# NVlabs/intrinsic3d

Measured on AMD Instinct MI355X. Metric: Gauss-Newton iterations/s at the finest SDF level, higher is better.
Workload: dtype f32

## Files before the change

### include/intrinsic3d_hip.h

```cpp
#ifndef INTRINSIC3D_HIP_H
#define INTRINSIC3D_HIP_H
#include <stdint.h>
#ifdef __cplusplus
extern "C" {
#endif

typedef struct i3d_context i3d_context;

typedef enum {
    I3D_OK = 0,
    I3D_ERR_INVALID_ARGUMENT = 1,
    I3D_ERR_NO_DEVICE = 2,
    I3D_ERR_HIP = 3,
    I3D_ERR_STATE = 4,
    I3D_ERR_CAPACITY = 5,
    I3D_ERR_COMM = 6,
    I3D_ERR_IO = 7
} i3d_status;

int  i3d_create(int32_t device_ordinal, i3d_context** out);
void i3d_destroy(i3d_context* ctx);
const char* i3d_last_error(const i3d_context* ctx);
const char* i3d_version(void);

// ... 173 lines not shown
    i3d_track_stats base;
    int64_t photo_samples;
    double  photo_rms_initial, photo_rms_final;
} i3d_track_rgbd_stats;

void i3d_track_rgbd_desc_default(i3d_track_rgbd_desc* d);
int  i3d_track_frame_rgbd(i3d_context* ctx, const i3d_track_rgbd_desc* desc, int32_t width, int32_t height, const float* depth, const float* luminance,
                          double* pose6_io, i3d_track_rgbd_stats* stats);
int  i3d_debug_track_rgbd_sums(i3d_context* ctx, const i3d_track_rgbd_desc* desc, int32_t width, int32_t height, const float* depth, const float* luminance,
                               int32_t level, const double* pose_ref6, const double* pose_cur6, double* sums31, int64_t* inliers, int64_t* photo_samples);

int i3d_png_info(const uint8_t* data, uint64_t size, int32_t* width, int32_t* height, int32_t* channels, int32_t* bit_depth);
int i3d_png_decode(const uint8_t* data, uint64_t size, void* pixels, uint64_t capacity_bytes);
int i3d_pose_mat_to_vec6(const float* cam_to_world16, double* pose6);
typedef struct i3d_sensor i3d_sensor;
int  i3d_sensor_open(const char* folder, int32_t max_frames, float min_depth, float max_depth, i3d_sensor** out);
int  i3d_sensor_open_yaml(const char* sensor_yml, i3d_sensor** out, float* min_depth , float* max_depth );
void i3d_sensor_close(i3d_sensor* s);
int  i3d_sensor_info(const i3d_sensor* s, int32_t* num_frames, int32_t* num_loaded, int32_t* color_wh , int32_t* depth_wh ,
                     float* color_intr4 , float* depth_intr4);
int  i3d_sensor_color(const i3d_sensor* s, int32_t id, uint8_t* bgr );
int  i3d_sensor_depth(const i3d_sensor* s, int32_t id, float* depth );
int  i3d_sensor_pose(const i3d_sensor* s, int32_t id, float* cam_to_world16);
int  i3d_sensor_set_pose(i3d_sensor* s, int32_t id, const float* cam_to_world16);
int  i3d_sensor_set_pose_vec6(i3d_sensor* s, int32_t id, const double* pose_world_to_cam6);
int  i3d_sensor_save_poses(const i3d_sensor* s, const char* path);
int i3d_keyframes_load(const char* path, int32_t* window_size, uint64_t capacity, double* scores, uint8_t* is_keyframe, uint64_t* count);
int i3d_keyframes_save(const char* path, int32_t window_size, uint64_t count, const double* scores, const uint8_t* is_keyframe);
int i3d_keyframes_select(int32_t window_size, uint64_t count, const double* scores, uint8_t* is_keyframe);
int i3d_blur_score(const uint8_t* image, int32_t width, int32_t height, int32_t channels, double* score);
int i3d_init_frames_from_sensor(i3d_context* ctx, int32_t device_ordinal, const i3d_sensor* s, uint64_t num_flags, const uint8_t* is_keyframe,
                                int32_t num_rgbd_levels, int32_t frame_capacity, int32_t* frame_ids, int32_t* num_keyframes);

typedef struct i3d_fusion i3d_fusion;
int  i3d_fusion_create(int32_t device_ordinal, float voxel_size, float depth_min, float depth_max, const float* clip6, uint64_t initial_capacity, i3d_fusion** out);
void i3d_fusion_destroy(i3d_fusion* f);
const char* i3d_fusion_last_error(const i3d_fusion* f);
int  i3d_fusion_integrate(i3d_fusion* f, int32_t depth_w, int32_t depth_h, const float* depth_intr4, int32_t color_w, int32_t color_h, const float* color_intr4,
                          const float* depth, const uint8_t* bgr, const float* pose_cam_to_world16, int32_t erode_window);
int  i3d_fusion_finish(i3d_fusion* f, int32_t correct_iterations, uint64_t* count);
int  i3d_fusion_info(const i3d_fusion* f, uint64_t* frames, uint64_t* allocated, uint64_t* capacity, int32_t* correct_launches);
int  i3d_fusion_get(const i3d_fusion* f, int32_t* keys, float* sdf, float* weight, uint8_t* color);
int  i3d_fusion_save(const i3d_fusion* f, const char* path);

int i3d_fusion_render(i3d_fusion* f, const i3d_render_desc* desc, float* depth, float* normal, i3d_render_stats* stats);
int i3d_fusion_track(i3d_fusion* f, const i3d_track_desc* desc, int32_t width, int32_t height, const float* depth, double* pose6_io, i3d_track_stats* stats);

typedef struct {
    int32_t use_refined_sdf;
    int32_t project;
    int32_t max_steps;
    double  tolerance_voxels;
} i3d_query_desc;

typedef struct {
    int64_t valid, projected;
    double  sum_abs_sdf, sum_sq_sdf, max_abs_sdf;
    double  sum_abs_distance, sum_sq_distance, max_abs_distance;
    int64_t steps;
} i3d_query_stats;

void i3d_query_desc_default(i3d_query_desc* d);
int  i3d_query_points(i3d_context* ctx, const i3d_query_desc* desc, int64_t n, const double* points,
                      double* sdf, float* normal , float* albedo, double* foot , double* distance, uint8_t* status, i3d_query_stats* stats);
int  i3d_fusion_query_points(i3d_fusion* f, const i3d_query_desc* desc, int64_t n, const double* points,
                             double* sdf, float* normal , double* foot , double* distance, uint8_t* status, i3d_query_stats* stats);

typedef struct {
    int32_t use_refined_sdf;
    int32_t iterations;
    double  max_distance;
    double  stop_rotation, stop_translation;
} i3d_register_desc;

typedef struct {
    int32_t iterations;
    int32_t status;
    int64_t valid, inliers;
    double  rms_initial, rms_final;
    double  min_pivot_ratio;
} i3d_register_stats;

void i3d_register_desc_default(i3d_register_desc* d);
int  i3d_register_points(i3d_context* ctx, const i3d_register_desc* desc, int64_t n, const double* points , double* pose6_io, i3d_register_stats* stats);
int  i3d_fusion_register_points(i3d_fusion* f, const i3d_register_desc* desc, int64_t n, const double* points, double* pose6_io, i3d_register_stats* stats);

typedef struct {
    int32_t use_refined_sdf;
    int32_t use_context_camera;
    double  intrinsics4[4], distortion5[5];
    int32_t iterations;
    int32_t stride;
    double  max_distance;
    double  huber_delta;
    float   min_depth, max_depth;
    double  stop_rotation, stop_translation;
} i3d_track_sdf_desc;

typedef struct {
    int32_t iterations, status;
    int64_t valid_pixels, valid, inliers;
    double  rms_initial, rms_final;
    double  min_pivot_ratio;
} i3d_track_sdf_stats;

void i3d_track_sdf_desc_default(i3d_track_sdf_desc* d);
int  i3d_track_frame_sdf(i3d_context* ctx, const i3d_track_sdf_desc* desc, int32_t width, int32_t height, const float* depth, double* pose6_io,
                         i3d_track_sdf_stats* stats);
int  i3d_fusion_track_sdf(i3d_fusion* f, const i3d_track_sdf_desc* desc, int32_t width, int32_t height, const float* depth, double* pose6_io,
                          i3d_track_sdf_stats* stats);

int  i3d_track_frames_sdf(i3d_context* ctx, const i3d_track_sdf_desc* desc, int32_t num_frames, int32_t width, int32_t height,
                          const float* depth, double* poses6_io, i3d_track_sdf_stats* stats);
int  i3d_track_keyframes_sdf(i3d_context* ctx, const i3d_track_sdf_desc* desc, int32_t level, int32_t num, const int32_t* frames,
                             double* poses6_io, i3d_track_sdf_stats* stats);

int i3d_comm_unique_id(void* out128, int32_t* bytes);
int i3d_comm_init(i3d_context* ctx, int32_t rank, int32_t world, const void* unique_id, int32_t id_bytes);
void* i3d_comm_sim_create(int32_t world);
void  i3d_comm_sim_destroy(void* shared);
int   i3d_comm_init_sim(i3d_context* ctx, void* shared, int32_t rank);
int   i3d_shard_plan(int32_t A, int32_t world, int32_t rank, const int32_t* anbr, const uint8_t* active,
                     int32_t* chunk, int32_t* own0, int32_t* own1, uint8_t* in_compute_list );
int32_t i3d_shard_vec_index(int32_t a, int32_t chunk, int32_t albedo);
int   i3d_shard_need(int32_t A, int32_t world, const int32_t* anbr , const uint8_t* active , uint64_t* need );
int   i3d_comm_stats(i3d_context* ctx, int64_t* halo_calls, int64_t* halo_bytes_sent, int64_t* reduce_calls, int64_t* reduce_bytes,
                     int32_t* halo_entries_send, int32_t* halo_entries_recv, int32_t* ghost_tiles, int32_t* compute_list);
const char* i3d_comm_transport(i3d_context* ctx);

enum { I3D_K_CLASSIFY = 0, I3D_K_OBSERVE, I3D_K_BUILD, I3D_K_EG_PASS , I3D_K_GATHER, I3D_K_COST, I3D_K_VECTOR, I3D_K_SH,
       I3D_K_EG_AUX ,
       I3D_K_COMM ,
       I3D_K_EG_MR2, I3D_K_EG_MR3 , I3D_K_COUNT };
int i3d_timing_enable(i3d_context* ctx, int32_t on);
int i3d_timing_select(i3d_context* ctx, uint32_t category_mask);
int i3d_timing_get(i3d_context* ctx, double* ms , int64_t* launches , int32_t reset);
int i3d_timing_get_work(i3d_context* ctx, double* ms , int64_t* launches );
int i3d_timing_get_work_ex(i3d_context* ctx, double* ms, int64_t* launches, double* slow_ms , int64_t* slow_launches );
const char* i3d_kernel_name(int32_t k);
int i3d_problem_sizes(i3d_context* ctx, int64_t out[6]);

int i3d_debug_assemble(i3d_context* ctx, const i3d_optimizer_config* cfg, int32_t iteration, int32_t* slots_out);
int64_t i3d_debug_map_order(const int32_t* keys, int64_t n, int32_t mode, int32_t* order);
int i3d_debug_flags(i3d_context* ctx, uint8_t* flags );
int i3d_debug_eg_rows(i3d_context* ctx, int32_t* frame , float* weight ,
                      float* residual , float* jac );
int i3d_debug_reg_rows(i3d_context* ctx, uint8_t* has_er , uint8_t* has_es , float* ea_weight );
int i3d_debug_neighbors(i3d_context* ctx, int32_t* nbr );
int i3d_debug_normal_eq(i3d_context* ctx, double* gradient, double* jtj_diag, double* cost);
int i3d_debug_jtj_apply(i3d_context* ctx, const double* x, double* y);
int i3d_debug_counters(i3d_context* ctx, int64_t* stream_syncs);
int i3d_debug_ladder_stats(i3d_context* ctx, int64_t* out6);
int i3d_debug_ladder_passes(i3d_context* ctx, int64_t* out8);
int i3d_debug_cull_stats(i3d_context* ctx, int64_t* pairs, int64_t* culled);

int i3d_debug_register_sums(i3d_context* ctx, const i3d_register_desc* desc, int64_t n, const double* points, const double* pose6, const double* pivot3,
                            double* sums29, int64_t* valid);
int i3d_debug_register_row_cap(i3d_context* ctx, int32_t rows);
int i3d_debug_track_sdf_sums(i3d_context* ctx, const i3d_track_sdf_desc* desc, int32_t width, int32_t height, const float* depth,
                             const double* pose6 , const double* pivot3, double* sums29, int64_t* valid, int64_t* valid_pixels);
int i3d_debug_track_batch_frames(i3d_context* ctx, int32_t frames_per_chunk);

#ifdef __cplusplus
}
#endif
#endif
```

### intrinsic3d_amd/binding.py

```python
from __future__ import annotations

import ctypes as C
import os

import numpy as np

_HERE = os.path.dirname(os.path.abspath(__file__))
LIB_PATH = os.environ.get("I3D_LIB") or os.path.join(_HERE, "libintrinsic3d_hip.so")

K_NAMES = ["classify", "observe", "build", "eg_pass", "gather", "cost", "vector", "sh", "eg_aux", "comm", "eg_mr2", "eg_mr3"]


class OptimizerConfig(C.Structure):
    _fields_ = [("iterations", C.c_int32), ("lm_steps", C.c_int32),
                ("lambda_g", C.c_double), ("lambda_r0", C.c_double), ("lambda_r1", C.c_double),
                ("lambda_s0", C.c_double), ("lambda_s1", C.c_double), ("lambda_a", C.c_double),
                ("fix_poses", C.c_int32), ("fix_intrinsics", C.c_int32), ("fix_distortion", C.c_int32),
                ("occlusion_distance", C.c_float), ("num_observations", C.c_int32),
                ("thres_shell", C.c_double), ("grid_level", C.c_int32), ("rgbd_level", C.c_int32),
                ("pcg_fixed_iterations", C.c_int32), ("verbose", C.c_int32), ("carry_trust_radius", C.c_int32), ("fix_sdf", C.c_int32)]


class IterationStats(C.Structure):
    _fields_ = [("rows", C.c_int64 * 4), ("weight_sum", C.c_double * 4), ("type_weight", C.c_double * 4),
# ... 93 lines not shown
    names = tuple(k for k in QUERY_OUTPUTS if has_albedo or k != "albedo")
    if outputs is None:
        outputs = tuple(k for k in names if d.project or k not in ("foot", "distance"))
    unknown = set(outputs) - set(names)
    if unknown:
        raise ValueError(f"{what}: unknown outputs {sorted(unknown)}")
    shape = {"sdf": ((n,), np.float64), "normal": ((n, 3), np.float32), "albedo": ((n,), np.float32), "foot": ((n, 3), np.float64),
             "distance": ((n,), np.float64), "status": ((n,), np.uint8)}
    out = {k: np.zeros(*shape[k]) for k in outputs}
    st = QueryStats()
    check(call(C.byref(d), n, _p(pts), *[_p(out.get(k)) for k in names], C.byref(st)), what)
    out["stats"] = st.as_dict()
    return out


class RegisterDesc(C.Structure):
    _fields_ = [("use_refined_sdf", C.c_int32), ("iterations", C.c_int32), ("max_distance", C.c_double), ("stop_rotation", C.c_double),
                ("stop_translation", C.c_double)]


class RegisterStats(C.Structure):
    _fields_ = [("iterations", C.c_int32), ("status", C.c_int32), ("valid", C.c_int64), ("inliers", C.c_int64), ("rms_initial", C.c_double),
                ("rms_final", C.c_double), ("min_pivot_ratio", C.c_double)]

    def as_dict(self):
        return {k: (float if t is C.c_double else int)(getattr(self, k)) for k, t in self._fields_}


def register_desc_default(**kw) -> RegisterDesc:
    d = RegisterDesc()
    load().i3d_register_desc_default(C.byref(d))
    for k, v in kw.items():
        if k == "refined":
            d.use_refined_sdf = int(bool(v))
        elif k in dict(RegisterDesc._fields_):
            setattr(d, k, v)
        else:
            raise ValueError(f"register_desc_default: unknown field {k}")
    return d


def _register(call, what, check, points, pose, desc):
    d = register_desc_default(**desc)
    pts = np.ascontiguousarray(points, np.float64).reshape(-1, 3)
    p6 = np.array(pose, np.float64).reshape(6).copy()
    st = RegisterStats()
    check(call(C.byref(d), pts.shape[0], _p(pts), _p(p6), C.byref(st)), what)
    return p6, st.as_dict()


class TrackSdfDesc(C.Structure):
    _fields_ = [("use_refined_sdf", C.c_int32), ("use_context_camera", C.c_int32), ("intrinsics4", C.c_double * 4), ("distortion5", C.c_double * 5),
                ("iterations", C.c_int32), ("stride", C.c_int32), ("max_distance", C.c_double), ("huber_delta", C.c_double),
                ("min_depth", C.c_float), ("max_depth", C.c_float), ("stop_rotation", C.c_double), ("stop_translation", C.c_double)]


class TrackSdfStats(C.Structure):
    _fields_ = [("iterations", C.c_int32), ("status", C.c_int32), ("valid_pixels", C.c_int64), ("valid", C.c_int64), ("inliers", C.c_int64),
                ("rms_initial", C.c_double), ("rms_final", C.c_double), ("min_pivot_ratio", C.c_double)]

    def as_dict(self):
        return {k: (float if t is C.c_double else int)(getattr(self, k)) for k, t in self._fields_}


def track_sdf_desc_default(**kw) -> TrackSdfDesc:
    d = TrackSdfDesc()
    load().i3d_track_sdf_desc_default(C.byref(d))
    for k, v in kw.items():
        if k in ("intr", "intrinsics4"):
            d.intrinsics4[:] = [float(x) for x in v]
        elif k in ("dist", "distortion5"):
            d.distortion5[:] = [float(x) for x in v]
        elif k == "refined":
            d.use_refined_sdf = int(bool(v))
        elif k in dict(TrackSdfDesc._fields_):
            setattr(d, k, v)
        else:
            raise ValueError(f"track_sdf_desc_default: unknown field {k}")
    return d


def _track_sdf(call, what, check, depth, pose6, d):
    dep = np.ascontiguousarray(depth, np.float32)
    h, w = dep.shape
    pose = np.ascontiguousarray(np.asarray(pose6, np.float64).reshape(6)).copy()
    st = TrackSdfStats()
    check(call(C.byref(d), int(w), int(h), _p(dep), _p(pose), C.byref(st)), what)
    return pose, st.as_dict()


def track_desc_default(**kw) -> TrackDesc:
    d = TrackDesc()
    load().i3d_track_desc_default(C.byref(d))
    for k, v in kw.items():
        if k == "iterations":
            it = [int(x) for x in v] + [0] * (4 - len(v))
            d.iterations[:] = it[:4]
        elif k in ("intr", "intrinsics4"):
            d.intrinsics4[:] = [float(x) for x in v]; d.use_context_camera = 0
        elif k in ("dist", "distortion5"):
            d.distortion5[:] = [float(x) for x in v]; d.use_context_camera = 0
        elif k == "refined":
            d.use_refined_sdf = int(bool(v))
        elif k in dict(TrackDesc._fields_):
            setattr(d, k, v)
        else:
            raise ValueError(f"track_desc_default: unknown field {k}")
    return d


def track_rgbd_desc_default(**kw) -> TrackRgbdDesc:
    d = TrackRgbdDesc()
    load().i3d_track_rgbd_desc_default(C.byref(d))
    own = ("geometric_weight", "photo_weight", "max_photo_residual")
    for k in own:
        if k in kw:
            setattr(d, k, float(kw[k]))
    base = {k: v for k, v in kw.items() if k not in own}
    if base:
        d.base = track_desc_default(**base)
    return d


REFINE_CALLBACK = C.CFUNCTYPE(None, C.c_void_p, C.c_int32, C.c_int32, C.c_int32, C.c_int32)


class GridView(C.Structure):
    _fields_ = [("num_voxels", C.c_int64), ("voxel_size", C.c_float), ("truncation", C.c_float),
                ("keys", C.c_void_p), ("sdf", C.c_void_p), ("sdf_refined", C.c_void_p), ("albedo", C.c_void_p),
                ("weight", C.c_void_p), ("color", C.c_void_p)]


EXPORTS = ["i3d_create", "i3d_destroy", "i3d_last_error", "i3d_version", "i3d_set_grid", "i3d_get_grid", "i3d_update_grid",
           "i3d_set_frames", "i3d_set_frames_rgbd", "i3d_get_frame_image", "i3d_resize_depth", "i3d_set_camera", "i3d_get_camera", "i3d_set_voxel_sh", "i3d_get_voxel_sh",
           "i3d_optimizer_config_default", "i3d_optimize", "i3d_optimize_host", "i3d_estimate_sh",
           "i3d_set_grid_from_tsdf_records", "i3d_recompute_colors", "i3d_clear_outside_thin_shell", "i3d_upsample", "i3d_grid_info",
           "i3d_export_grid", "i3d_refine",
           "i3d_tsdf_read_header", "i3d_tsdf_read_records", "i3d_tsdf_write", "i3d_sbr_write", "i3d_sbr_read", "i3d_write_poses",
           "i3d_write_intrinsics", "i3d_read_intrinsics", "i3d_config_load_yaml", "i3d_yaml_get",
           "i3d_extract_mesh", "i3d_get_mesh", "i3d_render_view", "i3d_track_desc_default", "i3d_track_frame", "i3d_track_rgbd_desc_default", "i3d_track_frame_rgbd",
           "i3d_query_desc_default", "i3d_query_points", "i3d_fusion_query_points",
           "i3d_register_desc_default", "i3d_register_points", "i3d_fusion_register_points", "i3d_debug_register_sums", "i3d_debug_register_row_cap",
           "i3d_track_sdf_desc_default", "i3d_track_frame_sdf", "i3d_fusion_track_sdf", "i3d_debug_track_sdf_sums",
           "i3d_track_frames_sdf", "i3d_track_keyframes_sdf", "i3d_debug_track_batch_frames",
           "i3d_export_mesh_ply", "i3d_write_ply", "i3d_mc_tables", "i3d_visualization_colors",
           "i3d_png_info", "i3d_png_decode", "i3d_pose_mat_to_vec6", "i3d_sensor_open", "i3d_sensor_open_yaml", "i3d_sensor_close", "i3d_sensor_info", "i3d_sensor_color",
           "i3d_sensor_depth", "i3d_sensor_pose", "i3d_sensor_set_pose", "i3d_sensor_set_pose_vec6", "i3d_sensor_save_poses",
           "i3d_mesh_remove_loose_components", "i3d_keyframes_load", "i3d_keyframes_save", "i3d_keyframes_select", "i3d_blur_score", "i3d_init_frames_from_sensor",
           "i3d_fusion_create", "i3d_fusion_destroy", "i3d_fusion_last_error", "i3d_fusion_integrate", "i3d_fusion_finish", "i3d_fusion_info", "i3d_fusion_get",
           "i3d_fusion_save", "i3d_fusion_render", "i3d_fusion_track", "i3d_shard_need", "i3d_comm_stats",
           "i3d_comm_unique_id", "i3d_comm_init", "i3d_comm_sim_create", "i3d_comm_sim_destroy", "i3d_comm_init_sim", "i3d_shard_plan", "i3d_shard_vec_index",
           "i3d_comm_transport", "i3d_timing_enable", "i3d_timing_select", "i3d_timing_get", "i3d_timing_get_work", "i3d_timing_get_work_ex", "i3d_kernel_name", "i3d_problem_sizes",
           "i3d_debug_assemble", "i3d_debug_map_order", "i3d_debug_flags", "i3d_debug_eg_rows", "i3d_debug_reg_rows", "i3d_debug_neighbors",
           "i3d_debug_normal_eq", "i3d_debug_jtj_apply", "i3d_debug_counters", "i3d_debug_cull_stats", "i3d_debug_ladder_stats", "i3d_debug_ladder_passes", "i3d_debug_track_sums", "i3d_debug_track_rgbd_sums"]

_lib = None


def load():
    global _lib
    if _lib is not None:
        return _lib
    if not os.path.exists(LIB_PATH):
        raise RuntimeError(f"{LIB_PATH} is missing: build it with `make -C intrinsic3d_amd/csrc` "
                           "(or __graft_entry__.build()); the product path has no CPU fallback")
    L = C.CDLL(LIB_PATH)
    vp, i32, i64, f32, f64 = C.c_void_p, C.c_int32, C.c_int64, C.c_float, C.c_double
    L.i3d_create.restype = i32; L.i3d_create.argtypes = [i32, C.POINTER(vp)]
    L.i3d_destroy.argtypes = [vp]
    L.i3d_last_error.restype = C.c_char_p; L.i3d_last_error.argtypes = [vp]
    L.i3d_version.restype = C.c_char_p
    L.i3d_set_grid.restype = i32; L.i3d_set_grid.argtypes = [vp, C.POINTER(GridView)]
    L.i3d_get_grid.restype = i32; L.i3d_get_grid.argtypes = [vp, vp, vp]
    L.i3d_update_grid.restype = i32; L.i3d_update_grid.argtypes = [vp, vp, vp, vp]
    L.i3d_set_frames.restype = i32; L.i3d_set_frames.argtypes = [vp, i32, i32, vp, vp, vp, vp, vp]
    L.i3d_set_frames_rgbd.restype = i32; L.i3d_set_frames_rgbd.argtypes = [vp, i32, i32, i32, i32, vp, vp]
    L.i3d_resize_depth.restype = i32; L.i3d_resize_depth.argtypes = [i32, i32, i32, vp, vp, i32, i32, vp, vp]
    L.i3d_get_frame_image.restype = i32; L.i3d_get_frame_image.argtypes = [vp, i32, i32, vp, vp]
    L.i3d_set_camera.restype = i32; L.i3d_set_camera.argtypes = [vp, vp, vp, vp]
    L.i3d_get_camera.restype = i32; L.i3d_get_camera.argtypes = [vp, vp, vp, vp]
    L.i3d_set_voxel_sh.restype = i32; L.i3d_set_voxel_sh.argtypes = [vp, vp]
    L.i3d_get_voxel_sh.restype = i32; L.i3d_get_voxel_sh.argtypes = [vp, vp]
    L.i3d_optimizer_config_default.argtypes = [C.POINTER(OptimizerConfig)]
    L.i3d_optimize.restype = i32; L.i3d_optimize.argtypes = [vp, C.POINTER(OptimizerConfig), vp]
    L.i3d_optimize_host.restype = i32
    L.i3d_optimize_host.argtypes = [i32, C.POINTER(OptimizerConfig), C.POINTER(GridView), vp, vp, i32, i32, vp, vp, vp, vp, vp, vp, vp, vp, vp]
    L.i3d_estimate_sh.restype = i32
    L.i3d_estimate_sh.argtypes = [vp, f32, f64, f64, C.POINTER(i32), vp, vp, i32, C.POINTER(ShStats)]
    L.i3d_comm_unique_id.restype = i32; L.i3d_comm_unique_id.argtypes = [vp, C.POINTER(i32)]
    L.i3d_comm_init.restype = i32; L.i3d_comm_init.argtypes = [vp, i32, i32, vp, i32]
    L.i3d_comm_sim_create.restype = vp; L.i3d_comm_sim_create.argtypes = [i32]
    L.i3d_comm_sim_destroy.argtypes = [vp]
    L.i3d_comm_init_sim.restype = i32; L.i3d_comm_init_sim.argtypes = [vp, vp, i32]
    L.i3d_shard_plan.restype = i32; L.i3d_shard_plan.argtypes = [i32, i32, i32, vp, vp, C.POINTER(i32), C.POINTER(i32), C.POINTER(i32), vp]
    L.i3d_shard_vec_index.restype = i32; L.i3d_shard_vec_index.argtypes = [i32, i32, i32]
    L.i3d_shard_need.restype = i32; L.i3d_shard_need.argtypes = [i32, i32, vp, vp, vp]
    L.i3d_comm_stats.restype = i32; L.i3d_comm_stats.argtypes = [vp] * 9
    L.i3d_timing_enable.restype = i32; L.i3d_timing_enable.argtypes = [vp, i32]
    L.i3d_timing_select.restype = i32; L.i3d_timing_select.argtypes = [vp, C.c_uint32]
    L.i3d_timing_get.restype = i32; L.i3d_timing_get.argtypes = [vp, vp, vp, i32]
    L.i3d_timing_get_work.restype = i32; L.i3d_timing_get_work.argtypes = [vp, vp, vp]
    L.i3d_timing_get_work_ex.restype = i32; L.i3d_timing_get_work_ex.argtypes = [vp, vp, vp, vp, vp]
    L.i3d_kernel_name.restype = C.c_char_p; L.i3d_kernel_name.argtypes = [i32]
    L.i3d_comm_transport.restype = C.c_char_p; L.i3d_comm_transport.argtypes = [vp]
    L.i3d_problem_sizes.restype = i32; L.i3d_problem_sizes.argtypes = [vp, vp]
    L.i3d_debug_assemble.restype = i32; L.i3d_debug_assemble.argtypes = [vp, C.POINTER(OptimizerConfig), i32, C.POINTER(i32)]
    L.i3d_debug_flags.restype = i32; L.i3d_debug_flags.argtypes = [vp, vp]
    L.i3d_debug_eg_rows.restype = i32; L.i3d_debug_eg_rows.argtypes = [vp, vp, vp, vp, vp]
    L.i3d_debug_reg_rows.restype = i32; L.i3d_debug_reg_rows.argtypes = [vp, vp, vp, vp]
    L.i3d_debug_neighbors.restype = i32; L.i3d_debug_neighbors.argtypes = [vp, vp]
    L.i3d_debug_normal_eq.restype = i32; L.i3d_debug_normal_eq.argtypes = [vp, vp, vp, C.POINTER(f64)]
    L.i3d_debug_jtj_apply.restype = i32; L.i3d_debug_jtj_apply.argtypes = [vp, vp, vp]
    L.i3d_debug_counters.restype = i32; L.i3d_debug_counters.argtypes = [vp, vp]
    L.i3d_debug_ladder_stats.restype = i32; L.i3d_debug_ladder_stats.argtypes = [vp, vp]
    L.i3d_debug_ladder_passes.restype = i32; L.i3d_debug_ladder_passes.argtypes = [vp, vp]
    L.i3d_debug_cull_stats.restype = i32; L.i3d_debug_cull_stats.argtypes = [vp, vp, vp]
    L.i3d_set_grid_from_tsdf_records.restype = i32; L.i3d_set_grid_from_tsdf_records.argtypes = [vp, f32, i64, vp, vp, vp, vp]
    L.i3d_recompute_colors.restype = i32; L.i3d_recompute_colors.argtypes = [vp, f32, i32]
    L.i3d_clear_outside_thin_shell.restype = i32; L.i3d_clear_outside_thin_shell.argtypes = [vp, f64, C.POINTER(i64)]
    L.i3d_upsample.restype = i32; L.i3d_upsample.argtypes = [vp, C.POINTER(i64)]
    L.i3d_grid_info.restype = i32; L.i3d_grid_info.argtypes = [vp, C.POINTER(i64), C.POINTER(f32), C.POINTER(f32)]
    L.i3d_export_grid.restype = i32; L.i3d_export_grid.argtypes = [vp, vp, vp, vp, vp, vp, vp]
    L.i3d_refine.restype = i32; L.i3d_refine.argtypes = [vp, C.POINTER(RefineConfig), C.POINTER(OptimizerConfig), REFINE_CALLBACK, vp]
    u64 = C.c_uint64; cp = C.c_char_p
    L.i3d_tsdf_read_header.restype = i32; L.i3d_tsdf_read_header.argtypes = [cp, C.POINTER(f32), C.POINTER(f32), C.POINTER(f32), C.POINTER(u64), C.POINTER(f32)]
    L.i3d_tsdf_read_records.restype = i32; L.i3d_tsdf_read_records.argtypes = [cp, u64, vp, vp, vp, vp]
    L.i3d_tsdf_write.restype = i32; L.i3d_tsdf_write.argtypes = [cp, f32, f32, f32, f32, u64, vp, vp, vp, vp]
    L.i3d_sbr_write.restype = i32; L.i3d_sbr_write.argtypes = [cp, f32, f32, f32, f32, u64, vp, vp, vp, vp, vp, vp]
    L.i3d_sbr_read.restype = i32; L.i3d_sbr_read.argtypes = [cp, u64, vp, vp, vp, vp, vp, vp]
    L.i3d_write_poses.restype = i32; L.i3d_write_poses.argtypes = [cp, i32, vp, vp]
    L.i3d_write_intrinsics.restype = i32; L.i3d_write_intrinsics.argtypes = [cp, i32, i32, vp, vp]
    L.i3d_read_intrinsics.restype = i32; L.i3d_read_intrinsics.argtypes = [cp, C.POINTER(i32), C.POINTER(i32), vp, vp]
    L.i3d_extract_mesh.restype = i32; L.i3d_extract_mesh.argtypes = [vp, i32, i32, i32, C.POINTER(i64), C.POINTER(i64)]
    L.i3d_get_mesh.restype = i32; L.i3d_get_mesh.argtypes = [vp, vp, vp, vp]
    L.i3d_export_mesh_ply.restype = i32; L.i3d_export_mesh_ply.argtypes = [vp, cp, i32, i32, i32]
    L.i3d_write_ply.restype = i32; L.i3d_write_ply.argtypes = [cp, i64, vp, vp, i64, vp]
    L.i3d_mesh_remove_loose_components.restype = i32; L.i3d_mesh_remove_loose_components.argtypes = [vp, vp, vp, vp, vp]
    L.i3d_render_view.restype = i32; L.i3d_render_view.argtypes = [vp, C.POINTER(RenderDesc), vp, vp, vp, vp, vp, vp, C.POINTER(RenderStats)]
    L.i3d_track_desc_default.restype = None; L.i3d_track_desc_default.argtypes = [C.POINTER(TrackDesc)]
    L.i3d_track_frame.restype = i32; L.i3d_track_frame.argtypes = [vp, C.POINTER(TrackDesc), i32, i32, vp, vp, C.POINTER(TrackStats)]
    L.i3d_debug_track_sums.restype = i32; L.i3d_debug_track_sums.argtypes = [vp, C.POINTER(TrackDesc), i32, i32, vp, i32, vp, vp, vp, vp]
    L.i3d_track_rgbd_desc_default.restype = None; L.i3d_track_rgbd_desc_default.argtypes = [C.POINTER(TrackRgbdDesc)]
    L.i3d_track_frame_rgbd.restype = i32; L.i3d_track_frame_rgbd.argtypes = [vp, C.POINTER(TrackRgbdDesc), i32, i32, vp, vp, vp, C.POINTER(TrackRgbdStats)]
    L.i3d_debug_track_rgbd_sums.restype = i32
    L.i3d_debug_track_rgbd_sums.argtypes = [vp, C.POINTER(TrackRgbdDesc), i32, i32, vp, vp, i32, vp, vp, vp, vp, vp]
    L.i3d_query_desc_default.restype = None; L.i3d_query_desc_default.argtypes = [C.POINTER(QueryDesc)]
    L.i3d_query_points.restype = i32; L.i3d_query_points.argtypes = [vp, C.POINTER(QueryDesc), i64, vp, vp, vp, vp, vp, vp, vp, C.POINTER(QueryStats)]
    L.i3d_fusion_query_points.restype = i32; L.i3d_fusion_query_points.argtypes = [vp, C.POINTER(QueryDesc), i64, vp, vp, vp, vp, vp, vp, C.POINTER(QueryStats)]
    L.i3d_register_desc_default.restype = None; L.i3d_register_desc_default.argtypes = [C.POINTER(RegisterDesc)]
    L.i3d_register_points.restype = i32; L.i3d_register_points.argtypes = [vp, C.POINTER(RegisterDesc), i64, vp, vp, C.POINTER(RegisterStats)]
    L.i3d_fusion_register_points.restype = i32; L.i3d_fusion_register_points.argtypes = [vp, C.POINTER(RegisterDesc), i64, vp, vp, C.POINTER(RegisterStats)]
    L.i3d_debug_register_sums.restype = i32; L.i3d_debug_register_sums.argtypes = [vp, C.POINTER(RegisterDesc), i64, vp, vp, vp, vp, C.POINTER(i64)]
    L.i3d_debug_register_row_cap.restype = i32; L.i3d_debug_register_row_cap.argtypes = [vp, i32]
    L.i3d_track_sdf_desc_default.restype = None; L.i3d_track_sdf_desc_default.argtypes = [C.POINTER(TrackSdfDesc)]
    L.i3d_track_frame_sdf.restype = i32; L.i3d_track_frame_sdf.argtypes = [vp, C.POINTER(TrackSdfDesc), i32, i32, vp, vp, C.POINTER(TrackSdfStats)]
    L.i3d_fusion_track_sdf.restype = i32; L.i3d_fusion_track_sdf.argtypes = [vp, C.POINTER(TrackSdfDesc), i32, i32, vp, vp, C.POINTER(TrackSdfStats)]
    L.i3d_debug_track_sdf_sums.restype = i32
    L.i3d_debug_track_sdf_sums.argtypes = [vp, C.POINTER(TrackSdfDesc), i32, i32, vp, vp, vp, vp, C.POINTER(i64), C.POINTER(i64)]
    L.i3d_track_frames_sdf.restype = i32; L.i3d_track_frames_sdf.argtypes = [vp, C.POINTER(TrackSdfDesc), i32, i32, i32, vp, vp, vp]
    L.i3d_track_keyframes_sdf.restype = i32; L.i3d_track_keyframes_sdf.argtypes = [vp, C.POINTER(TrackSdfDesc), i32, i32, vp, vp, vp]
    L.i3d_debug_track_batch_frames.restype = i32; L.i3d_debug_track_batch_frames.argtypes = [vp, i32]
    L.i3d_mc_tables.restype = i32; L.i3d_mc_tables.argtypes = [vp, vp]
    L.i3d_config_load_yaml.restype = i32; L.i3d_config_load_yaml.argtypes = [cp, C.POINTER(RefineConfig), C.POINTER(OptimizerConfig)]
    u64 = C.c_uint64; f32 = C.c_float
    L.i3d_fusion_create.restype = i32; L.i3d_fusion_create.argtypes = [i32, f32, f32, f32, vp, u64, C.POINTER(vp)]
    L.i3d_fusion_destroy.restype = None; L.i3d_fusion_destroy.argtypes = [vp]
    L.i3d_fusion_last_error.restype = C.c_char_p; L.i3d_fusion_last_error.argtypes = [vp]
    L.i3d_fusion_integrate.restype = i32; L.i3d_fusion_integrate.argtypes = [vp, i32, i32, vp, i32, i32, vp, vp, vp, vp, i32]
    L.i3d_fusion_finish.restype = i32; L.i3d_fusion_finish.argtypes = [vp, i32, vp]
    L.i3d_fusion_info.restype = i32; L.i3d_fusion_info.argtypes = [vp, vp, vp, vp, vp]
    L.i3d_fusion_get.restype = i32; L.i3d_fusion_get.argtypes = [vp, vp, vp, vp, vp]
    L.i3d_fusion_save.restype = i32; L.i3d_fusion_save.argtypes = [vp, cp]
    L.i3d_fusion_render.restype = i32; L.i3d_fusion_render.argtypes = [vp, C.POINTER(RenderDesc), vp, vp, C.POINTER(RenderStats)]
    L.i3d_fusion_track.restype = i32; L.i3d_fusion_track.argtypes = [vp, C.POINTER(TrackDesc), i32, i32, vp, vp, C.POINTER(TrackStats)]
    L.i3d_debug_map_order.restype = i64; L.i3d_debug_map_order.argtypes = [vp, i64, i32, vp]
    L.i3d_blur_score.restype = i32; L.i3d_blur_score.argtypes = [vp, i32, i32, i32, vp]
    L.i3d_yaml_get.restype = i32; L.i3d_yaml_get.argtypes = [cp, cp, vp, u64]
    L.i3d_png_info.restype = i32; L.i3d_png_info.argtypes = [vp, u64, vp, vp, vp, vp]
    L.i3d_png_decode.restype = i32; L.i3d_png_decode.argtypes = [vp, u64, vp, u64]
    L.i3d_pose_mat_to_vec6.restype = i32; L.i3d_pose_mat_to_vec6.argtypes = [vp, vp]
    L.i3d_sensor_open.restype = i32; L.i3d_sensor_open.argtypes = [cp, i32, f32, f32, C.POINTER(vp)]
    L.i3d_sensor_close.restype = None; L.i3d_sensor_close.argtypes = [vp]
    L.i3d_sensor_info.restype = i32; L.i3d_sensor_info.argtypes = [vp, vp, vp, vp, vp, vp, vp]
    L.i3d_sensor_color.restype = i32; L.i3d_sensor_color.argtypes = [vp, i32, vp]
    L.i3d_sensor_depth.restype = i32; L.i3d_sensor_depth.argtypes = [vp, i32, vp]
    L.i3d_sensor_pose.restype = i32; L.i3d_sensor_pose.argtypes = [vp, i32, vp]
    L.i3d_sensor_set_pose.restype = i32; L.i3d_sensor_set_pose.argtypes = [vp, i32, vp]
    L.i3d_sensor_set_pose_vec6.restype = i32; L.i3d_sensor_set_pose_vec6.argtypes = [vp, i32, vp]
    L.i3d_sensor_save_poses.restype = i32; L.i3d_sensor_save_poses.argtypes = [vp, cp]
    L.i3d_keyframes_load.restype = i32; L.i3d_keyframes_load.argtypes = [cp, vp, u64, vp, vp, vp]
    L.i3d_keyframes_save.restype = i32; L.i3d_keyframes_save.argtypes = [cp, i32, u64, vp, vp]
    L.i3d_keyframes_select.restype = i32; L.i3d_keyframes_select.argtypes = [i32, u64, vp, vp]
    L.i3d_init_frames_from_sensor.restype = i32; L.i3d_init_frames_from_sensor.argtypes = [vp, i32, vp, u64, vp, i32, i32, vp, vp]
    _lib = L
    return L


def default_config(**kw) -> OptimizerConfig:
    cfg = OptimizerConfig()
    load().i3d_optimizer_config_default(C.byref(cfg))
    for k, v in kw.items():
        setattr(cfg, k, v)
    return cfg


def _pyramid_sizes(w, h, levels):
    out = [(int(w), int(h))]
    for _ in range(1, int(levels)):
        out.append((out[-1][0] // 2, out[-1][1] // 2))
    return out


def _p(a):
    return None if a is None else a.ctypes.data_as(C.c_void_p)


class I3DError(RuntimeError):
    pass


class Context:

    def __init__(self, device: int = 0):
        self.L = load()
        h = C.c_void_p()
        rc = self.L.i3d_create(int(device), C.byref(h))
        if rc != 0:
            raise I3DError(f"i3d_create failed ({rc}): {self.L.i3d_last_error(None).decode()}")
        self.h = h
        self.N = 0
        self.K = 0
        self._keep = []

    def _check(self, rc, what):
        if rc != 0:
            raise I3DError(f"{what} failed ({rc}): {self.L.i3d_last_error(self.h).decode()}")

    def close(self):
        if self.h:
            self.L.i3d_destroy(self.h)
            self.h = None

    def __enter__(self):
        return self

    def __exit__(self, *a):
        self.close()

    def set_grid(self, voxel_size, keys, sdf, sdf_refined, albedo, weight, color, truncation=None):
        keys = np.ascontiguousarray(keys, np.int32); sdf = np.ascontiguousarray(sdf, np.float64)
        sr = np.ascontiguousarray(sdf_refined, np.float64); al = np.ascontiguousarray(albedo, np.float64)
        w = np.ascontiguousarray(weight, np.float32); col = np.ascontiguousarray(color, np.uint8)
        gv = GridView(keys.shape[0], float(voxel_size), float(np.float32(voxel_size) * np.float32(5.0)) if truncation is None else float(truncation),
                      _p(keys), _p(sdf), _p(sr), _p(al), _p(w), _p(col))
        self._check(self.L.i3d_set_grid(self.h, C.byref(gv)), "i3d_set_grid")
        self.N = keys.shape[0]

    def set_frames(self, frames, levels):
        K = len(frames); self.K = K
        ws = np.array([frames[0]["lum"][l].shape[1] for l in range(levels)], np.int32)
        hs = np.array([frames[0]["lum"][l].shape[0] for l in range(levels)], np.int32)
        self._sizes = [(int(w), int(h)) for w, h in zip(ws, hs)]
        arr_t = C.c_void_p * (K * levels)
        lum = arr_t(); dep = arr_t(); bgr = arr_t(); keep = []
        for f in range(K):
            for l in range(levels):
                a = np.ascontiguousarray(frames[f]["lum"][l], np.float32); b = np.ascontiguousarray(frames[f]["depth"][l], np.float32)
                c = frames[f].get("bgr")
# ... 173 lines not shown
    def track_frame_sdf(self, depth, pose6, **desc):
        return _track_sdf(lambda *a: self.L.i3d_track_frame_sdf(self.h, *a), "i3d_track_frame_sdf", self._check, depth, pose6, track_sdf_desc_default(**desc))

    def track_frames_sdf(self, depths, poses, **desc):
        d = track_sdf_desc_default(**desc)
        dep = np.ascontiguousarray(depths, np.float32)
        if dep.ndim != 3:
            raise ValueError("track_frames_sdf: depths must be [B, h, w]")
        n, h, w = dep.shape
        po = np.ascontiguousarray(np.asarray(poses, np.float64).reshape(-1, 6)).copy()
        if po.shape[0] != n:
            raise ValueError("track_frames_sdf: one pose per frame")
        st = (TrackSdfStats * max(n, 1))()
        self._check(self.L.i3d_track_frames_sdf(self.h, C.byref(d), int(n), int(w), int(h), _p(dep), _p(po), C.cast(st, C.c_void_p)), "i3d_track_frames_sdf")
        return po, [st[i].as_dict() for i in range(n)]

    def track_keyframes_sdf(self, poses, level=0, frames=None, **desc):
        d = track_sdf_desc_default(**dict(dict(use_context_camera=1), **desc))
        po = np.ascontiguousarray(np.asarray(poses, np.float64).reshape(-1, 6)).copy()
        n = po.shape[0]
        idx = None if frames is None else np.ascontiguousarray(frames, np.int32).reshape(-1)
        if idx is not None and idx.shape[0] != n:
            raise ValueError("track_keyframes_sdf: one pose per frame index")
        st = (TrackSdfStats * max(n, 1))()
        self._check(self.L.i3d_track_keyframes_sdf(self.h, C.byref(d), int(level), int(n), _p(idx), _p(po), C.cast(st, C.c_void_p)), "i3d_track_keyframes_sdf")
        return po, [st[i].as_dict() for i in range(n)]

    def debug_track_batch_frames(self, n):
        self._check(self.L.i3d_debug_track_batch_frames(self.h, int(n)), "i3d_debug_track_batch_frames")

    def debug_track_sdf_sums(self, depth, pose6, pivot3, **desc):
        d = track_sdf_desc_default(**desc)
        dep = np.ascontiguousarray(depth, np.float32)
        h, w = dep.shape
        po = np.ascontiguousarray(pose6, np.float64).reshape(6); pv = np.ascontiguousarray(pivot3, np.float64).reshape(3)
        sums = np.full(29, -1.0); v = C.c_int64(-1); u = C.c_int64(-1)
        self._check(self.L.i3d_debug_track_sdf_sums(self.h, C.byref(d), int(w), int(h), _p(dep), _p(po), _p(pv), _p(sums), C.byref(v), C.byref(u)),
                    "i3d_debug_track_sdf_sums")
        return sums, int(v.value), int(u.value)

    def _level_size(self, level):
        return self._sizes[level] if 0 <= level < len(getattr(self, "_sizes", ())) else (0, 0)

    @staticmethod
    def comm_unique_id() -> bytes:
        buf = C.create_string_buffer(256); n = C.c_int32(0)
        rc = load().i3d_comm_unique_id(buf, C.byref(n))
        if rc != 0:
            raise I3DError(f"i3d_comm_unique_id failed ({rc})")
        return buf.raw[:n.value]

    def comm_init(self, rank: int, world: int, unique_id: bytes):
        self._check(self.L.i3d_comm_init(self.h, int(rank), int(world), unique_id, len(unique_id)), "i3d_comm_init")

    def comm_stats(self):
        a = [C.c_int64() for _ in range(4)]; b = [C.c_int32() for _ in range(4)]
        self._check(self.L.i3d_comm_stats(self.h, *[C.byref(x) for x in a], *[C.byref(x) for x in b]), "i3d_comm_stats")
        return dict(zip(["halo_calls", "halo_bytes_sent", "reduce_calls", "reduce_bytes", "halo_send", "halo_recv", "ghost_tiles", "compute_list"], [x.value for x in a + b]))

    def comm_transport(self) -> str:
        return (self.L.i3d_comm_transport(self.h) or b"").decode()

    def comm_init_sim(self, shared, rank: int):
        self._check(self.L.i3d_comm_init_sim(self.h, shared, int(rank)), "i3d_comm_init_sim")

    def optimize(self, cfg: OptimizerConfig):
        stats = (IterationStats * cfg.iterations)()
        self._check(self.L.i3d_optimize(self.h, C.byref(cfg), C.cast(stats, C.c_void_p)), "i3d_optimize")
        return list(stats)

    def estimate_sh(self, subvolume_size, lambda_reg, thres_shell, cap=8192):
        S = C.c_int32(0); sh = np.zeros((cap, 9)); idx = np.zeros((cap, 3), np.int32); st = ShStats()
        self._check(self.L.i3d_estimate_sh(self.h, float(subvolume_size), float(lambda_reg), float(thres_shell), C.byref(S), _p(sh), _p(idx), cap, C.byref(st)), "i3d_estimate_sh")
        return sh[:S.value].copy(), idx[:S.value].copy(), st

    def timing_enable(self, on=True):
        self._check(self.L.i3d_timing_enable(self.h, 1 if on else 0), "i3d_timing_enable")

    def timing_select(self, names):
        mask = 0
        for n in names:
            mask |= 1 << K_NAMES.index(n)
        self._check(self.L.i3d_timing_select(self.h, mask), "i3d_timing_select")

    def timing_get_work(self):
        ms = np.zeros(len(K_NAMES)); n = np.zeros(len(K_NAMES), np.int64)
        self._check(self.L.i3d_timing_get_work(self.h, _p(ms), _p(n)), "i3d_timing_get_work")
        return {k: (ms[i], int(n[i])) for i, k in enumerate(K_NAMES)}

    def timing_get_work_ex(self):
        ms = np.zeros(len(K_NAMES)); n = np.zeros(len(K_NAMES), np.int64); sms = np.zeros(len(K_NAMES)); sn = np.zeros(len(K_NAMES), np.int64)
        self._check(self.L.i3d_timing_get_work_ex(self.h, _p(ms), _p(n), _p(sms), _p(sn)), "i3d_timing_get_work_ex")
        return {k: (ms[i], int(n[i]), sms[i], int(sn[i])) for i, k in enumerate(K_NAMES)}

    def timing_get(self, reset=True):
        ms = np.zeros(len(K_NAMES)); n = np.zeros(len(K_NAMES), np.int64)
        self._check(self.L.i3d_timing_get(self.h, _p(ms), _p(n), 1 if reset else 0), "i3d_timing_get")
        return {k: (ms[i], int(n[i])) for i, k in enumerate(K_NAMES)}

    def problem_sizes(self):
        o = np.zeros(6, np.int64)
        self._check(self.L.i3d_problem_sizes(self.h, _p(o)), "i3d_problem_sizes")
        return dict(zip(["active", "eg", "er", "es", "ea", "free"], [int(x) for x in o]))

    def debug_assemble(self, cfg, iteration=0):
        s = C.c_int32(0)
        self._check(self.L.i3d_debug_assemble(self.h, C.byref(cfg), int(iteration), C.byref(s)), "i3d_debug_assemble")
        self.slots = s.value
        return s.value

    def debug_flags(self):
        f = np.zeros(self.N, np.uint8)
        self._check(self.L.i3d_debug_flags(self.h, _p(f)), "i3d_debug_flags")
        return f

    def debug_eg_rows(self, jac=True):
        S = self.slots
        fr = np.zeros((self.N, S), np.int32); w = np.zeros((self.N, S), np.float32); r = np.zeros((self.N, S), np.float32)
        J = np.zeros((self.N, S, 29), np.float32) if jac else None
        self._check(self.L.i3d_debug_eg_rows(self.h, _p(fr), _p(w), _p(r), _p(J)), "i3d_debug_eg_rows")
        return fr, w, r, J

    def debug_reg_rows(self):
        er = np.zeros(self.N, np.uint8); es = np.zeros(self.N, np.uint8); ea = np.zeros((self.N, 6), np.float32)
        self._check(self.L.i3d_debug_reg_rows(self.h, _p(er), _p(es), _p(ea)), "i3d_debug_reg_rows")
        return er, es, ea

    def debug_neighbors(self):
        nb = np.zeros((self.N, 18), np.int32)
        self._check(self.L.i3d_debug_neighbors(self.h, _p(nb)), "i3d_debug_neighbors")
        return nb

    def debug_normal_eq(self):
        NP = 2 * self.N + 6 * self.K + 9
        g = np.zeros(NP); d = np.zeros(NP); cost = C.c_double(0)
        self._check(self.L.i3d_debug_normal_eq(self.h, _p(g), _p(d), C.byref(cost)), "i3d_debug_normal_eq")
        return g, d, cost.value

    def debug_counters(self):
        n = C.c_int64(0)
        self._check(self.L.i3d_debug_counters(self.h, C.byref(n)), "i3d_debug_counters")
        return {"stream_syncs": int(n.value)}

    def debug_ladder_stats(self):
        a = (C.c_int64 * 6)()
        self._check(self.L.i3d_debug_ladder_stats(self.h, a), "i3d_debug_ladder_stats")
        return {"batches": int(a[0]), "row_streams": int(a[1]), "system_passes": int(a[2]), "resyncs": int(a[3]), "unused_systems": int(a[4]), "depth": int(a[5])}

    def debug_ladder_passes(self):
        a = (C.c_int64 * 8)()
        self._check(self.L.i3d_debug_ladder_passes(self.h, a), "i3d_debug_ladder_passes")
        return {"live": [int(a[n]) for n in range(7)], "paired": int(a[7])}

    def debug_cull_stats(self):
        a = C.c_int64(0); b = C.c_int64(0)
        self._check(self.L.i3d_debug_cull_stats(self.h, C.byref(a), C.byref(b)), "i3d_debug_cull_stats")
        return int(a.value), int(b.value)

    def debug_jtj_apply(self, x):
        x = np.ascontiguousarray(x, np.float64); y = np.zeros_like(x)
        self._check(self.L.i3d_debug_jtj_apply(self.h, _p(x), _p(y)), "i3d_debug_jtj_apply")
        return y


def shard_need(A, world, anbr, active):
    anbr = np.ascontiguousarray(anbr, np.int32); active = np.ascontiguousarray(active, np.uint8); need = np.zeros(A, np.uint64)
    rc = load().i3d_shard_need(int(A), int(world), _p(anbr), _p(active), _p(need))
    if rc != 0:
        raise I3DError(f"i3d_shard_need failed ({rc})")
    return need


def shard_plan(A, world, rank, anbr, active):
    anbr = np.ascontiguousarray(anbr, np.int32); active = np.ascontiguousarray(active, np.uint8)
    ch = C.c_int32(); o0 = C.c_int32(); o1 = C.c_int32(); mask = np.zeros(A, np.uint8)
    rc = load().i3d_shard_plan(int(A), int(world), int(rank), _p(anbr), _p(active), C.byref(ch), C.byref(o0), C.byref(o1), _p(mask))
    if rc != 0:
        raise I3DError(f"i3d_shard_plan failed ({rc})")
    return ch.value, o0.value, o1.value, mask.astype(bool)


def _io_check(rc, what):
    if rc != 0:
        raise I3DError(f"{what} failed ({rc})")


def tsdf_read(path):
    L = load(); p = str(path).encode()
    vs, tr, iw, ml = C.c_float(), C.c_float(), C.c_float(), C.c_float(); n = C.c_uint64()
    _io_check(L.i3d_tsdf_read_header(p, C.byref(vs), C.byref(tr), C.byref(iw), C.byref(n), C.byref(ml)), "i3d_tsdf_read_header")
    N = int(n.value)
    out = dict(voxel_size=np.float32(vs.value), truncation=np.float32(tr.value), integration_weight_sample=np.float32(iw.value),
               max_load_factor=np.float32(ml.value), keys=np.zeros((N, 3), np.int32), sdf=np.zeros(N, np.float32),
               weight=np.zeros(N, np.float32), color=np.zeros((N, 3), np.uint8))
    _io_check(L.i3d_tsdf_read_records(p, N, _p(out["keys"]), _p(out["sdf"]), _p(out["weight"]), _p(out["color"])), "i3d_tsdf_read_records")
    return out


def tsdf_write(path, voxel_size, keys, sdf, weight, color, truncation=None, integration_weight_sample=0.0, max_load_factor=0.6):
    keys = np.ascontiguousarray(keys, np.int32); sdf = np.ascontiguousarray(sdf, np.float32)
    weight = np.ascontiguousarray(weight, np.float32); color = np.ascontiguousarray(color, np.uint8)
    tr = float(np.float32(voxel_size) * np.float32(5.0)) if truncation is None else float(truncation)
    _io_check(load().i3d_tsdf_write(str(path).encode(), float(voxel_size), tr, float(integration_weight_sample), float(max_load_factor), len(sdf),
                                    _p(keys), _p(sdf), _p(weight), _p(color)), "i3d_tsdf_write")


def sbr_write(path, voxel_size, grid, truncation=None, integration_weight_sample=0.0, max_load_factor=0.6):
    tr = float(np.float32(voxel_size) * np.float32(5.0)) if truncation is None else float(truncation)
    g = {k: np.ascontiguousarray(v) for k, v in grid.items() if isinstance(v, np.ndarray)}
    _io_check(load().i3d_sbr_write(str(path).encode(), float(voxel_size), tr, float(integration_weight_sample), float(max_load_factor), len(g["sdf"]),
                                   _p(g["keys"]), _p(g["sdf"]), _p(g["sdf_refined"]), _p(g["albedo"]), _p(g["weight"]), _p(g["color"])), "i3d_sbr_write")


def sbr_read(path):
    L = load(); p = str(path).encode()
    vs = C.c_float(); n = C.c_uint64()
    _io_check(L.i3d_tsdf_read_header(p, C.byref(vs), None, None, C.byref(n), None), "i3d_tsdf_read_header")
    N = int(n.value)
    out = dict(voxel_size=np.float32(vs.value), keys=np.zeros((N, 3), np.int32), sdf=np.zeros(N), sdf_refined=np.zeros(N), albedo=np.zeros(N),
               weight=np.zeros(N, np.float32), color=np.zeros((N, 3), np.uint8))
    _io_check(L.i3d_sbr_read(p, N, _p(out["keys"]), _p(out["sdf"]), _p(out["sdf_refined"]), _p(out["albedo"]), _p(out["weight"]), _p(out["color"])), "i3d_sbr_read")
    return out


def write_poses(path, timestamps, poses_world_to_cam):
    t = np.ascontiguousarray(timestamps, np.float64); p = np.ascontiguousarray(poses_world_to_cam, np.float64).reshape(-1, 6)
    _io_check(load().i3d_write_poses(str(path).encode(), len(t), _p(t), _p(p)), "i3d_write_poses")


def write_intrinsics(path, width, height, intr, dist):
    a = np.ascontiguousarray(intr, np.float64); d = np.ascontiguousarray(dist, np.float64)
    _io_check(load().i3d_write_intrinsics(str(path).encode(), int(width), int(height), _p(a), _p(d)), "i3d_write_intrinsics")


def read_intrinsics(path):
    w, h = C.c_int32(), C.c_int32(); a = np.zeros(4); d = np.zeros(5)
    rc = load().i3d_read_intrinsics(str(path).encode(), C.byref(w), C.byref(h), _p(a), _p(d))
    return rc == 0, int(w.value), int(h.value), a, d


def load_yaml_config(path):
    rc = RefineConfig(); oc = default_config()
    _io_check(load().i3d_config_load_yaml(str(path).encode(), C.byref(rc), C.byref(oc)), "i3d_config_load_yaml")
    return rc, oc


def yaml_get(path, key, default=None):
    buf = C.create_string_buffer(4096)
    rc = load().i3d_yaml_get(str(path).encode(), key.encode(), buf, 4096)
    if rc == 1 and default is not None:
        return default
    _io_check(rc, f"i3d_yaml_get({key})")
    return buf.value.decode()


def mesh_remove_loose_components(vertices, colors, faces):
    v = np.array(vertices, np.float32, copy=True).reshape(-1, 3); f = np.array(faces, np.int32, copy=True).reshape(-1, 3)
    c = None if colors is None else np.array(colors, np.uint8, copy=True).reshape(-1, 3)
    nv, nf = C.c_int64(len(v)), C.c_int64(len(f))
    _io_check(load().i3d_mesh_remove_loose_components(C.byref(nv), _p(v), None if c is None else _p(c), C.byref(nf), _p(f)), "i3d_mesh_remove_loose_components")
    return v[:nv.value].copy(), (None if c is None else c[:nv.value].copy()), f[:nf.value].copy()


COLOR_MODES = {"": 0, "albedo": 1, "normals": 2, "lap": 3, "lum": 4, "lum_grad": 5, "shading_sv": 6, "shading_sv_const": 7, "chroma": 8}


def visualization_colors(mode, voxel_size, keys, sdf_refined, albedo, weight, color, subvolume_size=0.0, sub_index=None, sub_sh=None, visit_rank=None):
    k = np.ascontiguousarray(keys, np.int32); n = len(k); out = np.zeros((n, 3), np.uint8)
    s = np.ascontiguousarray(sdf_refined, np.float64); a = np.ascontiguousarray(albedo, np.float64); w = np.ascontiguousarray(weight, np.float32); c = np.ascontiguousarray(color, np.uint8)
    si = None if sub_index is None else np.ascontiguousarray(sub_index, np.int32); ss = None if sub_sh is None else np.ascontiguousarray(sub_sh, np.float64)
    L = load(); L.i3d_visualization_colors.restype = C.c_int32
    L.i3d_visualization_colors.argtypes = [C.c_int32, C.c_float, C.c_int64] + [C.c_void_p] * 6 + [C.c_float, C.c_int32, C.c_void_p, C.c_void_p, C.c_void_p]
    vr = None if visit_rank is None else np.ascontiguousarray(visit_rank, np.int64)
    _io_check(L.i3d_visualization_colors(COLOR_MODES[mode] if isinstance(mode, str) else int(mode), float(voxel_size), n, _p(k), _p(s), _p(a), _p(w), _p(c), _p(vr), float(subvolume_size),
                                         0 if si is None else len(si), _p(si), _p(ss), _p(out)), "i3d_visualization_colors")
    return out


def write_ply(path, vertices, colors, faces):
    v = np.ascontiguousarray(vertices, np.float32); f = np.ascontiguousarray(faces, np.int32)
    c = None if colors is None else np.ascontiguousarray(colors, np.uint8)
    _io_check(load().i3d_write_ply(str(path).encode(), len(v), _p(v), _p(c), len(f), _p(f)), "i3d_write_ply")


def mc_tables():
    ntri = np.zeros(256, np.uint8); tri = np.zeros((256, 16), np.int8)
    mx = load().i3d_mc_tables(_p(ntri), _p(tri))
    return ntri, tri, mx


def optimize_host(cfg, voxel_size, keys, sdf, sdf_refined, albedo, weight, color, frames, levels, intr, dist, poses, voxel_sh, device=0):
    L = load()
    keys = np.ascontiguousarray(keys, np.int32); sdf = np.ascontiguousarray(sdf, np.float64)
    sr = np.array(sdf_refined, np.float64); al = np.array(albedo, np.float64)
    w = np.ascontiguousarray(weight, np.float32); col = np.ascontiguousarray(color, np.uint8)
    gv = GridView(keys.shape[0], float(voxel_size), float(np.float32(voxel_size) * np.float32(5.0)), _p(keys), _p(sdf), _p(sr), _p(al), _p(w), _p(col))
    K = len(frames)
    ws = np.array([frames[0]["lum"][l].shape[1] for l in range(levels)], np.int32); hs = np.array([frames[0]["lum"][l].shape[0] for l in range(levels)], np.int32)
    arr_t = C.c_void_p * (K * levels); lum = arr_t(); dep = arr_t(); keep = []
    for f in range(K):
        for l in range(levels):
            a = np.ascontiguousarray(frames[f]["lum"][l], np.float32); b = np.ascontiguousarray(frames[f]["depth"][l], np.float32); keep += [a, b]
            lum[f * levels + l] = a.ctypes.data; dep[f * levels + l] = b.ctypes.data
    i4 = np.array(intr, np.float64); d5 = np.array(dist, np.float64); p6 = np.array(poses, np.float64); sh = np.ascontiguousarray(voxel_sh, np.float64)
    stats = (IterationStats * cfg.iterations)()
    rc = L.i3d_optimize_host(int(device), C.byref(cfg), C.byref(gv), _p(sr), _p(al), K, int(levels), _p(ws), _p(hs), C.cast(lum, C.c_void_p), C.cast(dep, C.c_void_p),
# ... 202 lines not shown
```

### intrinsic3d_amd/csrc/device/kernels.hpp

```cpp
#pragma once
#include "common.hpp"
#include "p2p_device.hpp"

namespace i3d {

struct HashTable { unsigned long long* keys; int* vals; unsigned int mask; };
void launch_sort_keys(hipStream_t st, int N, const int* keys_xyz , unsigned long long* sort_keys, int* iota);
void launch_permute_grid(hipStream_t st, int N, const int* perm, const int* keys_xyz, const double* sdf, const double* sdf_ref,
                         const double* alb, const float* w, const uint8_t* rgb,
                         int* cx, int* cy, int* cz, int* rank, double* sdf0, double* x_sdf, double* x_alb, float* f_sdf, float* f_alb,
                         float* weight, uchar4* color);
void launch_hash_build(hipStream_t st, int N, const int* cx, const int* cy, const int* cz, HashTable t);
void launch_nbr_build(hipStream_t st, int N, const int* cx, const int* cy, const int* cz, HashTable t, int* nbr);
void launch_classify(hipStream_t st, GridView g, OptParams p, int* active_flag);
void launch_compact(hipStream_t st, int N, const int* active_flag, const int* active_scan, const uint8_t* flags, int* aidx, int* alist, uint8_t* aflags);
void launch_partition_blocks(hipStream_t st, GridView g, int A, int* alist, uint8_t* aflags, int* aidx);
void launch_group_rows(hipStream_t st, int A, const uint8_t* nrows, int* gmax);
void launch_anbr(hipStream_t st, int N, int A, int Acap, const int* alist, const int* nbr, const int* aidx, int* anbr);
void launch_scatter_sh(hipStream_t st, int N, const int* rank, const double* sh_visit , float* sh );
void launch_gather_visit(hipStream_t st, int N, const int* rank, const double* x_sdf, const double* x_alb, double* out_sdf, double* out_alb);
void launch_update_fields(hipStream_t st, int N, const int* rank, const double* sdf_ref, const double* alb, const uint8_t* rgb,
                          double* x_sdf, double* x_alb, float* f_sdf, float* f_alb, uchar4* color);

void launch_observe(hipStream_t st, GridView g, RowView r, OptParams p, const FrameConst* frames, const unsigned* cull_mask = nullptr, bool prefilter = false);
constexpr int CULL_BLOCK = 8, CULL_MAX_LEVELS = 12;
struct CullPyramid { int levels, cells; int bw[CULL_MAX_LEVELS], bh[CULL_MAX_LEVELS], off[CULL_MAX_LEVELS]; };
CullPyramid cull_pyramid(int w, int h);
void launch_depth_blocks(hipStream_t st, const FrameConst* frames, int K, int w, int h, float2* out);
void launch_group_cull(hipStream_t st, GridView g, RowView r, OptParams p, const FrameConst* frames, const float2* dblocks, float4* bounds, unsigned* mask);

void launch_build(hipStream_t st, GridView g, RowView r, OptParams p, const FrameConst* frames, bool with_jacobian, double* cost_out , double* scratch,
                  const double* cam9 = nullptr, const LmState* lm = nullptr);
void launch_weight_sums(hipStream_t st, RowView r, GridView g, bool with_cost, double* sums13 , double* scratch);

enum PassMode { PASS_GRAD = 0, PASS_JTJP = 1, PASS_COLNORM = 2 };
struct Seg2 { size_t off0, off1; int n; };
struct PassBuffers {
    float* C;
    float* treg;
    double* shared;
    double* blocks;
    float* part; int part_stride;
};
struct GradColBuffers {
    float* Cg; float* Cc;
    float* tregg; float* tregc;
    float* part; int part_stride;
    int col_off;
    double* cost_partials; double* cost_out;
};
int  launch_eg_gradcol(hipStream_t st, GridView g, RowView r, OptParams p, GradColBuffers b);
int  launch_eg_pass(hipStream_t st, PassMode mode, GridView g, RowView r, OptParams p, const float* u , PassBuffers b, const PcgState* state);
void launch_sum_rows(hipStream_t st, PassMode mode, int K, const float* part, int nrows, int stride, double* shared, double* blocks);
void launch_gather(hipStream_t st, PassMode mode, RowView r, PassBuffers b, float* out );
int  launch_gather_tail(hipStream_t st, RowView r, PassBuffers b, float* out, const float* S, const float* D2, const float* v, double* dot_partials ,
                        bool dot_atomic, const PcgState* state);
void launch_reduce_partials(hipStream_t st, const double* partials, int nblk, int ncomp, double* dst, const PcgState* state, bool assign = false);
void launch_shared_finalize(hipStream_t st, size_t tail_off, int K, OptParams p, const double* shared, float* out , bool tail, const float* S, const float* D2,
                            const float* v, double* dot_out, const PcgState* state);

void launch_fill(hipStream_t st, int n, float* x, float v);
void launch_fill_d(hipStream_t st, int n, double* x, double v);
void launch_int_to_double(hipStream_t st, const int* src, double* dst);
void launch_mul(hipStream_t st, int n, const float* a, const float* b, float* out);
void launch_scale_from_colnorm(hipStream_t st, int n, const float* c, const float* freemask, float* S, float* cm);
void launch_lm_diag(hipStream_t st, int n, const float* c, const float* S, float inv_radius, float* D2, float* Minv_diag);
void launch_dot(hipStream_t st, int n, const float* a, const float* b, double* out , double* scratch);
void launch_count_above2(hipStream_t st, Seg2 sg, const float* a, const float* m, float tol, double* out, double* scratch);
void launch_count_above(hipStream_t st, int n, const float* a, const float* m, float tol, double* out, double* scratch);
void launch_dot2(hipStream_t st, Seg2 sg, const float* a, const float* b, double* out , double* scratch);
void launch_mul2(hipStream_t st, Seg2 sg, const float* a, const float* b, float* out);
void launch_freemask(hipStream_t st, RowView r, OptParams p, float* mask );

void launch_pcg_init(hipStream_t st, PcgState* state, int fixed_iterations, int max_iterations, const LmState* lm = nullptr);
int  launch_pcg_step(hipStream_t st, int mode, Seg2 sg, const float* p, const float* q, float* x, float* r, const float* b, const float* D2, const float* Minv,
                     float* z, const float* S_for_inline_q, double* partials , PcgState* state);
void launch_pcg_tail_x(hipStream_t st, size_t tail_off, int K, const float* p, float* x, const PcgState* state);
void launch_pcg_tail_a(hipStream_t st, int mode, size_t tail_off, int K, const float* Minv_blocks, const float* p, const float* q, float* x, float* r, const float* b,
                       const float* D2, float* z, const double* partials, int nblk, PcgState* state,
                       double* shared_zero, int nzero, int* host_flags, int seq,
                       const P2PDev& pd);
int  launch_pcg_direction(hipStream_t st, Seg2 sg, size_t tail_off, int ntail, const float* z, float* p, const float* S, float* u, const float* D2,
                          double* d2_partials , const PcgState* state);
void launch_pcg_tail_b(hipStream_t st, size_t tail_off, int K, OptParams p, double* shared, const double* pq_slice, const double* pq_partials, int nblk,
                       const double* pq_partials2, int nblk2, bool rowwise,
                       float* q, const float* S, const float* D2, const float* v, PcgState* state, const P2PDev& pd);
struct TilePlan {
    unsigned* lnbr;
    float* eaw_sym;
    int* halo_idx; int* halo_cnt;
    int* iota; int* ext_e; int* ext_pos;
    float* qh;
    int* ext_off;
    int* overflow;
    int T, hmax;
    int tile_first, ntiles_own;
    const int* ghost_tiles; int n_ghost;
    int det;
    const unsigned short* hp_off;
    const unsigned short* hp_src;
    int pull;
};
inline int tile_plan_pull_cap(int hmax) { return 4 * hmax; }
int    tile_plan_T();
int    tile_plan_tiles(int A);
int    tile_plan_hmax();
inline int tile_plan_hmax_of(int T) { return T == 1024 ? 2048 : 1536; }
inline int tile_plan_tiles_of(int A, int T) { return (A + T - 1) / T; }
size_t tile_plan_temp_bytes(int ntiles);
hipError_t launch_tile_plan(hipStream_t st, RowView r, TilePlan t, void* temp, size_t temp_bytes);
void launch_eaw_sym(hipStream_t st, RowView r, TilePlan t, const int* cflag );
int  launch_eg_tile(hipStream_t st, RowView r, OptParams p, const float* u, TilePlan t, double* shared, float* qacc, double* pq_partials ,
                    const PcgState* state, float* cam_partials = nullptr, int cam_stride = 0);
void launch_ext_offsets(hipStream_t st, int n, const int* ext_e, int A, int* ext_off);
void eg_tile_launch_shape(const TilePlan& t, int K, int& blocks, int& tiles_per_block);

struct LadVec;
int  eg_tile_mr_max_systems(int K);
int  launch_eg_tile_mr(hipStream_t st, RowView r, OptParams p, TilePlan t, int nsys, const int* sys, const float* u0, float* qacc0, float* qh0, double* pq0 , float* cam0, int cam_stride,
                       const PcgState* st0 , const LadVec& lv);
int  launch_eg_tile_mr_pair(hipStream_t st, RowView r, OptParams p, TilePlan t, int na, int nb, const int* sys, const float* u0, float* qacc0, float* qh0, double* pq0 , float* cam0,
                            int cam_stride, const PcgState* st0, const LadVec& lv);

struct ShardArgs {
    P2PDev pd; RimLists rim; int seq;
    int n_slice_partials;
    int n_rim_wg;
    const float* zb; float* pb; float* ub; const float* cmb; int chunk;
};
struct LadVec {
    size_t vec;
    size_t qh;
    size_t cam;
    size_t part;
    size_t mblk;
    size_t tail;
    int sysid[LADDER_MAX];
};
struct Step3Args {
    int nq; int chunk4;
    const float4* p; const float4* qacc; float4* x; float4* r; const float4* b; float4* z;
    const float4* cm; const LmState* lm;
    const int* ext_off; const int* ext_pos; const float2* qh; int e0;
    const double* pq_partials; int n_pq; const double* d2_partials; int n_d2;
    int n_slice_wg;
    int K; int fix_poses, fix_intr, fix_dist;
    const float* cam_partials; int n_cam; int cam_stride; const float* Mblk;
    const float* tp; float* tx; float* tr; const float* tb; const float* tD2; float* tz; const float* tS;
    double* step_partials;
    PcgState* cur;
    int sharded; ShardArgs sh;
    int lad_sys;
    const double* redop; int redop_stride;
};
void launch_pcg_init3(hipStream_t st, PcgState* st2 , int fixed_iterations, int max_iterations, const LmState* lm = nullptr);
int  launch_pcg_dir3(hipStream_t st, bool init, Seg2 sg, size_t tail_off, int ntail, const float* z, float* p, const float* S, float* u, const float* D2, const float* cm, const LmState* lm,
                     const double* step_partials, int n_step, double* d2_partials, const PcgState* prev, PcgState* next, int* host_flags, int seq,
                     const ShardArgs* sa = nullptr);
void launch_rim_u(hipStream_t st, const ShardArgs& sa, const PcgState* state);
int  pcg_step3_slice_wgs(int n_entries, int cap = 0);
int  pcg_step3_tail_wgs(int K);
int  launch_pcg_step3(hipStream_t st, int mode , Step3Args a);
void launch_halo_fold(hipStream_t st, RowView r, TilePlan t, float* qacc, const PcgState* state);
void launch_pcg_init_lad(hipStream_t st, PcgState* st2_all , int B, int fixed_iterations, int max_iterations, const LmState* lm);
int  launch_pcg_dir3_lad(hipStream_t st, bool init, int nsys, Seg2 sg, size_t tail_off, int ntail, const float* z0, float* p0, const float* S, float* u0, const float* tD2_0, const float* cm, const LmState* lm,
                         const double* step_partials0, int n_step, double* d2_partials0, PcgState* st2_0, int prev_parity, int* host_flags0, int seq, const LadVec& lv,
                         int n_slice_partials = 0, const double* red4_0 = nullptr );
int  launch_pcg_step3_lad(hipStream_t st, int mode, int nsys, Step3Args a, const LadVec& lv);
void launch_lad_reduce_step(hipStream_t st, int nsys, const double* step_partials0, int n_slice, double* red4_0, const LadVec& lv);
void launch_lad_reduce_op(hipStream_t st, int nsys, const float* cam_partials0, int n_cam, int cam_stride, int NS, const double* pq_partials0, int n_pq, const double* d2_partials0, int n_d2,
                          double* redop0, int redop_stride, const LadVec& lv);

void launch_need_mask(hipStream_t st, RowView r, int slice, unsigned long long* need );
void launch_halo_items(hipStream_t st, int A, int slice, int me, const unsigned long long* need, unsigned long long* items, int* count , int cap);
void launch_tile_flags(hipStream_t st, int A, int T, const int* cflag, int* tileflag );
size_t halo_sort_temp_bytes(int cap);
hipError_t launch_halo_sort(hipStream_t st, void* temp, size_t temp_bytes, const unsigned long long* in, unsigned long long* out, int n);

void launch_candidate(hipStream_t st, GridView g, RowView r, int K, float sign, const float* step, const float* S, const double* x_shared, double* xc_sdf, double* xc_alb,
                      double* xc_shared, double* norms2 , const float* mask, double* scratch, const LmState* lm = nullptr);
void launch_accept(hipStream_t st, GridView g, RowView r, const double* xc_sdf, const double* xc_alb, const LmState* lm = nullptr);
void launch_set_double(hipStream_t st, double* dst, double v);
void launch_lm_init(hipStream_t st, LmState* lm, const double* cost, const double* ngrad, const double* nfree, double radius0, LmRecord* rec, int seq);
void launch_lm_begin(hipStream_t st, LmState* lm, int K, int fix_poses, int fix_intr, int fix_dist, const double* cdiag, const double* tri, float* Mblk,
                     const float* tc, const float* tS, float* tD2, float* tMinv, LmRecord* rec, int seq);
void launch_lm_diag_dev(hipStream_t st, int n, const float* c, const float* S, const LmState* lm, float* D2, float* Minv);
void launch_cand_frames(hipStream_t st, int K, const double* xc, const FrameConst* base, FrameConst* out, const LmState* lm);
void launch_lm_decide(hipStream_t st, LmState* lm, const PcgState* ps, const double* norms2, const double* cand_cost, int attempt, int lm_steps, LmRecord* rec, int seq,
                      int lad_next = -1 , int debug_invalid = 0);
void launch_lm_begin_lad(hipStream_t st, LmState* lm, int B, int K, int fix_poses, int fix_intr, int fix_dist, const double* cdiag, const double* tri, float* Mblk, size_t mblk_stride,
                         const float* tc, const float* tS, float* tD2, size_t tail_stride, LmRecord* rec, int seq);
void launch_mark_compute(hipStream_t st, RowView r, int* flag);
void launch_compact_list(hipStream_t st, int A, const int* flag, const int* scan, int* list);

}
```

### intrinsic3d_amd/csrc/device/pcg_fused.hip

```cpp
#include "kernels.hpp"
#include "reduce_device.hpp"
#include <cstring>

namespace i3d {

constexpr int PF_THREADS = 512;
constexpr int PF_MAX_WG = 512;
constexpr int PF_POSES_PER_WG = 10;

template <int NC>
static __device__ inline void reduce_partials_all(const double* __restrict__ P, int nblk, double (&tot)[NC], double* sm ,
                                                  const double* __restrict__ P2 = nullptr, int nblk2 = 0 ) {
    double v[NC];
#pragma unroll
    for (int k = 0; k < NC; ++k) v[k] = 0.0;
    for (int i = threadIdx.x; i < nblk; i += PF_THREADS) {
#pragma unroll
        for (int k = 0; k < NC; ++k) v[k] += P[(size_t)i * NC + k];
    }
    for (int i = threadIdx.x; i < nblk2; i += PF_THREADS) {
#pragma unroll
        for (int k = 0; k < NC; ++k) v[k] += P2[(size_t)i * NC + k];
    }
#pragma unroll
    for (int k = 0; k < NC; ++k) for (int o = 32; o > 0; o >>= 1) v[k] += __shfl_down(v[k], o, 64);
    if ((threadIdx.x & 63) == 0) {
#pragma unroll
        for (int k = 0; k < NC; ++k) sm[k * 8 + (threadIdx.x >> 6)] = v[k];
    }
    __syncthreads();
#pragma unroll
    for (int k = 0; k < NC; ++k) { double t = 0.0; for (int w = 0; w < PF_THREADS / 64; ++w) t += sm[k * 8 + w]; tot[k] = t; }
    __syncthreads();
}

__global__ void k_pcg_init3(PcgState* st2, int fixed_iterations, int max_iterations, const LmState* lm) {
    const bool over = lm && lm->done;
    for (int b = 0; b < 2; ++b) {
        PcgState* st = st2 + b;
        for (int k = 0; k < 4; ++k) st->acc[k] = 0.0;
        st->rho = 0.0; st->last_rho = 1.0; st->pq = 0.0; st->alpha = 0.0; st->beta = 0.0; st->xbr = 0.0; st->xr = 0.0; st->d2xx = 0.0;
        st->Q0 = 0.0; st->Q1 = 0.0; st->it = 0; st->done = (fixed_iterations == 0 || over) ? 1 : 0; st->fixed_iterations = fixed_iterations; st->max_iterations = max_iterations;
    }
}
void launch_pcg_init3(hipStream_t st, PcgState* st2, int fixed_iterations, int max_iterations, const LmState* lm) { k_pcg_init3<<<1, 1, 0, st>>>(st2, fixed_iterations, max_iterations, lm); }

static __device__ inline void lm_from_colnorm(float cm, float inv_radius, float& s, float& d2, float& minv) { s = lm_scale(cm); lm_diag(cm, s, inv_radius, d2, minv); }

template <int SH>
static __device__ __forceinline__ void pcg_dir3_body(int init, int n4, int seg4, size_t tail_rel, int ntail, const float* __restrict__ z, float* __restrict__ p,
                                                        const float* __restrict__ S, float* __restrict__ u, const float* __restrict__ tD2 ,
                                                        const float* __restrict__ cm, const float inv_radius, const double* __restrict__ step_partials, int n_step, double* __restrict__ d2_partials,
                                                        const PcgState* __restrict__ prev, PcgState* __restrict__ next, int* host_flags, int seq, const ShardArgs& sa,
                                                        const double* __restrict__ red4 = nullptr ) {
    __shared__ double sm[4 * 8];
    __shared__ double smx[SH == 1 ? 4 * P2P_MAX_RANKS : 1];
    auto publish = [&](int done) { if (host_flags) { __hip_atomic_store(&host_flags[2 * (seq & 1) + 1], done, __ATOMIC_RELAXED, __HIP_MEMORY_SCOPE_SYSTEM);
                                                     __hip_atomic_store(&host_flags[2 * (seq & 1)], seq, __ATOMIC_RELEASE, __HIP_MEMORY_SCOPE_SYSTEM); } };
    const int n_rim = SH == 1 ? sa.n_rim_wg : 0, n_main = SH ? (int)gridDim.x - n_rim - 1 : (int)gridDim.x;
    const int lid = SH == 1 ? ((int)blockIdx.x < n_rim ? n_main + 1 + (int)blockIdx.x : (int)blockIdx.x - n_rim) : (int)blockIdx.x;
    const bool rim_wg = SH == 1 && lid > n_main, tail_wg = SH ? lid == n_main : lid == n_main - 1;
    const bool writer = lid == 0 && threadIdx.x == 0;
    const float4* z4 = reinterpret_cast<const float4*>(z); float4* p4 = reinterpret_cast<float4*>(p);
    const float4* C4 = reinterpret_cast<const float4*>(cm); float4* u4 = reinterpret_cast<float4*>(u);
    if (prev->done) { if (writer) { *next = *prev; publish(prev->done); } return; }
    double tot[4];
    if (!SH) reduce_partials_all<4>(step_partials, n_step, tot, sm);
    else if (SH == 2) {
        reduce_partials_all<4>(step_partials + 4 * (size_t)sa.n_slice_partials, n_step - sa.n_slice_partials, tot, sm);
#pragma unroll
        for (int k = 0; k < 4; ++k) tot[k] += red4[k];
    } else {
        const unsigned e32 = p2p_pass_epoch(seq, P2P_X_DIR);
        if (rim_wg) {
            const RimLists& rl = sa.rim;
            for (int j = (lid - n_main - 1) * PF_THREADS + threadIdx.x; j < rl.n_send; j += n_rim * PF_THREADS) {
                const int e = rl.send_idx[j], k = rl.send_peer[j];
                p2p_put_rim(sa.pd, 0, e32, k, j - rl.send_off[k], sa.zb[e], sa.zb[(size_t)sa.chunk + e]);
            }
        }
        {   double loc[4];
            reduce_partials_all<4>(step_partials, sa.n_slice_partials, loc, sm);
            if (lid == 0 && threadIdx.x < 4) p2p_put_double_all(sa.pd, 0, e32, threadIdx.x, threadIdx.x == 0 ? loc[0] : threadIdx.x == 1 ? loc[1] : threadIdx.x == 2 ? loc[2] : loc[3]); }
        double tl[4];
        reduce_partials_all<4>(step_partials + 4 * (size_t)sa.n_slice_partials, n_step - sa.n_slice_partials, tl, sm);
        p2p_sum_all<4>(sa.pd, 0, e32, tot, smx);
#pragma unroll
        for (int k = 0; k < 4; ++k) tot[k] += tl[k];
    }
    int it = prev->it, done = 0; bool stop = false;
    double Q0 = prev->Q0, Q1 = prev->Q1, xbr = prev->xbr, xr = prev->xr, d2xx = prev->d2xx;
    if (!init) {
        xbr = tot[1]; xr = tot[2]; d2xx = tot[3];
        it = it + 1;
        Q1 = -tot[1];
        if (prev->fixed_iterations >= 0) { Q0 = Q1; if (it >= prev->fixed_iterations) { done = 1; stop = true; } }
        else {
            const double zeta = (double)it * (Q1 - Q0) / Q1;
            if (zeta < 0.1) { done = 1; stop = true; }
            else { Q0 = Q1; if (it >= prev->max_iterations) { done = 1; stop = true; } }
        }
    }
    double rho = prev->rho, last_rho = prev->last_rho, beta = prev->beta;
    if (!stop) {
        const double rho_new = tot[0];
        if (rho_new == 0.0 || isinf(rho_new) || isnan(rho_new)) { done = 2; stop = true; }
        else {
            if (it > 0) { const double bt = rho_new / prev->rho; if (bt == 0.0 || isinf(bt) || isnan(bt)) { done = 2; stop = true; } else beta = bt; }
            else beta = 0.0;
            if (!stop) { last_rho = prev->rho; rho = rho_new; }
        }
    }
    if (writer) {
        PcgState s = *prev;
        s.rho = rho; s.last_rho = last_rho; s.beta = beta; s.xbr = xbr; s.xr = xr; s.d2xx = d2xx; s.Q0 = Q0; s.Q1 = Q1; s.it = it; s.done = done; s.pq = 0.0;
        *next = s;
        publish(done);
    }
    if (stop) return;
    const float betaf = (float)beta; const bool first = it == 0;
    if (rim_wg) {
        const RimLists& rl = sa.rim; const unsigned e32 = p2p_pass_epoch(seq, P2P_X_DIR);
        for (int j = (lid - n_main - 1) * PF_THREADS + threadIdx.x; j < rl.n_recv; j += n_rim * PF_THREADS) {
            const int e = rl.recv_idx[j], k = rl.recv_peer[j];
            float zs, za; p2p_get_rim(sa.pd, 0, e32, k, j - rl.recv_off[k], zs, za);
            const size_t ea = (size_t)sa.chunk + e;
            const float ps = first ? zs : zs + betaf * sa.pb[e], pa = first ? za : za + betaf * sa.pb[ea];
            sa.pb[e] = ps; sa.pb[ea] = pa;
            sa.ub[e] = lm_scale(sa.cmb[e]) * ps; sa.ub[ea] = lm_scale(sa.cmb[ea]) * pa;
        }
        return;
    }
    double d2 = 0.0;
    if (!SH || !tail_wg) {
        for (int j = lid * PF_THREADS + threadIdx.x; j < 2 * n4; j += n_main * PF_THREADS) {
            const int i = j < n4 ? j : j - n4 + seg4;
            float4 pi = z4[i]; const float4 cv = C4[i];
            if (!first) { const float4 po = p4[i]; pi.x += betaf * po.x; pi.y += betaf * po.y; pi.z += betaf * po.z; pi.w += betaf * po.w; }
            p4[i] = pi;
            float4 sv, dd; float mi;
            lm_from_colnorm(cv.x, inv_radius, sv.x, dd.x, mi); lm_from_colnorm(cv.y, inv_radius, sv.y, dd.y, mi);
            lm_from_colnorm(cv.z, inv_radius, sv.z, dd.z, mi); lm_from_colnorm(cv.w, inv_radius, sv.w, dd.w, mi);
            u4[i] = make_float4(sv.x * pi.x, sv.y * pi.y, sv.z * pi.z, sv.w * pi.w);
            d2 += (double)dd.x * (double)pi.x * (double)pi.x + (double)dd.y * (double)pi.y * (double)pi.y + (double)dd.z * (double)pi.z * (double)pi.z + (double)dd.w * (double)pi.w * (double)pi.w;
        }
    }
    if (tail_wg) {
        for (int t = threadIdx.x; t < ntail; t += PF_THREADS) {
            const size_t i = tail_rel + t;
            const float pi = first ? z[i] : z[i] + betaf * p[i]; p[i] = pi; u[i] = S[i] * pi;
            d2 += (double)tD2[t] * (double)pi * (double)pi;
        }
    }
    { const double t = block_sum_d(d2); if (threadIdx.x == 0) d2_partials[lid] = t; }
}
template <int SH>
__global__ void __launch_bounds__(PF_THREADS, SH ? 4 : 1) k_pcg_dir3(int init, int n4, int seg4, size_t tail_rel, int ntail, const float* __restrict__ z, float* __restrict__ p,
                                                        const float* __restrict__ S, float* __restrict__ u, const float* __restrict__ D2 ,
                                                        const float* __restrict__ cm, const LmState* __restrict__ lm, const double* __restrict__ step_partials, int n_step, double* __restrict__ d2_partials,
                                                        const PcgState* __restrict__ prev, PcgState* __restrict__ next, int* host_flags, int seq, ShardArgs sa) {
    pcg_dir3_body<SH>(init, n4, seg4, tail_rel, ntail, z, p, S, u, D2 + tail_rel, cm, lm->inv_radius , step_partials, n_step, d2_partials, prev, next, host_flags, seq, sa);
}
template <bool COLL>
__global__ void __launch_bounds__(PF_THREADS, 1) k_pcg_dir3_lad(int init, int n4, int seg4, size_t tail_rel, int ntail, const float* __restrict__ z0, float* __restrict__ p0,
                                                        const float* __restrict__ S, float* __restrict__ u0, const float* __restrict__ tD2_0, const float* __restrict__ cm, const LmState* __restrict__ lm,
                                                        const double* __restrict__ step_partials0, int n_step, double* __restrict__ d2_partials0, PcgState* __restrict__ st2_0 , int prev_parity,
                                                        int* host_flags0, int seq, LadVec lv, int n_slice_partials, const double* __restrict__ red4_0) {
    const int j = lv.sysid[blockIdx.y];
    ShardArgs none; none.n_rim_wg = 0; none.n_slice_partials = n_slice_partials;
    const size_t vo = (size_t)j * lv.vec;
    pcg_dir3_body<COLL ? 2 : 0>(init, n4, seg4, tail_rel, ntail, z0 + vo, p0 + vo, S, u0 + vo, tD2_0 + (size_t)j * lv.tail, cm, lm->lad_inv_radius[j], step_partials0 + (size_t)j * lv.part, n_step,
                                d2_partials0 + (size_t)j * lv.part, st2_0 + 2 * j + prev_parity, st2_0 + 2 * j + (prev_parity ^ 1), host_flags0 + 4 * j, seq, none, COLL ? red4_0 + 4 * j : nullptr);
}

static int dir3_main_wgs(int n_entries, int cap) { int b = (n_entries / 2 + PF_THREADS - 1) / PF_THREADS; b = b < 1 ? 1 : b; return b > cap ? cap : b; }
int launch_pcg_dir3(hipStream_t st, bool init, Seg2 sg, size_t tail_off, int ntail, const float* z, float* p, const float* S, float* u, const float* D2, const float* cm, const LmState* lm,
                    const double* step_partials, int n_step, double* d2_partials, const PcgState* prev, PcgState* next, int* host_flags, int seq, const ShardArgs* sa) {
    const int n4 = sg.n >> 2, seg4 = (int)((sg.off1 - sg.off0) >> 2);
    const size_t o = sg.off0;
    if (!sa) {
        const int blocks = dir3_main_wgs(sg.n, PF_MAX_WG);
        ShardArgs none; std::memset(&none, 0, sizeof(none));
        k_pcg_dir3<0><<<blocks, PF_THREADS, 0, st>>>(init ? 1 : 0, n4, seg4, tail_off - o, ntail, z + o, p + o, S + o, u + o, D2 + o, cm + o, lm, step_partials, n_step, d2_partials, prev, next, host_flags, seq, none);
        return blocks;
    }
    const int cap = sa->pd.wg_cap > 0 ? sa->pd.wg_cap : PF_MAX_WG;
    const int n_main = dir3_main_wgs(sg.n, cap);
    k_pcg_dir3<1><<<sa->n_rim_wg + n_main + 1, PF_THREADS, 0, st>>>(init ? 1 : 0, n4, seg4, tail_off - o, ntail, z + o, p + o, S + o, u + o, D2 + o, cm + o, lm, step_partials, n_step, d2_partials, prev, next,
                                                                       host_flags, seq, *sa);
    return n_main;
}

int launch_pcg_dir3_lad(hipStream_t st, bool init, int nsys, Seg2 sg, size_t tail_off, int ntail, const float* z0, float* p0, const float* S, float* u0, const float* tD2_0, const float* cm, const LmState* lm,
                        const double* step_partials0, int n_step, double* d2_partials0, PcgState* st2_0, int prev_parity, int* host_flags0, int seq, const LadVec& lv,
                        int n_slice_partials, const double* red4_0) {
    const int n4 = sg.n >> 2, seg4 = (int)((sg.off1 - sg.off0) >> 2);
    const size_t o = sg.off0;
    const int blocks = dir3_main_wgs(sg.n, PF_MAX_WG);
    if (red4_0)
        k_pcg_dir3_lad<true><<<dim3(blocks + 1, nsys), PF_THREADS, 0, st>>>(init ? 1 : 0, n4, seg4, tail_off - o, ntail, z0 + o, p0 + o, S + o, u0 + o, tD2_0, cm + o, lm, step_partials0, n_step, d2_partials0,
                                                                            st2_0, prev_parity, host_flags0, seq, lv, n_slice_partials, red4_0);
    else
        k_pcg_dir3_lad<false><<<dim3(blocks, nsys), PF_THREADS, 0, st>>>(init ? 1 : 0, n4, seg4, tail_off - o, ntail, z0 + o, p0 + o, S + o, u0 + o, tD2_0, cm + o, lm, step_partials0, n_step, d2_partials0,
                                                                         st2_0, prev_parity, host_flags0, seq, lv, 0, nullptr);
    return blocks;
}

__global__ void __launch_bounds__(PF_THREADS) k_rim_u(ShardArgs sa, const PcgState* __restrict__ state) {
    if (state->done) return;
    const RimLists& rl = sa.rim; const unsigned e32 = p2p_pass_epoch(sa.seq, P2P_X_RESET_RIM);
    for (int j = blockIdx.x * PF_THREADS + threadIdx.x; j < rl.n_send; j += gridDim.x * PF_THREADS) {
        const int e = rl.send_idx[j], k = rl.send_peer[j];
        p2p_put_rim(sa.pd, 0, e32, k, j - rl.send_off[k], sa.ub[e], sa.ub[(size_t)sa.chunk + e]);
    }
    for (int j = blockIdx.x * PF_THREADS + threadIdx.x; j < rl.n_recv; j += gridDim.x * PF_THREADS) {
        const int e = rl.recv_idx[j], k = rl.recv_peer[j];
        float us, ua; p2p_get_rim(sa.pd, 0, e32, k, j - rl.recv_off[k], us, ua);
        sa.ub[e] = us; sa.ub[(size_t)sa.chunk + e] = ua;
    }
}
void launch_rim_u(hipStream_t st, const ShardArgs& sa, const PcgState* state) { if (sa.rim.n_send > 0 || sa.rim.n_recv > 0) k_rim_u<<<sa.n_rim_wg > 0 ? sa.n_rim_wg : 1, PF_THREADS, 0, st>>>(sa, state); }

enum { S3_INIT = 0, S3_NORMAL = 1, S3_XONLY = 2, S3_RESET = 3 };


struct S3Off { size_t v4, vo, qh2, part, cam, mblk, tail; int st, sys; };
struct S3In { float4 as, aa; int4 o; int o4; float4 x[2], p[2], b[2], cm[2], r[2]; };
template <int MODE> static __device__ inline void s3_load(const Step3Args& a, const S3Off& o, int q, S3In& v) {
    const float4* const qacc = a.qacc + o.v4; const float4* const x = a.x + o.v4; const float4* const p = a.p + o.v4; const float4* const r = a.r + o.v4;
    if (MODE == S3_NORMAL || MODE == S3_RESET) {
        v.as = qacc[q]; v.aa = qacc[q + a.chunk4];
        const int e = a.e0 + 4 * q;
        v.o = *reinterpret_cast<const int4*>(a.ext_off + e);
        v.o4 = a.ext_off[e + 4];
    }
#pragma unroll
    for (int seg = 0; seg < 2; ++seg) {
        const int i = q + seg * a.chunk4;
        v.cm[seg] = a.cm[i];
        if (MODE == S3_INIT) v.r[seg] = r[i];
        else {
            v.x[seg] = x[i];
            if (MODE != S3_RESET) v.p[seg] = p[i];
            if (MODE != S3_XONLY) { v.b[seg] = a.b[i]; if (MODE == S3_NORMAL) v.r[seg] = r[i]; }
        }
    }
}

template <int MODE, int SH>
static __device__ __forceinline__ void pcg_step3_body(const Step3Args& a, const S3Off& o) {
    __shared__ double sm[4 * 8];
    __shared__ double smx[SH == 1 ? P2P_MAX_RANKS : 1];
    __shared__ double camv[64];
    __shared__ double camred[8][64];
    __shared__ float rs[64];
    PcgState* const cur = a.cur + o.st;
    float4* const X = a.x + o.v4; float4* const R = a.r + o.v4; float4* const Z = a.z + o.v4;
    const double* const pq_partials = a.pq_partials + o.part; const double* const d2_partials = a.d2_partials + o.part; double* const step_partials = a.step_partials + o.part;
    const float2* const qh = a.qh + o.qh2; const float* const cam_partials = a.cam_partials + o.cam; const float* const Mblk = a.Mblk + o.mblk;
    const float* const tp = a.tp + o.vo; float* const tx = a.tx + o.vo; float* const tr = a.tr + o.vo; float* const tz = a.tz + o.vo; const float* const tD2 = a.tD2 + o.tail;
    const bool slice_wg = (int)blockIdx.x < a.n_slice_wg;
    const int q0 = blockIdx.x * PF_THREADS + threadIdx.x, qstride = a.n_slice_wg * PF_THREADS;
    S3In in;
    __shared__ int done_s;
    if (threadIdx.x == 0) done_s = cur->done;
    __syncthreads();
    if (done_s) return;
    const float inv_radius = o.sys >= 0 ? a.lm->lad_inv_radius[o.sys] : a.lm->inv_radius;
    float alpha = 0.0f;
    if (MODE == S3_NORMAL || MODE == S3_XONLY) {
        double t1[1];
        if (SH == 2) t1[0] = a.redop[(size_t)(o.sys < 0 ? 0 : o.sys) * a.redop_stride + 6 * a.K + 9] + d2_partials[a.n_d2];
        else reduce_partials_all<1>(pq_partials, a.n_pq, t1, sm, d2_partials, a.n_d2);
        if (SH == 1) {
            const unsigned e32 = p2p_pass_epoch(a.sh.seq, P2P_X_STEP);
            if (blockIdx.x == 0 && threadIdx.x == 0) p2p_put_double_all(a.sh.pd, 1, e32, 0, t1[0]);
            p2p_sum_all<1>(a.sh.pd, 1, e32, t1, smx);
            t1[0] += d2_partials[a.n_d2];
        }
        const double pq = t1[0];
        const double al = cur->rho / pq;
        const bool bad = !(pq > 0.0) || isinf(pq) || isinf(al);
        if (blockIdx.x == 0 && threadIdx.x == 0) { cur->pq = pq; if (bad) cur->done = 2; else cur->alpha = al; }
        if (bad) return;
        alpha = (float)al;
    }
    double s0 = 0.0, s1 = 0.0, s2 = 0.0, s3 = 0.0;
    if (slice_wg) {
        for (int q = q0; q < a.nq; q += qstride) {
            s3_load<MODE>(a, o, q, in);
            float accv[2][4];
            if (MODE == S3_NORMAL || MODE == S3_RESET) {
                const float4 as = in.as, aa = in.aa;
                accv[0][0] = as.x; accv[0][1] = as.y; accv[0][2] = as.z; accv[0][3] = as.w; accv[1][0] = aa.x; accv[1][1] = aa.y; accv[1][2] = aa.z; accv[1][3] = aa.w;
                const int ob[5] = {in.o.x, in.o.y, in.o.z, in.o.w, in.o4};
                for (int j0 = ob[0]; j0 < ob[4]; j0 += 8) {
                    int pos[8]; float2 hv[8];
#pragma unroll
                    for (int u = 0; u < 8; ++u) pos[u] = (j0 + u < ob[4]) ? a.ext_pos[j0 + u] : -1;
#pragma unroll
                    for (int u = 0; u < 8; ++u) hv[u] = pos[u] >= 0 ? qh[pos[u]] : make_float2(0.0f, 0.0f);
#pragma unroll
                    for (int u = 0; u < 8; ++u) {
                        const int j = j0 + u;
                        if (j < ob[4]) {
#pragma unroll
                            for (int k = 0; k < 4; ++k) { const bool mine = j >= ob[k] && j < ob[k + 1]; accv[0][k] += mine ? hv[u].x : 0.0f; accv[1][k] += mine ? hv[u].y : 0.0f; }
                        }
                    }
                }
            }
#pragma unroll
            for (int seg = 0; seg < 2; ++seg) {
                const int i = q + seg * a.chunk4;
                float xv[4], rv[4], svv[4], dv[4], mv[4];
                { const float4 cv = in.cm[seg]; lm_from_colnorm(cv.x, inv_radius, svv[0], dv[0], mv[0]); lm_from_colnorm(cv.y, inv_radius, svv[1], dv[1], mv[1]);
                  lm_from_colnorm(cv.z, inv_radius, svv[2], dv[2], mv[2]); lm_from_colnorm(cv.w, inv_radius, svv[3], dv[3], mv[3]); }
                if (MODE == S3_INIT) { const float4 t = in.r[seg]; rv[0] = t.x; rv[1] = t.y; rv[2] = t.z; rv[3] = t.w; }
                else {
                    const float4 xo = in.x[seg];
                    xv[0] = xo.x; xv[1] = xo.y; xv[2] = xo.z; xv[3] = xo.w;
                    float pv[4] = {0.0f, 0.0f, 0.0f, 0.0f};
                    if (MODE != S3_RESET) {
                        const float4 pp = in.p[seg]; pv[0] = pp.x; pv[1] = pp.y; pv[2] = pp.z; pv[3] = pp.w;
#pragma unroll
                        for (int k = 0; k < 4; ++k) xv[k] += alpha * pv[k];
                        X[i] = make_float4(xv[0], xv[1], xv[2], xv[3]);
                    }
                    if (MODE == S3_XONLY) continue;
                    const float4 bb = in.b[seg];
                    const float bv[4] = {bb.x, bb.y, bb.z, bb.w};
                    float qq[4];
#pragma unroll
                    for (int k = 0; k < 4; ++k) qq[k] = svv[k] * accv[seg][k] + dv[k] * (MODE == S3_NORMAL ? pv[k] : xv[k]);
                    if (MODE == S3_NORMAL) { const float4 ro = in.r[seg]; rv[0] = ro.x - alpha * qq[0]; rv[1] = ro.y - alpha * qq[1]; rv[2] = ro.z - alpha * qq[2]; rv[3] = ro.w - alpha * qq[3]; }
                    else { rv[0] = bv[0] - qq[0]; rv[1] = bv[1] - qq[1]; rv[2] = bv[2] - qq[2]; rv[3] = bv[3] - qq[3]; }
                    R[i] = make_float4(rv[0], rv[1], rv[2], rv[3]);
#pragma unroll
                    for (int k = 0; k < 4; ++k) { const double xd = xv[k]; s1 += xd * ((double)bv[k] + (double)rv[k]); s2 += xd * (double)rv[k]; s3 += (double)dv[k] * xd * xd; }
                }
                const float zv[4] = {mv[0] * rv[0], mv[1] * rv[1], mv[2] * rv[2], mv[3] * rv[3]};
                Z[i] = make_float4(zv[0], zv[1], zv[2], zv[3]);
#pragma unroll
                for (int k = 0; k < 4; ++k) s0 += (double)rv[k] * (double)zv[k];
            }
        }
    } else {
        const int K = a.K, tw = (int)blockIdx.x - a.n_slice_wg, n_pose_wg = (K + PF_POSES_PER_WG - 1) / PF_POSES_PER_WG;
        int col0, ncol;
        if (tw < n_pose_wg) { col0 = 6 * PF_POSES_PER_WG * tw; const int c1 = min(6 * K, col0 + 6 * PF_POSES_PER_WG); ncol = c1 - col0; }
        else { col0 = 6 * K; ncol = 9; }
        const int t = threadIdx.x;
        if (MODE == S3_NORMAL || MODE == S3_RESET) {
            const int g = t / 64, c = t % 64;
            double v = 0.0;
            if (SH != 2 && c < ncol) for (int w = g; w < a.n_cam; w += 8) v += (double)cam_partials[(size_t)w * a.cam_stride + col0 + c];
            camred[g][c] = v;
            __syncthreads();
            if (t < ncol) {
                double s = 0.0; for (int gg = 0; gg < 8; ++gg) s += camred[gg][t];
                if (SH == 2) s = a.redop[(size_t)(o.sys < 0 ? 0 : o.sys) * a.redop_stride + col0 + t];
                if (SH == 1) {
                    const unsigned e32 = p2p_pass_epoch(a.sh.seq, MODE == S3_RESET ? P2P_X_RESET_STEP : P2P_X_STEP);
                    p2p_put_double_all(a.sh.pd, 1, e32, 1 + col0 + t, s);
                    s = 0.0; for (int j = 0; j < a.sh.pd.L.world; ++j) s += p2p_get_double(a.sh.pd, 1, e32, j, 1 + col0 + t);
                }
                camv[t] = s;
            }
            __syncthreads();
        }
        if (t < ncol) {
            const int i = col0 + t;
            const bool fixed = i < 6 * K ? a.fix_poses : (i < 6 * K + 4 ? a.fix_intr : a.fix_dist);
            float ri;
            if (MODE == S3_INIT) ri = tr[i];
            else {
                float xi = tx[i];
                if (MODE != S3_RESET) { xi += alpha * tp[i]; tx[i] = xi; }
                if (MODE == S3_XONLY) ri = 0.0f;
                else {
                    const float vv = MODE == S3_NORMAL ? tp[i] : xi;
                    const float qi = a.tS[i] * (fixed ? 0.0f : (float)camv[t]) + tD2[i] * vv;
                    ri = MODE == S3_NORMAL ? tr[i] - alpha * qi : a.tb[i] - qi;
                    tr[i] = ri;
                    const double xd = xi; s1 += xd * ((double)a.tb[i] + (double)ri); s2 += xd * (double)ri; s3 += (double)tD2[i] * xd * xd;
                }
            }
            rs[t] = ri;
        }
        if (MODE == S3_XONLY) return;
        __syncthreads();
        if (t < ncol) {
            const int i = col0 + t;
            int base, n, row; const float* M;
            if (i < 6 * K) { const int f = i / 6; base = 6 * f; n = 6; row = i - base; M = Mblk + 36 * f; }
            else if (i < 6 * K + 4) { base = 6 * K; n = 4; row = i - base; M = Mblk + 36 * K; }
            else { base = 6 * K + 4; n = 5; row = i - base; M = Mblk + 36 * K + 16; }
            float s = 0.0f;
            for (int j = 0; j < n; ++j) s += M[row * n + j] * rs[base - col0 + j];
            tz[i] = s; s0 += (double)rs[t] * (double)s;
        }
    }
    if (MODE == S3_XONLY) return;
    block_partial_d(s0, step_partials, 4, 0); block_partial_d(s1, step_partials, 4, 1); block_partial_d(s2, step_partials, 4, 2); block_partial_d(s3, step_partials, 4, 3);
}
template <int MODE, int SH>
__global__ void __launch_bounds__(PF_THREADS) k_pcg_step3(Step3Args a) { const S3Off o{0, 0, 0, 0, 0, 0, 0, 0, -1}; pcg_step3_body<MODE, SH>(a, o); }
template <int MODE, bool COLL>
__global__ void __launch_bounds__(PF_THREADS) k_pcg_step3_lad(Step3Args a, LadVec lv) {
    const int j = lv.sysid[blockIdx.y];
    const S3Off o{((size_t)j * lv.vec) >> 2, (size_t)j * lv.vec, ((size_t)j * lv.qh) >> 1, (size_t)j * lv.part, (size_t)j * lv.cam, (size_t)j * lv.mblk, (size_t)j * lv.tail, 2 * j, j};
    pcg_step3_body<MODE, COLL ? 2 : 0>(a, o);
}

int pcg_step3_slice_wgs(int n_entries, int cap) { if (cap <= 0 || cap > PF_MAX_WG) cap = PF_MAX_WG; int b = (n_entries / 4 + PF_THREADS - 1) / PF_THREADS; return b < 1 ? 1 : (b > cap ? cap : b); }
int pcg_step3_tail_wgs(int K) { return (K + PF_POSES_PER_WG - 1) / PF_POSES_PER_WG + 1; }

int launch_pcg_step3(hipStream_t st, int mode, Step3Args a) {
    const int blocks = a.n_slice_wg + pcg_step3_tail_wgs(a.K);
#define I3D_S3(M) do { if (a.sharded) k_pcg_step3<M, 1><<<blocks, PF_THREADS, 0, st>>>(a); else k_pcg_step3<M, 0><<<blocks, PF_THREADS, 0, st>>>(a); } while (0)
    switch (mode) {
        case S3_INIT:   I3D_S3(S3_INIT); break;
        case S3_NORMAL: I3D_S3(S3_NORMAL); break;
        case S3_XONLY:  I3D_S3(S3_XONLY); break;
        default:        I3D_S3(S3_RESET); break;
    }
#undef I3D_S3
    return mode == S3_XONLY ? 0 : blocks;
}

int launch_pcg_step3_lad(hipStream_t st, int mode, int nsys, Step3Args a, const LadVec& lv) {
    const int blocks = a.n_slice_wg + pcg_step3_tail_wgs(a.K);
    const dim3 grid(blocks, nsys);
#define I3D_S3L(M) do { if (a.redop) k_pcg_step3_lad<M, true><<<grid, PF_THREADS, 0, st>>>(a, lv); else k_pcg_step3_lad<M, false><<<grid, PF_THREADS, 0, st>>>(a, lv); } while (0)
    switch (mode) {
        case S3_INIT:   I3D_S3L(S3_INIT); break;
        case S3_NORMAL: I3D_S3L(S3_NORMAL); break;
        case S3_XONLY:  I3D_S3L(S3_XONLY); break;
        default:        I3D_S3L(S3_RESET); break;
    }
#undef I3D_S3L
    return mode == S3_XONLY ? 0 : blocks;
}

__global__ void __launch_bounds__(PF_THREADS) k_lad_reduce_step(const double* __restrict__ step_partials0, int n_slice, double* __restrict__ red4_0, LadVec lv) {
    __shared__ double sm[4 * 8];
    const int j = lv.sysid[blockIdx.x];
    double tot[4];
    reduce_partials_all<4>(step_partials0 + (size_t)j * lv.part, n_slice, tot, sm);
    if (threadIdx.x < 4) red4_0[4 * j + threadIdx.x] = threadIdx.x == 0 ? tot[0] : threadIdx.x == 1 ? tot[1] : threadIdx.x == 2 ? tot[2] : tot[3];
}
void launch_lad_reduce_step(hipStream_t st, int nsys, const double* step_partials0, int n_slice, double* red4_0, const LadVec& lv) {
    k_lad_reduce_step<<<nsys, PF_THREADS, 0, st>>>(step_partials0, n_slice, red4_0, lv);
}
__global__ void __launch_bounds__(PF_THREADS) k_lad_reduce_op(const float* __restrict__ cam_partials0, int n_cam, int cam_stride, int NS, const double* __restrict__ pq_partials0, int n_pq,
                                                              const double* __restrict__ d2_partials0, int n_d2, double* __restrict__ redop0, int redop_stride, LadVec lv) {
    __shared__ double sm[8];
    __shared__ double camred[8][64];
    const int j = lv.sysid[blockIdx.y];
    double* const out = redop0 + (size_t)j * redop_stride;
    const int ncw = (NS + 63) / 64;
    if ((int)blockIdx.x < ncw) {
        const int t = threadIdx.x, g = t / 64, c = t % 64, col = (int)blockIdx.x * 64 + c;
        const float* cp = cam_partials0 + (size_t)j * lv.cam;
        double v = 0.0;
        if (col < NS) for (int w = g; w < n_cam; w += 8) v += (double)cp[(size_t)w * cam_stride + col];
        camred[g][c] = v;
        __syncthreads();
        if (t < 64 && col < NS) { double s = 0.0; for (int gg = 0; gg < 8; ++gg) s += camred[gg][t]; out[col] = s; }
    } else {
        double t1[1];
        reduce_partials_all<1>(pq_partials0 + (size_t)j * lv.part, n_pq, t1, sm, d2_partials0 + (size_t)j * lv.part, n_d2);
        if (threadIdx.x == 0) out[NS] = t1[0];
    }
}
void launch_lad_reduce_op(hipStream_t st, int nsys, const float* cam_partials0, int n_cam, int cam_stride, int NS, const double* pq_partials0, int n_pq, const double* d2_partials0, int n_d2,
                          double* redop0, int redop_stride, const LadVec& lv) {
    k_lad_reduce_op<<<dim3((NS + 63) / 64 + 1, nsys), PF_THREADS, 0, st>>>(cam_partials0, n_cam, cam_stride, NS, pq_partials0, n_pq, d2_partials0, n_d2, redop0, redop_stride, lv);
}

__global__ void k_pcg_init_lad(PcgState* st2_all, int B, int fixed_iterations, int max_iterations, const LmState* lm) {
    const int j = threadIdx.x;
    if (j >= B) return;
    const bool over = lm->done != 0 || lm->lad_radius[j] < 1e-32;
    for (int b = 0; b < 2; ++b) {
        PcgState* st = st2_all + 2 * j + b;
        for (int k = 0; k < 4; ++k) st->acc[k] = 0.0;
        st->rho = 0.0; st->last_rho = 1.0; st->pq = 0.0; st->alpha = 0.0; st->beta = 0.0; st->xbr = 0.0; st->xr = 0.0; st->d2xx = 0.0;
        st->Q0 = 0.0; st->Q1 = 0.0; st->it = 0; st->done = (fixed_iterations == 0 || over) ? 1 : 0; st->fixed_iterations = fixed_iterations; st->max_iterations = max_iterations;
    }
}
void launch_pcg_init_lad(hipStream_t st, PcgState* st2_all, int B, int fixed_iterations, int max_iterations, const LmState* lm) { k_pcg_init_lad<<<1, LADDER_MAX, 0, st>>>(st2_all, B, fixed_iterations, max_iterations, lm); }

__global__ void k_ext_offsets(int n, const int* __restrict__ ext_e, int A, int* __restrict__ ext_off) {
    const int e = blockIdx.x * blockDim.x + threadIdx.x;
    if (e > A) return;
    int lo = 0, hi = n;
    while (lo < hi) { const int mid = (lo + hi) >> 1; if (ext_e[mid] < e) lo = mid + 1; else hi = mid; }
    ext_off[e] = lo;
}
void launch_ext_offsets(hipStream_t st, int n, const int* ext_e, int A, int* ext_off) { k_ext_offsets<<<(A + 1 + 255) / 256, 256, 0, st>>>(n, ext_e, A, ext_off); }

}
```

### intrinsic3d_amd/csrc/host/capi.cpp

```cpp
#include <cstdlib>
#include "context.hpp"

using namespace i3d;

extern "C" {

int i3d_optimize(i3d_context* c, const i3d_optimizer_config* cfg, i3d_iteration_stats* stats) {
    if (!c || !cfg) return ctx_fail(c, I3D_ERR_INVALID_ARGUMENT, "i3d_optimize: null argument");
    return optimize(c, *cfg, stats);
}

int i3d_optimize_host(int32_t device_ordinal, const i3d_optimizer_config* cfg, const i3d_grid_view* grid,
                      double* sdf_refined_io, double* albedo_io, int32_t num_frames, int32_t levels, const int32_t* widths,
                      const int32_t* heights, const float* const* lum, const float* const* depth,
                      double* intr_io, double* dist_io, double* poses_io, const double* voxel_sh, i3d_iteration_stats* stats) {
    if (!cfg || !grid || !sdf_refined_io || !albedo_io || !intr_io || !dist_io || !poses_io || !voxel_sh) return I3D_ERR_INVALID_ARGUMENT;
    i3d_context* c = nullptr;
    int rc = i3d_create(device_ordinal, &c); if (rc) return rc;
    i3d_grid_view gv = *grid; gv.sdf_refined = sdf_refined_io; gv.albedo = albedo_io;
    rc = i3d_set_grid(c, &gv);
    if (!rc) rc = i3d_set_frames(c, num_frames, levels, widths, heights, lum, depth, nullptr);
    if (!rc) rc = i3d_set_camera(c, intr_io, dist_io, poses_io);
    if (!rc) rc = i3d_set_voxel_sh(c, voxel_sh);
    if (!rc) rc = i3d_optimize(c, cfg, stats);
// ... 25 lines not shown
    if (!c || !shared) return ctx_fail(c, I3D_ERR_INVALID_ARGUMENT, "i3d_comm_init_sim: bad arguments");
    delete c->comm; c->comm = make_sim_comm((SimShared*)shared, rank); c->assembled = false; c->slots = 0;
    return I3D_OK;
}

int i3d_shard_plan(int32_t A, int32_t world, int32_t rank, const int32_t* anbr, const uint8_t* active, int32_t* chunk, int32_t* own0,
                   int32_t* own1, uint8_t* in_compute_list) {
    if (A < 0 || world < 1 || rank < 0 || rank >= world || !chunk || !own0 || !own1) return I3D_ERR_INVALID_ARGUMENT;
    int ch, o0, o1; shard_range(A, world, rank, ch, o0, o1);
    *chunk = ch; *own0 = o0; *own1 = o1;
    if (in_compute_list && anbr && active)
        for (int a = 0; a < A; ++a) in_compute_list[a] = shard_needs_entry(a, o0, o1, active[a] != 0, anbr, (size_t)A) ? 1 : 0;
    return I3D_OK;
}
int32_t i3d_shard_vec_index(int32_t a, int32_t chunk, int32_t albedo) { return albedo ? vec_alb(a, chunk) : vec_sdf(a, chunk); }
int i3d_shard_need(int32_t A, int32_t world, const int32_t* anbr, const uint8_t* active, uint64_t* need) {
    if (A < 0 || world < 1 || world > 64 || !anbr || !active || !need) return I3D_ERR_INVALID_ARGUMENT;
    int chunk, o0, o1; shard_range(A, world, 0, chunk, o0, o1);
    const int slice = chunk / world;
    for (int a = 0; a < A; ++a) need[a] = 0;
    for (int a = 0; a < A; ++a) {
        if (!active[a]) continue;
        int col[12]; bool interior;
        const unsigned long long ranks = shard_entry_ranks(a, slice, anbr, (size_t)A, col, interior);
        if (interior) continue;
        for (int k = 0; k < world; ++k) if ((ranks >> k) & 1ull) {
            if (a / slice != k) need[a] |= 1ull << k;
            for (int i = 0; i < 12; ++i) if (col[i] >= 0 && col[i] / slice != k) need[col[i]] |= 1ull << k;
        }
    }
    return I3D_OK;
}
int i3d_comm_stats(i3d_context* c, int64_t* halo_calls, int64_t* halo_bytes_sent, int64_t* reduce_calls, int64_t* reduce_bytes, int32_t* halo_entries_send, int32_t* halo_entries_recv,
                   int32_t* ghost_tiles, int32_t* compute_list) {
    if (!c) return I3D_ERR_INVALID_ARGUMENT;
    if (halo_calls) *halo_calls = c->comm ? c->comm->halo_calls : 0; if (halo_bytes_sent) *halo_bytes_sent = c->comm ? c->comm->halo_bytes_sent : 0;
    if (reduce_calls) *reduce_calls = c->comm ? c->comm->reduce_calls : 0; if (reduce_bytes) *reduce_bytes = c->comm ? c->comm->reduce_bytes : 0;
    if (halo_entries_send) *halo_entries_send = c->halo.n_send; if (halo_entries_recv) *halo_entries_recv = c->halo.n_recv;
    if (ghost_tiles) *ghost_tiles = c->n_ghost_tiles; if (compute_list) *compute_list = c->nC;
    return I3D_OK;
}

const char* i3d_comm_transport(i3d_context* c) { return (c && c->comm) ? c->comm->transport : ""; }

int i3d_debug_assemble(i3d_context* c, const i3d_optimizer_config* cfg, int32_t iteration, int32_t* slots_out) {
    if (!c || !cfg) return ctx_fail(c, I3D_ERR_INVALID_ARGUMENT, "i3d_debug_assemble: null argument");
    CTX_HIP(c, hipSetDevice(c->device));
    OptParams p; i3d_iteration_stats st; std::memset(&st, 0, sizeof(st));
    int rc = assemble(c, *cfg, iteration, p, &st);
    if (!rc && slots_out) *slots_out = c->slots;
    return rc;
}

int i3d_debug_flags(i3d_context* c, uint8_t* flags) {
    if (!c || !flags || !c->have_grid) return ctx_fail(c, I3D_ERR_STATE, "i3d_debug_flags: no grid");
    const int N = c->N; std::vector<uint8_t> f(N); std::vector<int> rank(N);
    CTX_HIP(c, hipMemcpy(f.data(), c->flags.p, N, hipMemcpyDeviceToHost));
    CTX_HIP(c, hipMemcpy(rank.data(), c->rank.p, sizeof(int) * (size_t)N, hipMemcpyDeviceToHost));
    for (int s = 0; s < N; ++s) flags[rank[s]] = f[s];
    return I3D_OK;
}

int i3d_debug_eg_rows(i3d_context* c, int32_t* frame, float* weight, float* residual, float* jac) {
    if (!c || !c->assembled) return ctx_fail(c, I3D_ERR_STATE, "i3d_debug_eg_rows: not assembled");
    const int N = c->N, A = c->A, S = c->slots; const size_t Acap = c->Acap;
    const size_t nrow = ((Acap + 63) / 64) * 64 * (size_t)S;
    std::vector<int> rank(N), alist(A > 0 ? A : 1); std::vector<float4> rows(nrow / 64 * ROW_BLOCK_F4); std::vector<float2> wr(nrow); std::vector<uint8_t> nr(Acap);
    CTX_HIP(c, hipMemcpy(rank.data(), c->rank.p, sizeof(int) * (size_t)N, hipMemcpyDeviceToHost));
    if (A > 0) CTX_HIP(c, hipMemcpy(alist.data(), c->alist.p, sizeof(int) * (size_t)A, hipMemcpyDeviceToHost));
    CTX_HIP(c, hipMemcpy(rows.data(), c->rows.p, sizeof(float4) * rows.size(), hipMemcpyDeviceToHost));
    const float2* const jt = reinterpret_cast<const float2*>(rows.data());
    CTX_HIP(c, hipMemcpy(wr.data(), c->row_wr.p, sizeof(float2) * nrow, hipMemcpyDeviceToHost));
    CTX_HIP(c, hipMemcpy(nr.data(), c->nrows.p, Acap, hipMemcpyDeviceToHost));
    for (size_t i = 0; i < (size_t)N * S; ++i) { if (frame) frame[i] = -1; if (weight) weight[i] = 0.0f; if (residual) residual[i] = 0.0f; }
    if (jac) std::memset(jac, 0, sizeof(float) * (size_t)N * S * P_TOTAL);
    const float tw = (float)c->last_params.type_w[0];
    std::vector<uint8_t> afl(Acap); CTX_HIP(c, hipMemcpy(afl.data(), c->aflags.p, Acap, hipMemcpyDeviceToHost));
    for (int a = 0; a < A; ++a) {
        if (!(afl[a] & F_ACTIVE)) continue;
        const int v = rank[alist[a]];
        for (int k = 0; k < (int)nr[a]; ++k) {
            const float2 m = wr[row_scalar_index(a, k, S)];
            if (m.x == 0.0f) continue;
            const size_t o = (size_t)v * S + k;
            if (frame) { int f; std::memcpy(&f, &jt[row_jt_index(a, k, S)].y, sizeof(int)); frame[o] = f & ~ROW_FREE_BIT; }
            if (weight) weight[o] = m.x * tw;
            if (residual) residual[o] = m.y;
            if (jac) {
                const float isw = 1.0f / std::sqrt(m.x);
                for (int q = 0; q < 7; ++q) { const float4 t = rows[row_index(a, k, q, S)]; jac[o * P_TOTAL + 4 * q] = t.x * isw; jac[o * P_TOTAL + 4 * q + 1] = t.y * isw; jac[o * P_TOTAL + 4 * q + 2] = t.z * isw; jac[o * P_TOTAL + 4 * q + 3] = t.w * isw; }
                jac[o * P_TOTAL + 28] = jt[row_jt_index(a, k, S)].x * isw;
            }
        }
    }
    return I3D_OK;
}

int i3d_debug_reg_rows(i3d_context* c, uint8_t* has_er, uint8_t* has_es, float* ea_weight) {
    if (!c || !c->assembled) return ctx_fail(c, I3D_ERR_STATE, "i3d_debug_reg_rows: not assembled");
    const int N = c->N, A = c->A; const size_t Acap = c->Acap;
    std::vector<int> rank(N), alist(A > 0 ? A : 1); std::vector<uint8_t> rf(Acap), afl(Acap); std::vector<float> ew(Acap * 6);
    CTX_HIP(c, hipMemcpy(rank.data(), c->rank.p, sizeof(int) * (size_t)N, hipMemcpyDeviceToHost));
    if (A > 0) CTX_HIP(c, hipMemcpy(alist.data(), c->alist.p, sizeof(int) * (size_t)A, hipMemcpyDeviceToHost));
    CTX_HIP(c, hipMemcpy(rf.data(), c->regflags.p, Acap, hipMemcpyDeviceToHost));
    CTX_HIP(c, hipMemcpy(afl.data(), c->aflags.p, Acap, hipMemcpyDeviceToHost));
    CTX_HIP(c, hipMemcpy(ew.data(), c->ea_w.p, sizeof(float) * Acap * 6, hipMemcpyDeviceToHost));
    for (int v = 0; v < N; ++v) { if (has_er) has_er[v] = 0; if (has_es) has_es[v] = 0; if (ea_weight) for (int d = 0; d < 6; ++d) ea_weight[(size_t)v * 6 + d] = 0.0f; }
    const float tw = (float)c->last_params.type_w[3];
    for (int a = 0; a < A; ++a) {
        if (!(afl[a] & F_ACTIVE)) continue;
        const int v = rank[alist[a]];
        if (has_er) has_er[v] = rf[a] & 1;
        if (has_es) has_es[v] = (rf[a] >> 1) & 1;
        if (ea_weight) for (int d = 0; d < 6; ++d) ea_weight[(size_t)v * 6 + d] = ew[(size_t)d * Acap + a] * tw;
    }
    return I3D_OK;
}

int i3d_debug_neighbors(i3d_context* c, int32_t* nbr) {
    if (!c || !nbr || !c->have_grid) return ctx_fail(c, I3D_ERR_STATE, "i3d_debug_neighbors: no grid");
    const int N = c->N; std::vector<int> rank(N), t((size_t)NUM_NBR * N);
    CTX_HIP(c, hipMemcpy(rank.data(), c->rank.p, sizeof(int) * (size_t)N, hipMemcpyDeviceToHost));
    CTX_HIP(c, hipMemcpy(t.data(), c->nbr.p, sizeof(int) * (size_t)NUM_NBR * N, hipMemcpyDeviceToHost));
    for (int s = 0; s < N; ++s) for (int i = 0; i < NUM_NBR; ++i) { const int n = t[(size_t)i * N + s]; nbr[(size_t)rank[s] * NUM_NBR + i] = n < 0 ? -1 : rank[n]; }
    return I3D_OK;
}

int i3d_debug_normal_eq(i3d_context* c, double* gradient, double* jtj_diag, double* cost) {
    if (!c) return I3D_ERR_INVALID_ARGUMENT;
    return normal_eq_debug(c, gradient, jtj_diag, cost);
}
int i3d_debug_jtj_apply(i3d_context* c, const double* x, double* y) {
    if (!c || !x || !y) return ctx_fail(c, I3D_ERR_INVALID_ARGUMENT, "i3d_debug_jtj_apply: null pointer");
    return jtj_apply_debug(c, x, y);
}
int i3d_debug_counters(i3d_context* c, int64_t* stream_syncs) {
    if (!c) return I3D_ERR_INVALID_ARGUMENT;
    if (stream_syncs) *stream_syncs = (int64_t)c->n_syncs;
    return I3D_OK;
}

int i3d_debug_ladder_stats(i3d_context* c, int64_t* out6) {
    if (!c || !out6) return I3D_ERR_INVALID_ARGUMENT;
    out6[0] = c->lad_batches; out6[1] = c->lad_streams; out6[2] = c->lad_system_passes; out6[3] = c->lad_resyncs; out6[4] = c->lad_wasted; out6[5] = c->ladder_max;
    return I3D_OK;
}
int i3d_debug_ladder_passes(i3d_context* c, int64_t* out8) {
    if (!c || !out8) return I3D_ERR_INVALID_ARGUMENT;
    for (int n = 0; n < 7; ++n) out8[n] = c->lad_pass_live[n];
    out8[7] = c->lad_paired;
    return I3D_OK;
}

int i3d_debug_cull_stats(i3d_context* c, int64_t* pairs, int64_t* culled) {
    if (!c || !pairs || !culled) return I3D_ERR_INVALID_ARGUMENT;
    if (!c->cull_mask.p || c->nC <= 0) return ctx_fail(c, I3D_ERR_STATE, "i3d_debug_cull_stats: nothing assembled");
    const size_t ngroups = ((size_t)c->nC + 63) / 64, ncw = ((size_t)c->K + 31) / 32;
    *pairs = (int64_t)(ngroups * (size_t)c->K);
    if (!c->cull_on) { *culled = -1; return I3D_OK; }
    std::vector<unsigned> m(ngroups * ncw);
    CTX_HIP(c, hipSetDevice(c->device));
    CTX_HIP(c, hipMemcpy(m.data(), c->cull_mask.p, m.size() * sizeof(unsigned), hipMemcpyDeviceToHost));
    int64_t n = 0; for (unsigned w : m) n += __builtin_popcount(w);
    *culled = n;
    return I3D_OK;
}

}
```

### intrinsic3d_amd/csrc/host/context.hpp

```cpp
#pragma once
#include <functional>
#include <string>
#include <vector>
#include <cstring>
#include <cmath>
#include "../device/kernels.hpp"
#include "../device/render_kernels.hpp"
#include "../device/track_kernels.hpp"
#include "../device/query_kernels.hpp"
#include "../device/register_kernels.hpp"
#include "../device/track_sdf_kernels.hpp"
#include "comm.hpp"
#include "../../../include/intrinsic3d_hip.h"

namespace i3d {

template <class T>
struct DevBuf {
    T* p = nullptr; size_t n = 0;
    DevBuf() = default;
    DevBuf(const DevBuf&) = delete; DevBuf& operator=(const DevBuf&) = delete;
    DevBuf(DevBuf&& o) noexcept : p(o.p), n(o.n) { o.p = nullptr; o.n = 0; }
    DevBuf& operator=(DevBuf&& o) noexcept { if (this != &o) { release(); p = o.p; n = o.n; o.p = nullptr; o.n = 0; } return *this; }
    ~DevBuf() { release(); }
    void release() { if (p) (void)hipFree(p); p = nullptr; n = 0; }
    hipError_t alloc(size_t count) {
        if (count <= n && p) return hipSuccess;
        release();
        if (count == 0) return hipSuccess;
        hipError_t e = hipMalloc((void**)&p, count * sizeof(T));
        if (e == hipSuccess) n = count;
        return e;
    }
};

struct TrackBuffers {
    DevBuf<float> pyr, vn, model, lum; DevBuf<double> slab; DevBuf<TrackState> state; DevBuf<RenderStatsDev> rstats;
};

struct TrackModel {
    std::function<int(int code, const std::string& msg)> fail;
    std::function<int(const i3d_track_desc& d, const double*& intr, const double*& dist)> ready;
    std::function<void(const RenderCam& cam, const RenderPlanes& out, RenderStatsDev* stats)> cast;
    std::function<int()> intensity_ready;
};

struct TrackRgbd {
    const float* luminance; double geometric_weight, photo_weight; float max_photo_residual;
    int64_t photo_samples = 0; double photo_rms_initial = 0.0, photo_rms_final = 0.0;
};

int track_frame_run(hipStream_t st, TrackBuffers& b, const TrackModel& m, const char* what, const i3d_track_desc* d, int32_t w, int32_t h, const float* depth,
                    double* pose6_io, i3d_track_stats* stats, TrackRgbd* rgbd = nullptr);
int track_sums_run(hipStream_t st, TrackBuffers& b, const TrackModel& m, const char* what, const i3d_track_desc* d, int32_t w, int32_t h, const float* depth,
                   int32_t level, const double* pose_ref6, const double* pose_cur6, double* sums, int64_t* inliers, TrackRgbd* rgbd = nullptr);

struct QueryModel {
    std::function<int(int code, const std::string& msg)> fail;
    std::function<int()> ready;
    std::function<void(const QueryParams& p, const double* points, const QueryOut& out, QueryRow* rows, QueryRow* total)> launch;
    double voxel_size;
};
int query_run(hipStream_t st, DevBuf<unsigned char>& scratch, const QueryModel& m, const char* what, const i3d_query_desc* d, int64_t n, const double* points,
              double* sdf, float* normal, float* albedo, double* foot, double* distance, uint8_t* status, i3d_query_stats* stats);

void rot_to_aa(const double R[9], double aa[3]);
struct Pose { double R[9], t[3]; };
Pose pose_from_vec6(const double* p6);
void vec6_from_pose(const Pose& P, double* p6);

struct RegisterModel {
    std::function<int(int code, const std::string& msg)> fail;
    std::function<int()> ready;
    std::function<void(const RegisterParams& p, const double* points, const TrackState* state, int check_done, double* slab)> launch;
    double voxel_size;
    int row_cap = REGISTER_MAX_ROWS;
};
int register_run(hipStream_t st, DevBuf<unsigned char>& scratch, const RegisterModel& m, const char* what, const i3d_register_desc* d, int64_t n, const double* points,
                 double* pose6_io, i3d_register_stats* stats, const double* debug_pivot3 = nullptr, double* debug_sums29 = nullptr, int64_t* debug_valid = nullptr);

struct TrackSdfModel {
    std::function<int(int code, const std::string& msg)> fail;
    std::function<int(const i3d_track_sdf_desc& d, const double*& intr, const double*& dist)> ready;
    std::function<void(const TrackSdfParams& p, const float* depth, const TrackState* state, int check_done, double* slab)> launch;
    double voxel_size;
    int row_cap = REGISTER_MAX_ROWS;
};
int track_sdf_run(hipStream_t st, DevBuf<unsigned char>& scratch, const TrackSdfModel& m, const char* what, const i3d_track_sdf_desc* d, int32_t w, int32_t h,
                  const float* depth, double* pose6_io, i3d_track_sdf_stats* stats, const double* debug_pivot3 = nullptr, double* debug_sums29 = nullptr,
                  int64_t* debug_valid = nullptr, int64_t* debug_usable = nullptr);

struct Timing {
    bool on = false;
    unsigned mask = ~0u;
    double ms[I3D_K_COUNT] = {0};
    long long launches[I3D_K_COUNT] = {0};
    std::vector<float> each[I3D_K_COUNT];
    struct Pending { hipEvent_t a, b; int cat; };
    std::vector<Pending> pending;
    std::vector<hipEvent_t> pool;
};

}

struct i3d_context {
    int device = 0;
    hipStream_t stream = nullptr;
    std::string err;

    int N = 0; float voxel_size = 0, truncation = 0;
    i3d::DevBuf<int> cx, cy, cz, rank, nbr, aidx, alist, aflag, ascan;
    i3d::DevBuf<double> sdf0, x_sdf, x_alb, xc_sdf, xc_alb;
    i3d::DevBuf<float> f_sdf, f_alb, weight, sh;
    i3d::DevBuf<uchar4> color;
    i3d::DevBuf<uint8_t> flags;
    i3d::DevBuf<unsigned char> scan_tmp; size_t scan_tmp_bytes = 0;
    i3d::DevBuf<unsigned long long> hkeys; i3d::DevBuf<int> hvals; unsigned int hmask = 0;
    bool have_grid = false, have_sh = false;
    i3d::DevBuf<unsigned> render_bits; i3d::DevBuf<int> render_bounds; int render_lo[3] = {0, 0, 0}, render_dim[3] = {0, 0, 0}; bool render_bricks_ok = false;
    i3d::DevBuf<float> render_planes; i3d::DevBuf<i3d::RenderStatsDev> render_stats;
    i3d::TrackBuffers track;
    i3d::DevBuf<unsigned char> query_scratch;
    i3d::DevBuf<unsigned char> register_scratch; int register_row_cap = i3d::REGISTER_MAX_ROWS;
    i3d::DevBuf<unsigned char> track_sdf_scratch;
    i3d::DevBuf<unsigned char> track_sdf_batch_scratch; int track_batch_frames = 0;
    std::vector<unsigned long long> sv_keys; std::vector<double> sv_sh; float sv_size = 0.0f; bool have_subvolumes = false;

    int K = 0, levels = 0;
    std::vector<int> fw, fh;
    std::vector<i3d::DevBuf<float>> lum, depth;
    std::vector<i3d::DevBuf<uint8_t>> bgr;
    i3d::DevBuf<i3d::FrameConst> d_frames, d_frames_cand;
    bool have_frames = false;

    double intr[4] = {0, 0, 0, 0}, dist[5] = {0, 0, 0, 0, 0};
    std::vector<double> poses;
    bool have_camera = false;

    int Acap = 0, slots = 0, A = 0; long long n_active = 0;
    i3d::Comm* comm = nullptr; int chunk = 1, own0 = 0, own1 = 0, nC = 0;
    i3d::DevBuf<int> clist, cflag, cscan;
    i3d::HaloPlan halo; i3d::DevBuf<unsigned long long> need_mask, halo_items, halo_sorted; i3d::DevBuf<int> halo_count, halo_send_idx, halo_recv_idx, halo_send_peer, halo_recv_peer, halo_offs, tile_flag, ghost_tiles;
    i3d::DevBuf<float> halo_send_buf, halo_recv_buf; i3d::DevBuf<unsigned char> halo_temp; int n_ghost_tiles = 0, slice = 0;
    i3d::DevBuf<int> obs_frame, anbr; i3d::DevBuf<float> obs_w, ea_w, C, treg;
    i3d::DevBuf<float4> rows; i3d::DevBuf<float2> row_wr;
    i3d::DevBuf<uint8_t> aflags, nrows, regflags, ea_free; i3d::DevBuf<int> gmax;
    i3d::DevBuf<float2> cull_blocks; i3d::DevBuf<float4> cull_bounds; i3d::DevBuf<unsigned> cull_mask; int cull_level = -1; bool cull_on = false;
    double cost_at_build = 0.0;
    i3d::DevBuf<float> C2, treg2, gc_part;
    i3d::DevBuf<float> aux_part;
    i3d::DevBuf<unsigned> tp_lnbr; i3d::DevBuf<int> tp_halo_idx, tp_halo_cnt, tp_iota, tp_ext_e, tp_ext_pos, tp_ext_off, tp_overflow; i3d::DevBuf<float> tp_qh, tp_eaw, cam_part;
    i3d::DevBuf<unsigned char> tp_temp; bool tile_ok = false;
    i3d::DevBuf<unsigned short> tp_hp_off, tp_hp_src; bool halo_pull = false;
    bool ladder_lists = false;
    bool mr1_serial = false;
    int ladder_max = 1;
    int ladder_hint = 0, ladder_hint_prev = 0;
    i3d::LadVec lad{};
    i3d::DevBuf<float> lad_vec;
    i3d::DevBuf<float> lad_qh, lad_cam, lad_mblk, lad_tail;
    i3d::DevBuf<double> lad_part;
    i3d::DevBuf<double> lad_red;
    i3d::DevBuf<i3d::PcgState> lad_st;
    long long lad_batches = 0, lad_streams = 0, lad_system_passes = 0, lad_resyncs = 0, lad_wasted = 0;
    long long lad_pass_live[7] = {0, 0, 0, 0, 0, 0, 0}, lad_paired = 0;
    double t_add_end = 0.0;
    bool deterministic = false;
    int tile_T = 0;
    int plan_T() const { return tile_T > 0 ? tile_T : i3d::tile_plan_T(); }
    i3d::TilePlan tile_plan() const {
        const int T = plan_T();
        const bool sh = comm && (comm->world > 1 || comm->force);
        const int t0 = sh ? own0 / T : 0, t1 = sh ? (own1 + T - 1) / T : i3d::tile_plan_tiles_of(A, T);
        return i3d::TilePlan{tp_lnbr.p, tp_eaw.p, tp_halo_idx.p, tp_halo_cnt.p, tp_iota.p, tp_ext_e.p, tp_ext_pos.p, tp_qh.p, tp_ext_off.p, tp_overflow.p, T, i3d::tile_plan_hmax_of(T), t0, t1 > t0 ? t1 - t0 : 0,
                             ghost_tiles.p, sh ? n_ghost_tiles : 0, deterministic ? 1 : 0, (halo_pull || ladder_lists) ? tp_hp_off.p : nullptr, (halo_pull || ladder_lists) ? tp_hp_src.p : nullptr, halo_pull ? 1 : 0};
    }

    i3d::DevBuf<float> v_mask, v_c, v_S, v_cm, v_D2, v_Minv, v_b, v_x, v_r, v_p, v_z, v_q, v_u, v_acc, v_tmp, v_qacc;
    i3d::DevBuf<float> Minv_blocks;
    i3d::DevBuf<double> d_shared, d_blocks, d_scal, d_xshared, d_xcshared;
    i3d::DevBuf<i3d::PcgState> d_pcg, d_pcg2; i3d::DevBuf<double> d_partials; i3d::PcgState* h_pcg = nullptr; hipEvent_t pcg_ev[2] = {nullptr, nullptr};
    int* h_flags = nullptr; int* d_flags = nullptr; int pcg_seq = 1024;
    i3d::DevBuf<i3d::LmState> d_lm; i3d::LmRecord* h_lmrec = nullptr; i3d::LmRecord* d_lmrec = nullptr; int lm_seq = 1;
    i3d::DevBuf<double> d_cam_c, d_cam_H;
    hipEvent_t ev_asm[2] = {nullptr, nullptr};
    long long n_syncs = 0;
    double* h_pinned = nullptr; size_t h_pinned_n = 0;

    i3d::OptParams last_params; bool assembled = false;
    long long last_sizes[6] = {0, 0, 0, 0, 0, 0};
    i3d::Timing timing;

    i3d::GridView grid_view() const;
    i3d::RowView row_view() const;
};

namespace i3d {

int ctx_fail(i3d_context* c, int code, const std::string& msg);
int ctx_hip(i3d_context* c, hipError_t e, const char* what);
int ctx_launch_check(i3d_context* c);
#define CTX_HIP(c, expr) do { hipError_t _e = (expr); if (_e != hipSuccess) return i3d::ctx_hip((c), _e, #expr); } while (0)
void build_frame_consts(const i3d_context* c, int level, const double* poses, std::vector<FrameConst>& out);
int ensure_pinned(i3d_context* c, size_t n);
bool timing_begin(i3d_context* c, int cat);
void timing_end(i3d_context* c);
void timing_flush(i3d_context* c);
struct TimedScope { i3d_context* c; bool active; TimedScope(i3d_context* c_, int cat) : c(c_), active(timing_begin(c_, cat)) {} ~TimedScope() { if (active) timing_end(c); } };

struct GridStaging { DevBuf<int> kxyz; DevBuf<double> sdf, sdf_ref, alb; DevBuf<float> w; DevBuf<uint8_t> rgb; };
int set_grid_device(i3d_context* c, int N, float voxel_size, float truncation, GridStaging& st);

int render_ensure_bricks(i3d_context* c);
RenderGrid render_grid(const i3d_context* c, bool refined);
void render_cam_pose(RenderCam& cam, const double* pose6, const double* dist5, float min_depth, float max_depth);

int recompute_colors(i3d_context* c, float occlusion_distance, int num_observations);
int clear_outside_thin_shell(i3d_context* c, double thres_shell, int64_t* new_count);
int upsample_grid(i3d_context* c, int64_t* new_count);

int assemble(i3d_context* c, const i3d_optimizer_config& cfg, int iteration, OptParams& p, i3d_iteration_stats* st);
int optimize(i3d_context* c, const i3d_optimizer_config& cfg, i3d_iteration_stats* stats);
int normal_eq_debug(i3d_context* c, double* gradient, double* jtj_diag, double* cost);
int jtj_apply_debug(i3d_context* c, const double* x, double* y);

int estimate_sh(i3d_context* c, float subvolume_size, double lambda_reg, double thres_shell, int* num_subvolumes, double* sh,
                int32_t* sub_index, int cap, i3d_sh_stats* stats);

}
```

### intrinsic3d_amd/csrc/host/solver.cpp

```cpp
#include "context.hpp"
#include <rocprim/rocprim.hpp>
#include <chrono>
#include <limits>
#include <algorithm>

namespace i3d {

#ifdef I3D_MR_PHASES
void mr_phase_report_now();
#endif
#ifdef I3D_MR_BLOCKTIME
void mr_blocktime_report_now();
#endif

static double now_s() { return std::chrono::duration<double>(std::chrono::steady_clock::now().time_since_epoch()).count(); }

static OptParams make_params(const i3d_context* c, const i3d_optimizer_config& cfg, const double* intr, const double* dist) {
    OptParams p; std::memset(&p, 0, sizeof(p));
    p.thres_shell = cfg.thres_shell; p.lambda_a = cfg.lambda_a; p.K = c->K; p.level = cfg.rgbd_level;
    p.pyr_scale = 1.0 / std::pow(2.0, cfg.rgbd_level);
    p.occlusion = cfg.occlusion_distance;
    p.use_er = (cfg.lambda_r0 > 0.0 && cfg.lambda_r1 > 0.0); p.use_es = (cfg.lambda_s0 > 0.0 && cfg.lambda_s1 > 0.0); p.use_ea = cfg.lambda_a > 0.0;
    for (int i = 0; i < 4; ++i) { p.intr[i] = intr[i]; p.cam_f[i] = (float)(intr[i] * p.pyr_scale); }
    bool dz = true;
// ... 378 lines not shown
    { TimedScope t(c, I3D_K_VECTOR); launch_fill(s, (int)L.NP, c->v_x.p, 0.0f); launch_pcg_init(s, st, cfg.pcg_fixed_iterations, 500, c->d_lm.p); }
    CTX_HIP(c, hipMemcpyAsync(c->v_r.p, c->v_b.p, sizeof(float) * L.NP, hipMemcpyDeviceToDevice, s));
    double* const step_part = c->d_partials.p; double* const pq_part = c->d_partials.p + 4 * 2048; double* const d2_part = pq_part + 1024;
    int n_pq = 0, n_step = 0, n_d2 = 0;
    P2PDev pd; std::memset(&pd, 0, sizeof(pd));
    const bool fused = multi && tiled && c->comm->device_reduce(&pd) && L.NS + 1 <= pd.L.red_cap;
    if (!fused) pd.on = 0;
    auto rows_apply = [&](const float* v, float* out, bool with_dot, bool zero_first) -> int {
        if (zero_first) CTX_HIP(c, hipMemsetAsync(c->d_shared.p, 0, sizeof(double) * ((size_t)L.NS + 1), s));
        if (multi) { int rc = push_halo(c, c->v_u.p); if (rc) return rc; }
        if (tiled) {
            { TimedScope t(c, I3D_K_EG_PASS);
              n_pq = launch_eg_tile(s, r, p, c->v_u.p, c->tile_plan(), c->d_shared.p, c->v_qacc.p, with_dot ? pq_part : nullptr, st); }
            { TimedScope t(c, I3D_K_GATHER); launch_halo_fold(s, r, c->tile_plan(), c->v_qacc.p, st); }
            if (!with_dot) n_pq = 0;
            if (!multi || (fused && with_dot)) return I3D_OK;
            if (with_dot) { TimedScope t(c, I3D_K_VECTOR); launch_reduce_partials(s, pq_part, n_pq, 1, pq_slot, st); launch_reduce_partials(s, d2_part, n_d2, 1, pq_slot, st); }
            n_pq = 0;
            return allreduce(c, c->d_shared.p, (size_t)L.NS + 1);
        }
        { TimedScope t(c, I3D_K_EG_PASS); launch_eg_pass(s, PASS_JTJP, g, r, p, c->v_u.p, pb, st); }
        { TimedScope t(c, I3D_K_GATHER); n_pq = launch_gather_tail(s, r, pb, out, c->v_S.p, c->v_D2.p, v, with_dot ? pq_part : nullptr, false, st); }
        if (!with_dot) n_pq = 0;
        return I3D_OK;
    };
    auto fold_step = [&]() { if (multi && !fused) { launch_reduce_partials(s, step_part, n_step, 4, st->acc, st); n_step = 0; } };
    const float* const Sq = tiled ? c->v_S.p : nullptr;
    { TimedScope t(c, I3D_K_VECTOR);
      n_step = launch_pcg_step(s, 0 , own, c->v_p.p, c->v_q.p, c->v_x.p, c->v_r.p, c->v_b.p, c->v_D2.p, c->v_Minv.p, c->v_z.p, nullptr, step_part, st);
      fold_step(); }
    int tail_mode = 0;
    const int seq0 = c->pcg_seq;
    int it = 1;
    for (;; ++it) {
        if (multi && !fused) { int rc = allreduce(c, st->acc, 4); if (rc) return rc; }
        if (fused) { c->comm->count_reduce(4); c->comm->count_reduce((size_t)L.NS + 1); }
        { TimedScope t(c, I3D_K_VECTOR);
          launch_pcg_tail_a(s, tail_mode, to, K, c->Minv_blocks.p, c->v_p.p, tail_mode == 3 ? c->v_tmp.p : c->v_q.p, c->v_x.p, c->v_r.p, c->v_b.p, c->v_D2.p, c->v_z.p,
                            step_part, n_step, st, c->d_shared.p, L.NS + 1, c->d_flags, seq0 + it, pd); }
        { TimedScope t(c, I3D_K_VECTOR);
          n_d2 = launch_pcg_direction(s, own, to, L.NS, c->v_z.p, c->v_p.p, c->v_S.p, c->v_u.p, c->v_D2.p, tiled ? d2_part : nullptr, st); }
        { int rc = rows_apply(c->v_p.p, c->v_q.p, true, false); if (rc) return rc; }
        { TimedScope t(c, I3D_K_VECTOR); launch_pcg_tail_b(s, to, K, p, c->d_shared.p, pq_slot, pq_part, n_pq, d2_part, (tiled && (!multi || fused)) ? n_d2 : 0, tiled,
                                                           c->v_q.p, c->v_S.p, c->v_D2.p, c->v_p.p, st, pd); }
        const bool reset = (it % 10 == 0);
        if (!reset) {
            TimedScope t(c, I3D_K_VECTOR);
            n_step = launch_pcg_step(s, 1, own, c->v_p.p, tiled ? c->v_qacc.p : c->v_q.p, c->v_x.p, c->v_r.p, c->v_b.p, c->v_D2.p, c->v_Minv.p, c->v_z.p, Sq, step_part, st);
            fold_step();
            tail_mode = 1;
        } else {
            { TimedScope t(c, I3D_K_VECTOR);
              launch_pcg_step(s, 2, own, c->v_p.p, c->v_q.p, c->v_x.p, c->v_r.p, c->v_b.p, c->v_D2.p, c->v_Minv.p, c->v_z.p, nullptr, step_part, st);
              launch_pcg_tail_x(s, to, K, c->v_p.p, c->v_x.p, st);
              launch_mul2(s, own, c->v_S.p, c->v_x.p, c->v_u.p); launch_mul(s, L.NS, c->v_S.p + to, c->v_x.p + to, c->v_u.p + to); }
            { int rc = rows_apply(c->v_x.p, c->v_tmp.p, false, true); if (rc) return rc; }
            { TimedScope t(c, I3D_K_VECTOR);
              launch_shared_finalize(s, to, K, p, c->d_shared.p, c->v_tmp.p, true, c->v_S.p, c->v_D2.p, c->v_x.p, nullptr, st);
              n_step = launch_pcg_step(s, 3, own, c->v_p.p, tiled ? c->v_qacc.p : c->v_tmp.p, c->v_x.p, c->v_r.p, c->v_b.p, c->v_D2.p, c->v_Minv.p, c->v_z.p, Sq, step_part, st);
              fold_step(); }
            tail_mode = 3;
        }
        if (it >= 2) {
            const int want = seq0 + it - 1; volatile int* ring = c->h_flags + 2 * (want & 1);
            const double t_wait = now_s();
            while (__atomic_load_n((int*)&ring[0], __ATOMIC_ACQUIRE) != want) {
                if (now_s() - t_wait > 30.0) { CTX_HIP(c, sync_stream(c)); if (__atomic_load_n((int*)&ring[0], __ATOMIC_ACQUIRE) != want) return ctx_fail(c, I3D_ERR_HIP, "pcg_solve: the device stopped publishing its state"); }
            }
            if (__atomic_load_n((int*)&ring[1], __ATOMIC_ACQUIRE)) break;
        }
        if (it > 520) break;
    }
    c->pcg_seq = seq0 + PCG_SEQ_STRIDE;
    *final_state = st;
    return I3D_OK;
}

static int pcg_solve_fused(i3d_context* c, const i3d_optimizer_config& cfg, const OptParams& p, const PcgState** final_state) {
    hipStream_t s = c->stream;
    const Layout L = layout_of(c);
    const int K = c->K; const size_t to = L.tail_off; const Seg2 own = L.own;
    RowView r = c->row_view(); TilePlan tp = c->tile_plan();
    const bool sh = sharded(c);
    ShardArgs sa; std::memset(&sa, 0, sizeof(sa));
    if (sh) {
        if (!c->comm->fused_exchange(&sa.pd) || L.NS + 2 > sa.pd.L.red_cap) return ctx_fail(c, I3D_ERR_STATE, "pcg_solve_fused: the in-kernel exchanges are not available");
        const HaloPlan& h = c->halo;
        sa.rim = RimLists{h.n_send, h.n_recv, c->halo_send_idx.p, c->halo_send_peer.p, c->halo_recv_idx.p, c->halo_recv_peer.p, c->halo_offs.p, c->halo_offs.p + P2P_MAX_RANKS};
        sa.n_rim_wg = (h.n_send + h.n_recv) > 0 ? std::max(1, std::min(4, (std::max(h.n_send, h.n_recv) + 1023) / 1024)) : 1;
        sa.zb = c->v_z.p; sa.pb = c->v_p.p; sa.ub = c->v_u.p; sa.cmb = c->v_cm.p; sa.chunk = c->chunk;
    }
    const int wg_cap = sh ? sa.pd.wg_cap : 0;
    PcgState* const st2 = c->d_pcg2.p;
    const int NSP = (L.NS + 3) & ~3;
    double* const step_part = c->d_partials.p; double* const pq_part = c->d_partials.p + 4 * 2048; double* const d2_part = pq_part + 2048;
    { TimedScope t(c, I3D_K_VECTOR); launch_fill(s, (int)L.NP, c->v_x.p, 0.0f); launch_pcg_init3(s, st2, cfg.pcg_fixed_iterations, 500, c->d_lm.p); }
    CTX_HIP(c, hipMemcpyAsync(c->v_r.p, c->v_b.p, sizeof(float) * L.NP, hipMemcpyDeviceToDevice, s));
    Step3Args a; std::memset(&a, 0, sizeof(a));
    auto c4 = [&](const float* v) { return reinterpret_cast<const float4*>(v + own.off0); };
    auto m4 = [&](float* v) { return reinterpret_cast<float4*>(v + own.off0); };
    a.nq = own.n >> 2; a.chunk4 = (int)((own.off1 - own.off0) >> 2);
    a.p = c4(c->v_p.p); a.qacc = c4(c->v_qacc.p); a.x = m4(c->v_x.p); a.r = m4(c->v_r.p); a.b = c4(c->v_b.p); a.z = m4(c->v_z.p); a.cm = c4(c->v_cm.p); a.lm = c->d_lm.p;
    a.ext_off = tp.ext_off; a.ext_pos = tp.ext_pos; a.qh = reinterpret_cast<const float2*>(tp.qh); a.e0 = (int)own.off0;
    a.pq_partials = pq_part; a.d2_partials = d2_part; a.n_pq = 0; a.n_d2 = 0;
    a.n_slice_wg = pcg_step3_slice_wgs(own.n, wg_cap);
    a.sharded = sh ? 1 : 0;
    a.K = K; a.fix_poses = p.fix_poses; a.fix_intr = p.fix_intr; a.fix_dist = p.fix_dist; a.lad_sys = -1;
    a.cam_partials = c->cam_part.p; a.n_cam = 0; a.cam_stride = NSP; a.Mblk = c->Minv_blocks.p;
    a.tp = c->v_p.p + to; a.tx = c->v_x.p + to; a.tr = c->v_r.p + to; a.tb = c->v_b.p + to; a.tD2 = c->v_D2.p + to; a.tz = c->v_z.p + to; a.tS = c->v_S.p + to;
    a.step_partials = step_part;
    int n_step = 0;
    { TimedScope t(c, I3D_K_VECTOR); a.cur = st2; n_step = launch_pcg_step3(s, 0 , a); }
    const bool mr1 = c->mr1_serial && !sh && tp.T == 512 && tp.hp_off != nullptr && r.slots == 5;
    auto op = [&](double* pq, const PcgState* cur) -> int {
        if (mr1) { const int sys0[3] = {0, 0, 0}; LadVec z; std::memset(&z, 0, sizeof(z));
                   return launch_eg_tile_mr(s, r, p, tp, 1, sys0, c->v_u.p, c->v_qacc.p, tp.qh, pq, c->cam_part.p, NSP, cur, z); }
        return launch_eg_tile(s, r, p, c->v_u.p, tp, nullptr, c->v_qacc.p, pq, cur, c->cam_part.p, NSP);
    };
    const int seq0 = c->pcg_seq;
    int it = 1;
    for (;; ++it) {
        PcgState* const prev = st2 + ((it + 1) & 1); PcgState* const cur = st2 + (it & 1);
        sa.seq = seq0 + it; sa.n_slice_partials = a.n_slice_wg; a.sh = sa;
        { TimedScope t(c, I3D_K_VECTOR);
          a.n_d2 = launch_pcg_dir3(s, it == 1, own, to, L.NS, c->v_z.p, c->v_p.p, c->v_S.p, c->v_u.p, c->v_D2.p, c->v_cm.p, c->d_lm.p, step_part, n_step, d2_part, prev, cur, c->d_flags, seq0 + it,
                                   sh ? &sa : nullptr); }
        if (sh) { c->comm->count_reduce(4); c->comm->count_halo(c->halo.n_send); c->comm->count_reduce((size_t)L.NS + 1); }
        { TimedScope t(c, I3D_K_EG_PASS); a.n_pq = op(pq_part, cur); a.n_cam = a.n_pq; }
        a.cur = cur;
        if (it % 10 != 0) { TimedScope t(c, I3D_K_VECTOR); n_step = launch_pcg_step3(s, 1, a); }
        else {
            { TimedScope t(c, I3D_K_VECTOR); launch_pcg_step3(s, 2, a);
              launch_mul2(s, own, c->v_S.p, c->v_x.p, c->v_u.p); launch_mul(s, L.NS, c->v_S.p + to, c->v_x.p + to, c->v_u.p + to); }
            if (sh) { TimedScope t(c, I3D_K_COMM); launch_rim_u(s, sa, cur); c->comm->count_halo(c->halo.n_send); }
            { TimedScope t(c, I3D_K_EG_PASS); a.n_cam = op(nullptr, cur); }
            { TimedScope t(c, I3D_K_VECTOR); n_step = launch_pcg_step3(s, 3, a); }
        }
        if (it >= 2) {
            const int want = seq0 + it - 1; volatile int* ring = c->h_flags + 2 * (want & 1);
            const double t_wait = now_s();
            while (__atomic_load_n((int*)&ring[0], __ATOMIC_ACQUIRE) != want) {
                if (now_s() - t_wait > 30.0) { CTX_HIP(c, sync_stream(c)); if (__atomic_load_n((int*)&ring[0], __ATOMIC_ACQUIRE) != want) return ctx_fail(c, I3D_ERR_HIP, "pcg_solve: the device stopped publishing its state"); }
            }
            if (__atomic_load_n((int*)&ring[1], __ATOMIC_ACQUIRE)) break;
        }
        if (it > 520) break;
    }
    c->pcg_seq = seq0 + PCG_SEQ_STRIDE;
    *final_state = st2 + (it & 1);
    { const int lrc = ctx_launch_check(c); if (lrc) return lrc; }
    return I3D_OK;
}

constexpr int LAD_PART_STEP = 4 * 2048, LAD_PART_PQ = 2048, LAD_PART_D2 = 2048;
static size_t lad_redop_stride(int NS) { return ((size_t)NS + 1 + 3) & ~(size_t)3; }
static int alloc_ladder(i3d_context* c) {
    const Layout L = layout_of(c);
    const int nsys = c->ladder_max;
    LadVec& lv = c->lad;
    const size_t vec = ((size_t)L.NP + 65535) & ~(size_t)65535;
    const size_t qh = 2 * (size_t)tile_plan_tiles_of((int)std::min((size_t)c->Acap, ((size_t)c->chunk + 65535) & ~(size_t)65535), 512) * (size_t)tile_plan_hmax_of(512);
    const size_t cam = (size_t)2048 * (((size_t)L.NS + 3) & ~(size_t)3);
    lv.vec = vec; lv.qh = qh; lv.cam = cam; lv.part = LAD_PART_STEP + LAD_PART_PQ + LAD_PART_D2; lv.mblk = ((size_t)36 * c->K + 41 + 3) & ~(size_t)3; lv.tail = ((size_t)L.NS + 3) & ~(size_t)3;
    const bool fresh = c->lad_vec.n < (size_t)6 * nsys * vec || !c->lad_vec.p;
    bool ok = c->lad_vec.alloc((size_t)6 * nsys * vec) == hipSuccess;
    if (ok && fresh) ok = hipMemsetAsync(c->lad_vec.p, 0, sizeof(float) * c->lad_vec.n, c->stream) == hipSuccess;
    ok = ok && c->lad_qh.alloc((size_t)nsys * qh) == hipSuccess && c->lad_cam.alloc((size_t)nsys * cam) == hipSuccess && c->lad_part.alloc((size_t)nsys * lv.part) == hipSuccess
            && c->lad_mblk.alloc((size_t)nsys * lv.mblk) == hipSuccess && c->lad_tail.alloc((size_t)nsys * lv.tail) == hipSuccess && c->lad_st.alloc((size_t)2 * LADDER_MAX) == hipSuccess;
    if (ok && sharded(c)) {
        const size_t n = (size_t)LADDER_MAX * (4 + lad_redop_stride(L.NS));
        const bool fresh_r = c->lad_red.n < n || !c->lad_red.p;
        ok = c->lad_red.alloc(n) == hipSuccess;
        if (ok && fresh_r) ok = hipMemsetAsync(c->lad_red.p, 0, sizeof(double) * c->lad_red.n, c->stream) == hipSuccess;
    }
    if (!ok) {
        (void)hipGetLastError();
        c->lad_vec.release(); c->lad_qh.release(); c->lad_cam.release(); c->lad_part.release();
        std::fprintf(stderr, "[i3d] the slabs of the damping ladder (%d systems x %.1f MB) do not fit the device: this outer iteration runs the serial trust-region loop\n", nsys,
                     (double)(6 * vec + qh + cam) * 4.0 / 1e6);
        return 1;
    }
    return I3D_OK;
}
enum { LV_X = 0, LV_R, LV_P, LV_Z, LV_U, LV_Q };
static float* lad_vecp(const i3d_context* c, int kind, int sys = 0) { return c->lad_vec.p + ((size_t)kind * c->ladder_max + sys) * c->lad.vec; }

static int pcg_solve_ladder(i3d_context* c, const i3d_optimizer_config& cfg, const OptParams& p, int B, const PcgState** finals, int* passes_out) {
    hipStream_t s = c->stream;
    const Layout L = layout_of(c);
    const int K = c->K; const size_t to = L.tail_off; const Seg2 own = L.own;
    RowView r = c->row_view(); TilePlan tp = c->tile_plan();
    LadVec lv = c->lad;
    float* const X0 = lad_vecp(c, LV_X); float* const R0 = lad_vecp(c, LV_R); float* const P0 = lad_vecp(c, LV_P); float* const Z0 = lad_vecp(c, LV_Z);
    float* const U0 = lad_vecp(c, LV_U); float* const Q0 = lad_vecp(c, LV_Q);
    PcgState* const st2 = c->lad_st.p;
    const int NSP = (L.NS + 3) & ~3;
    double* const step_part0 = c->lad_part.p; double* const pq_part0 = step_part0 + LAD_PART_STEP; double* const d2_part0 = pq_part0 + LAD_PART_PQ;
    const bool use_mr = [] { const char* e = std::getenv("I3D_LADDER_MR"); return !(e && e[0] == '0'); }();
    const bool mr1 = [] { const char* e = std::getenv("I3D_LADDER_MR1"); return e && e[0] == '1'; }();
    const int group_cap = [] { const char* e = std::getenv("I3D_LADDER_GROUP"); const int v = e ? std::atoi(e) : 3; return v < 1 ? 1 : (v > 3 ? 3 : v); }();
    const int mr_cap = std::min(group_cap, eg_tile_mr_max_systems(K));
    const bool pair = [] { const char* e = std::getenv("I3D_LADDER_PAIR"); return !(e && e[0] == '0'); }();
    const bool mr_ok = use_mr && mr_cap >= 1 && tp.T == 512 && tp.hp_off != nullptr && r.slots == 5;
    const bool sh = sharded(c);
    double* const red4 = sh ? c->lad_red.p : nullptr;
    const int rstride = (int)lad_redop_stride(L.NS);
    double* const redop = sh ? c->lad_red.p + (size_t)LADDER_MAX * 4 : nullptr;
    { TimedScope t(c, I3D_K_VECTOR);
      for (int j = 0; j < B; ++j) { CTX_HIP(c, hipMemsetAsync(X0 + (size_t)j * lv.vec, 0, sizeof(float) * L.NP, s));
                                    CTX_HIP(c, hipMemcpyAsync(R0 + (size_t)j * lv.vec, c->v_b.p, sizeof(float) * L.NP, hipMemcpyDeviceToDevice, s)); }
      launch_pcg_init_lad(s, st2, B, cfg.pcg_fixed_iterations, 500, c->d_lm.p); }
    Step3Args a; std::memset(&a, 0, sizeof(a));
    auto c4 = [&](const float* v) { return reinterpret_cast<const float4*>(v + own.off0); };
    auto m4 = [&](float* v) { return reinterpret_cast<float4*>(v + own.off0); };
    a.nq = own.n >> 2; a.chunk4 = (int)((own.off1 - own.off0) >> 2);
    a.p = c4(P0); a.qacc = c4(Q0); a.x = m4(X0); a.r = m4(R0); a.b = c4(c->v_b.p); a.z = m4(Z0); a.cm = c4(c->v_cm.p); a.lm = c->d_lm.p;
    a.ext_off = tp.ext_off; a.ext_pos = tp.ext_pos; a.qh = reinterpret_cast<const float2*>(c->lad_qh.p); a.e0 = (int)own.off0;
    a.pq_partials = pq_part0; a.d2_partials = d2_part0; a.n_pq = 0; a.n_d2 = 0;
    a.n_slice_wg = pcg_step3_slice_wgs(own.n, 0);
    a.sharded = 0; a.lad_sys = 0; a.redop = redop; a.redop_stride = rstride;
    a.K = K; a.fix_poses = p.fix_poses; a.fix_intr = p.fix_intr; a.fix_dist = p.fix_dist;
    a.cam_partials = c->lad_cam.p; a.n_cam = 0; a.cam_stride = NSP; a.Mblk = c->lad_mblk.p;
    a.tp = P0 + to; a.tx = X0 + to; a.tr = R0 + to; a.tb = c->v_b.p + to; a.tD2 = c->lad_tail.p; a.tz = Z0 + to; a.tS = c->v_S.p + to;
    a.step_partials = step_part0;
    std::vector<int> live(B); for (int j = 0; j < B; ++j) live[j] = j;
    auto set_slots = [&]() { for (int q = 0; q < LADDER_MAX; ++q) lv.sysid[q] = live[q < (int)live.size() ? q : (int)live.size() - 1]; };
    auto rows_apply = [&](int parity, bool with_dot) -> int {
        int n = 0; const int nl = (int)live.size();
        if (sh) { TimedScope t(c, I3D_K_COMM);
                  if (c->comm->push_halo_multi(U0, lv.vec, live.data(), nl, c->halo, s)) return -1; }
        if (mr_ok && (nl > 1 || mr1 || sh)) {
            const int groups = (nl + mr_cap - 1) / mr_cap;
            int at = 0;
            if (groups == 2 && pair && !sh && nl - (nl + 1) / 2 >= 2) {
                const int na = (nl + 1) / 2;
                TimedScope t(c, na == 2 ? I3D_K_EG_MR2 : I3D_K_EG_MR3);
                n = launch_eg_tile_mr_pair(s, r, p, tp, na, nl - na, live.data(), U0, Q0, c->lad_qh.p, with_dot ? pq_part0 : nullptr, c->lad_cam.p, NSP, st2 + parity, lv);
                if (n > 0) { at = nl; ++c->lad_streams; ++c->lad_paired; }
            }
            for (int g = 0; g < groups && at < nl; ++g) {
                const int ng = (nl - at + (groups - g) - 1) / (groups - g);
                TimedScope t(c, ng == 1 ? I3D_K_EG_PASS : (ng == 2 ? I3D_K_EG_MR2 : I3D_K_EG_MR3));
                n = launch_eg_tile_mr(s, r, p, tp, ng, live.data() + at, U0, Q0, c->lad_qh.p, with_dot ? pq_part0 : nullptr, c->lad_cam.p, NSP, st2 + parity, lv);
                if (n <= 0) return -1;
                at += ng; ++c->lad_streams;
            }
        } else {
            for (int j : live) {
                TilePlan tj = tp; tj.qh = c->lad_qh.p + (size_t)j * lv.qh;
                TimedScope t(c, I3D_K_EG_PASS);
                n = launch_eg_tile(s, r, p, U0 + (size_t)j * lv.vec, tj, nullptr, Q0 + (size_t)j * lv.vec, with_dot ? pq_part0 + (size_t)j * lv.part : nullptr, st2 + 2 * j + parity,
                                   c->lad_cam.p + (size_t)j * lv.cam, NSP);
                ++c->lad_streams;
            }
        }
        c->lad_system_passes += nl; ++c->lad_pass_live[nl < 6 ? nl : 6];
        if (sh) {
            { TimedScope t(c, I3D_K_VECTOR); launch_lad_reduce_op(s, nl, c->lad_cam.p, n, NSP, L.NS, pq_part0, with_dot ? n : 0, d2_part0, with_dot ? a.n_d2 : 0, redop, rstride, lv); }
            if (allreduce(c, redop, (size_t)LADDER_MAX * rstride)) return -1;
        }
        return n;
    };
    auto step_sums = [&](int nl, int n_slice) -> int {
        if (!sh) return I3D_OK;
        { TimedScope t(c, I3D_K_VECTOR); launch_lad_reduce_step(s, nl, step_part0, n_slice, red4, lv); }
        return allreduce(c, red4, (size_t)LADDER_MAX * 4);
    };
    int n_step = 0;
    set_slots();
    { TimedScope t(c, I3D_K_VECTOR); a.cur = st2; n_step = launch_pcg_step3_lad(s, 0 , B, a, lv); }
    const int seq0 = c->pcg_seq;
    for (int j = 0; j < B; ++j) finals[j] = st2 + 2 * j;
    int it = 1;
    for (;; ++it) {
        set_slots();
        const int nl = (int)live.size();
        { const int rc = step_sums(nl, a.n_slice_wg); if (rc) return rc; }
        { TimedScope t(c, I3D_K_VECTOR);
          a.n_d2 = launch_pcg_dir3_lad(s, it == 1, nl, own, to, L.NS, Z0, P0, c->v_S.p, U0, c->lad_tail.p, c->v_cm.p, c->d_lm.p, step_part0, n_step, d2_part0, st2, (it + 1) & 1, c->d_flags, seq0 + it, lv,
                                       a.n_slice_wg, red4); }
        { const int n = rows_apply(it & 1, true); if (n < 0) return ctx_fail(c, I3D_ERR_STATE, "pcg_solve_ladder: the multi-system operator pass could not be launched"); a.n_pq = n; a.n_cam = n; }
        a.cur = st2 + (it & 1);
        if (it % 10 != 0) { TimedScope t(c, I3D_K_VECTOR); n_step = launch_pcg_step3_lad(s, 1, nl, a, lv); }
        else {
            { TimedScope t(c, I3D_K_VECTOR); launch_pcg_step3_lad(s, 2, nl, a, lv);
              for (int j : live) { float* xj = X0 + (size_t)j * lv.vec; float* uj = U0 + (size_t)j * lv.vec;
                                   launch_mul2(s, own, c->v_S.p, xj, uj); launch_mul(s, L.NS, c->v_S.p + to, xj + to, uj + to); } }
            { const int n = rows_apply(it & 1, false); if (n < 0) return ctx_fail(c, I3D_ERR_STATE, "pcg_solve_ladder: the multi-system operator pass could not be launched"); a.n_cam = n; }
            { TimedScope t(c, I3D_K_VECTOR); n_step = launch_pcg_step3_lad(s, 3, nl, a, lv); }
        }
        {
            const int want = seq0 + it;
            std::vector<int> still;
            for (int j : live) {
                volatile int* ring = c->h_flags + 4 * j + 2 * (want & 1);
                const double t_wait = now_s();
                while (__atomic_load_n((int*)&ring[0], __ATOMIC_ACQUIRE) != want) {
                    if (now_s() - t_wait > 30.0) { CTX_HIP(c, sync_stream(c)); if (__atomic_load_n((int*)&ring[0], __ATOMIC_ACQUIRE) != want) return ctx_fail(c, I3D_ERR_HIP, "pcg_solve_ladder: the device stopped publishing its state"); }
                }
                if (!__atomic_load_n((int*)&ring[1], __ATOMIC_ACQUIRE)) still.push_back(j);
                else finals[j] = st2 + 2 * j + (it & 1);
            }
            live.swap(still);
            if (live.empty()) break;
        }
        if (it > 520) break;
    }
    if (passes_out) *passes_out = it;
    c->pcg_seq = seq0 + PCG_SEQ_STRIDE;
    for (int j : live) finals[j] = st2 + 2 * j + (it & 1);
    { const int lrc = ctx_launch_check(c); if (lrc) return lrc; }
    return I3D_OK;
}

static int wait_record(i3d_context* c, int idx, int seq, LmRecord& out) {
    LmRecord* const r = c->h_lmrec + idx;
    const double t0 = now_s();
    while (__atomic_load_n(&r->seq, __ATOMIC_ACQUIRE) != seq) {
        if (now_s() - t0 > 60.0) {
            CTX_HIP(c, sync_stream(c));
            if (__atomic_load_n(&r->seq, __ATOMIC_ACQUIRE) != seq) return ctx_fail(c, I3D_ERR_HIP, "lm_solve: the device stopped publishing the state of the trust-region loop");
        }
    }
    out = *r;
    return I3D_OK;
}

static int lm_solve(i3d_context* c, const i3d_optimizer_config& cfg, OptParams& p, i3d_iteration_stats* st, double initial_radius) {
    hipStream_t s = c->stream;
    const Layout L = layout_of(c);
    const int N = c->N, K = c->K, NP = (int)L.NP, NS = L.NS;
    GridView g = c->grid_view(); RowView r = c->row_view();
    if (cfg.lm_steps > LM_REC_SLOTS - 2) return ctx_fail(c, I3D_ERR_CAPACITY, "optimize: more than 62 LM steps per outer iteration");
    { TimedScope t(c, I3D_K_VECTOR); launch_freemask(s, r, p, c->v_mask.p); }
    CTX_HIP(c, hipMemcpyAsync(c->xc_sdf.p, c->x_sdf.p, sizeof(double) * (size_t)N, hipMemcpyDeviceToDevice, s));
    CTX_HIP(c, hipMemcpyAsync(c->xc_alb.p, c->x_alb.p, sizeof(double) * (size_t)N, hipMemcpyDeviceToDevice, s));
    const bool one_stream = one_stream_gradcol(c);
    auto after_colnorm = [&]() -> int {
        CTX_HIP(c, hipMemcpyAsync(c->d_cam_c.p, c->d_shared.p, sizeof(double) * (size_t)NS, hipMemcpyDeviceToDevice, s));
        CTX_HIP(c, hipMemcpyAsync(c->d_cam_H.p, c->d_blocks.p, sizeof(double) * ((size_t)21 * K + 25), hipMemcpyDeviceToDevice, s));
        { int rc2 = allgather(c, c->v_c.p); if (rc2) return rc2; }
        { TimedScope t(c, I3D_K_VECTOR); launch_scale_from_colnorm(s, NP, c->v_c.p, c->v_mask.p, c->v_S.p, c->v_cm.p); }
        return I3D_OK;
    };
    int rc = I3D_OK;
    if (one_stream) { rc = run_gradcol(c, p, after_colnorm); if (rc) return rc; }
    else {
        rc = run_pass(c, PASS_COLNORM, p, nullptr, c->v_c.p); if (rc) return rc;
        rc = after_colnorm(); if (rc) return rc;
        rc = run_pass(c, PASS_GRAD, p, nullptr, c->v_acc.p); if (rc) return rc;
    }
    { TimedScope t(c, I3D_K_VECTOR); launch_mul(s, NP, c->v_S.p, c->v_acc.p, c->v_b.p); }
    if (env_off("I3D_COST0")) { rc = eval_cost_launch(c, p, false, c->d_frames.p); if (rc) return rc; }
    else if (!one_stream) { TimedScope t(c, I3D_K_VECTOR); launch_set_double(s, c->d_scal.p + 16, c->cost_at_build); }
    rc = count_above_dev(c, c->v_acc.p, c->v_mask.p, 1e-10f, c->d_scal.p + 8); if (rc) return rc;
    rc = dot_dev(c, c->v_mask.p, c->v_mask.p, c->d_scal.p + 9); if (rc) return rc;
    {
        double* xs = c->h_pinned;
        for (int i = 0; i < 6 * K; ++i) xs[i] = c->poses[i];
        for (int i = 0; i < 4; ++i) xs[6 * K + i] = c->intr[i];
        for (int i = 0; i < 5; ++i) xs[6 * K + 4 + i] = c->dist[i];
        CTX_HIP(c, hipMemcpyAsync(c->d_xshared.p, xs, sizeof(double) * NS, hipMemcpyHostToDevice, s));
    }
    const int seq0 = c->lm_seq; c->lm_seq += LM_REC_SLOTS;
    LmState* const lm = c->d_lm.p;
    launch_lm_init(s, lm, c->d_scal.p + 16, c->d_scal.p + 8, c->d_scal.p + 9, initial_radius, c->d_lmrec, seq0);

    static const bool legacy = [] { const char* e = std::getenv("I3D_PCG_LEGACY"); return e && e[0] == '1'; }();
    bool fused = c->tile_ok && !legacy;
    if (fused && sharded(c)) { P2PDev probe; fused = c->comm->fused_exchange(&probe) && L.NS + 2 <= probe.L.red_cap; }
    int attempts = 0; bool ended = false, accepted = false;
    auto consume = [&](const LmRecord& rec) {
        if (rec.kind == 0) {
            if (st) { st->cost_initial = rec.cost; st->cost_final = rec.cost; st->free_parameters = (int64_t)(rec.nfree + 0.5); st->termination = rec.final_ ? 1 : 0; st->final_radius = initial_radius; }
            c->last_sizes[5] = (long long)(rec.nfree + 0.5);
        } else if (rec.kind == 2) { if (st) st->termination = 1; }
        else {
            if (st) {
                st->lm_iterations = attempts + 1;
                if (attempts < 50) { st->pcg_iterations[attempts] = rec.pcg_it; st->step_accepted[attempts] = rec.accepted; }
                st->final_radius = rec.radius_after; st->termination = rec.termination;
                if (rec.accepted) { st->cost_final = rec.cost; st->successful_steps += 1; }
            }
            if (cfg.verbose) std::printf("  [i3d LM] it %d cand %.9e model %.3e rho %.4f radius -> %.3e cg %d%s\n", attempts + 1, rec.cand_cost, rec.model_change, rec.rel, rec.radius_after, rec.pcg_it,
                                         rec.accepted ? " accepted" : "");
            accepted = rec.accepted != 0;
            ++attempts;
        }
        if (rec.final_) ended = true;
    };
    const int dbg_invalid = [] { const char* e = std::getenv("I3D_DEBUG_INVALID_ATTEMPT"); return e ? std::atoi(e) : -1; }();
    bool ladder = c->ladder_max > 1 && c->tile_ok && !legacy && (sharded(c) ? !fused : fused) && c->plan_T() == 512 && c->tile_plan().hp_off != nullptr && c->slots == 5;
    if (ladder && alloc_ladder(c) != I3D_OK) {
        ladder = false;
    }
    if (ladder) {
        const LadVec& lv = c->lad;
        { LmRecord rec; rc = wait_record(c, 0, seq0, rec); if (rc) return rc; consume(rec); }
        const bool warm = c->ladder_hint > 0;
        int k = 0, prevB = 0; bool after_resync = false;
        while (k < cfg.lm_steps && !ended) {
            int B = after_resync ? 1 : (prevB == 0 ? (warm ? std::max(c->ladder_hint, c->ladder_hint_prev) : 2) : (warm ? 2 : 2 * prevB));
            B = std::max(1, std::min(B, std::min(c->ladder_max, cfg.lm_steps - k)));
            after_resync = false; prevB = B;
            { TimedScope t(c, I3D_K_VECTOR);
              launch_lm_begin_lad(s, lm, B, K, p.fix_poses, p.fix_intr, p.fix_dist, c->d_cam_c.p, c->d_cam_H.p, c->lad_mblk.p, lv.mblk, c->v_c.p + L.tail_off, c->v_S.p + L.tail_off, c->lad_tail.p, lv.tail,
                                  c->d_lmrec + 1 + k, seq0 + 1 + k); }
            const PcgState* fin[LADDER_MAX] = {nullptr};
            rc = pcg_solve_ladder(c, cfg, p, B, fin, nullptr); if (rc) return rc;
            ++c->lad_batches;
            for (int j = 0; j < B && sharded(c); ++j) { rc = allgather(c, lad_vecp(c, LV_X, j)); if (rc) return rc; }
            for (int j = 0; j < B; ++j) {
                { TimedScope t(c, I3D_K_VECTOR);
                  launch_candidate(s, g, r, K, -1.0f, lad_vecp(c, LV_X, j), c->v_S.p, c->d_xshared.p, c->xc_sdf.p, c->xc_alb.p, c->d_xcshared.p, c->d_scal.p + 4, c->v_mask.p, c->d_partials.p, lm);
                  launch_cand_frames(s, K, c->d_xcshared.p, c->d_frames.p, c->d_frames_cand.p, lm); }
                rc = eval_cost_launch(c, p, true, c->d_frames_cand.p, c->d_xcshared.p + 6 * K, lm); if (rc) return rc;
                { TimedScope t(c, I3D_K_VECTOR);
                  launch_lm_decide(s, lm, fin[j], c->d_scal.p + 4, c->d_scal.p + 16, k + j, cfg.lm_steps, c->d_lmrec + 1 + k + j, seq0 + 1 + k + j, j + 1, dbg_invalid == k + j ? 1 : 0);
                  launch_accept(s, g, r, c->xc_sdf.p, c->xc_alb.p, lm); }
            }
            int decided = 0;
            for (int j = 0; j < B && !ended; ++j) {
                LmRecord rec; rc = wait_record(c, 1 + k + j, seq0 + 1 + k + j, rec); if (rc) return rc;
                if (rec.kind == 3) {
                    __atomic_store_n(&c->h_lmrec[1 + k + j].seq, 0, __ATOMIC_RELEASE);
                    ++c->lad_resyncs; after_resync = true; break;
                }
                consume(rec); ++decided;
            }
            if (ended && decided < B) c->lad_wasted += B - decided;
            k += decided;
        }
        if (attempts > 0) { c->ladder_hint_prev = c->ladder_hint; c->ladder_hint = attempts; }
        ended = true;
    }
    int k = 0;
    for (; !ladder && k < cfg.lm_steps; ++k) {
        { TimedScope t(c, I3D_K_VECTOR);
          launch_lm_begin(s, lm, K, p.fix_poses, p.fix_intr, p.fix_dist, c->d_cam_c.p, c->d_cam_H.p, c->Minv_blocks.p, c->v_c.p + L.tail_off, c->v_S.p + L.tail_off, c->v_D2.p + L.tail_off, c->v_Minv.p + L.tail_off,
                          c->d_lmrec + 1 + k, seq0 + 1 + k);
          if (!fused) launch_lm_diag_dev(s, (int)L.tail_off, c->v_c.p, c->v_S.p, lm, c->v_D2.p, c->v_Minv.p); }
        const PcgState* ps = nullptr;
// ... 107 lines not shown
```

Baseline: 43.24.

## Drop ladder z vector by recomputing preconditioned residual, co-locate systems' workgroups

The ladder PCG no longer stores the preconditioned residual z per system. The direction kernel recomputes z from r and the Jacobi inverse, and only the small tail z is kept, in a side buffer. This cuts one full-vector write and read per iteration and shrinks the ladder slab from six vectors to five. A new co-located launch layout interleaves the workgroups of different damping systems in groups of eight on a 1D grid, so systems that share S and cm data run side by side. This adds index arithmetic, a few idle blocks from padding, and recomputed reciprocals.

```diff
diff --git a/include/intrinsic3d_hip.h b/include/intrinsic3d_hip.h
--- a/include/intrinsic3d_hip.h
+++ b/include/intrinsic3d_hip.h
@@ -349,6 +349,7 @@
 int i3d_debug_counters(i3d_context* ctx, int64_t* stream_syncs);
 int i3d_debug_ladder_stats(i3d_context* ctx, int64_t* out6);
 int i3d_debug_ladder_passes(i3d_context* ctx, int64_t* out8);
+int i3d_debug_ladder_vector(i3d_context* ctx, int64_t* out4);
 int i3d_debug_cull_stats(i3d_context* ctx, int64_t* pairs, int64_t* culled);
 
 int i3d_debug_register_sums(i3d_context* ctx, const i3d_register_desc* desc, int64_t n, const double* points, const double* pose6, const double* pivot3,
diff --git a/intrinsic3d_amd/binding.py b/intrinsic3d_amd/binding.py
--- a/intrinsic3d_amd/binding.py
+++ b/intrinsic3d_amd/binding.py
@@ -269,7 +269,7 @@
            "i3d_comm_unique_id", "i3d_comm_init", "i3d_comm_sim_create", "i3d_comm_sim_destroy", "i3d_comm_init_sim", "i3d_shard_plan", "i3d_shard_vec_index",
            "i3d_comm_transport", "i3d_timing_enable", "i3d_timing_select", "i3d_timing_get", "i3d_timing_get_work", "i3d_timing_get_work_ex", "i3d_kernel_name", "i3d_problem_sizes",
            "i3d_debug_assemble", "i3d_debug_map_order", "i3d_debug_flags", "i3d_debug_eg_rows", "i3d_debug_reg_rows", "i3d_debug_neighbors",
-           "i3d_debug_normal_eq", "i3d_debug_jtj_apply", "i3d_debug_counters", "i3d_debug_cull_stats", "i3d_debug_ladder_stats", "i3d_debug_ladder_passes", "i3d_debug_track_sums", "i3d_debug_track_rgbd_sums"]
+           "i3d_debug_normal_eq", "i3d_debug_jtj_apply", "i3d_debug_counters", "i3d_debug_cull_stats", "i3d_debug_ladder_stats", "i3d_debug_ladder_passes", "i3d_debug_ladder_vector", "i3d_debug_track_sums", "i3d_debug_track_rgbd_sums"]
 
 _lib = None
 
@@ -331,6 +331,8 @@
     L.i3d_debug_counters.restype = i32; L.i3d_debug_counters.argtypes = [vp, vp]
     L.i3d_debug_ladder_stats.restype = i32; L.i3d_debug_ladder_stats.argtypes = [vp, vp]
     L.i3d_debug_ladder_passes.restype = i32; L.i3d_debug_ladder_passes.argtypes = [vp, vp]
+    if hasattr(L, "i3d_debug_ladder_vector"):
+        L.i3d_debug_ladder_vector.restype = i32; L.i3d_debug_ladder_vector.argtypes = [vp, vp]
     L.i3d_debug_cull_stats.restype = i32; L.i3d_debug_cull_stats.argtypes = [vp, vp, vp]
     L.i3d_set_grid_from_tsdf_records.restype = i32; L.i3d_set_grid_from_tsdf_records.argtypes = [vp, f32, i64, vp, vp, vp, vp]
     L.i3d_recompute_colors.restype = i32; L.i3d_recompute_colors.argtypes = [vp, f32, i32]
@@ -810,6 +812,11 @@
         self._check(self.L.i3d_debug_ladder_passes(self.h, a), "i3d_debug_ladder_passes")
         return {"live": [int(a[n]) for n in range(7)], "paired": int(a[7])}
 
+    def debug_ladder_vector(self):
+        a = (C.c_int64 * 4)()
+        self._check(self.L.i3d_debug_ladder_vector(self.h, a), "i3d_debug_ladder_vector")
+        return {"step_slice_wgs": int(a[0]), "step_wgs": int(a[1]), "dir_wgs": int(a[2]), "coloc": int(a[3])}
+
     def debug_cull_stats(self):
         a = C.c_int64(0); b = C.c_int64(0)
         self._check(self.L.i3d_debug_cull_stats(self.h, C.byref(a), C.byref(b)), "i3d_debug_cull_stats")
diff --git a/intrinsic3d_amd/csrc/device/kernels.hpp b/intrinsic3d_amd/csrc/device/kernels.hpp
--- a/intrinsic3d_amd/csrc/device/kernels.hpp
+++ b/intrinsic3d_amd/csrc/device/kernels.hpp
@@ -163,10 +163,10 @@
 int  launch_pcg_step3(hipStream_t st, int mode , Step3Args a);
 void launch_halo_fold(hipStream_t st, RowView r, TilePlan t, float* qacc, const PcgState* state);
 void launch_pcg_init_lad(hipStream_t st, PcgState* st2_all , int B, int fixed_iterations, int max_iterations, const LmState* lm);
-int  launch_pcg_dir3_lad(hipStream_t st, bool init, int nsys, Seg2 sg, size_t tail_off, int ntail, const float* z0, float* p0, const float* S, float* u0, const float* tD2_0, const float* cm, const LmState* lm,
+int  launch_pcg_dir3_lad(hipStream_t st, bool init, int nsys, bool coloc, Seg2 sg, size_t tail_off, int ntail, const float* r0, const float* tz0, float* p0, const float* S, float* u0, const float* tD2_0, const float* cm, const LmState* lm,
                          const double* step_partials0, int n_step, double* d2_partials0, PcgState* st2_0, int prev_parity, int* host_flags0, int seq, const LadVec& lv,
                          int n_slice_partials = 0, const double* red4_0 = nullptr );
-int  launch_pcg_step3_lad(hipStream_t st, int mode, int nsys, Step3Args a, const LadVec& lv);
+int  launch_pcg_step3_lad(hipStream_t st, int mode, int nsys, bool coloc, Step3Args a, const LadVec& lv);
 void launch_lad_reduce_step(hipStream_t st, int nsys, const double* step_partials0, int n_slice, double* red4_0, const LadVec& lv);
 void launch_lad_reduce_op(hipStream_t st, int nsys, const float* cam_partials0, int n_cam, int cam_stride, int NS, const double* pq_partials0, int n_pq, const double* d2_partials0, int n_d2,
                           double* redop0, int redop_stride, const LadVec& lv);
diff --git a/intrinsic3d_amd/csrc/device/pcg_fused.hip b/intrinsic3d_amd/csrc/device/pcg_fused.hip
--- a/intrinsic3d_amd/csrc/device/pcg_fused.hip
+++ b/intrinsic3d_amd/csrc/device/pcg_fused.hip
@@ -47,8 +47,8 @@
 
 static __device__ inline void lm_from_colnorm(float cm, float inv_radius, float& s, float& d2, float& minv) { s = lm_scale(cm); lm_diag(cm, s, inv_radius, d2, minv); }
 
-template <int SH>
-static __device__ __forceinline__ void pcg_dir3_body(int init, int n4, int seg4, size_t tail_rel, int ntail, const float* __restrict__ z, float* __restrict__ p,
+template <int SH, bool NOZ = false>
+static __device__ __forceinline__ void pcg_dir3_body(const int wg, const int nwg, int init, int n4, int seg4, size_t tail_rel, int ntail, const float* __restrict__ z, const float* __restrict__ tz, float* __restrict__ p,
                                                         const float* __restrict__ S, float* __restrict__ u, const float* __restrict__ tD2 ,
                                                         const float* __restrict__ cm, const float inv_radius, const double* __restrict__ step_partials, int n_step, double* __restrict__ d2_partials,
                                                         const PcgState* __restrict__ prev, PcgState* __restrict__ next, int* host_flags, int seq, const ShardArgs& sa,
@@ -57,8 +57,8 @@
     __shared__ double smx[SH == 1 ? 4 * P2P_MAX_RANKS : 1];
     auto publish = [&](int done) { if (host_flags) { __hip_atomic_store(&host_flags[2 * (seq & 1) + 1], done, __ATOMIC_RELAXED, __HIP_MEMORY_SCOPE_SYSTEM);
                                                      __hip_atomic_store(&host_flags[2 * (seq & 1)], seq, __ATOMIC_RELEASE, __HIP_MEMORY_SCOPE_SYSTEM); } };
-    const int n_rim = SH == 1 ? sa.n_rim_wg : 0, n_main = SH ? (int)gridDim.x - n_rim - 1 : (int)gridDim.x;
-    const int lid = SH == 1 ? ((int)blockIdx.x < n_rim ? n_main + 1 + (int)blockIdx.x : (int)blockIdx.x - n_rim) : (int)blockIdx.x;
+    const int n_rim = SH == 1 ? sa.n_rim_wg : 0, n_main = SH ? nwg - n_rim - 1 : nwg;
+    const int lid = SH == 1 ? (wg < n_rim ? n_main + 1 + wg : wg - n_rim) : wg;
     const bool rim_wg = SH == 1 && lid > n_main, tail_wg = SH ? lid == n_main : lid == n_main - 1;
     const bool writer = lid == 0 && threadIdx.x == 0;
     const float4* z4 = reinterpret_cast<const float4*>(z); float4* p4 = reinterpret_cast<float4*>(p);
@@ -136,11 +136,27 @@
         for (int j = lid * PF_THREADS + threadIdx.x; j < 2 * n4; j += n_main * PF_THREADS) {
             const int i = j < n4 ? j : j - n4 + seg4;
             float4 pi = z4[i]; const float4 cv = C4[i];
-            if (!first) { const float4 po = p4[i]; pi.x += betaf * po.x; pi.y += betaf * po.y; pi.z += betaf * po.z; pi.w += betaf * po.w; }
-            p4[i] = pi;
-            float4 sv, dd; float mi;
-            lm_from_colnorm(cv.x, inv_radius, sv.x, dd.x, mi); lm_from_colnorm(cv.y, inv_radius, sv.y, dd.y, mi);
-            lm_from_colnorm(cv.z, inv_radius, sv.z, dd.z, mi); lm_from_colnorm(cv.w, inv_radius, sv.w, dd.w, mi);
+            float4 sv, dd;
+            if (NOZ) {
+                float4 mv; float unused;
+                lm_from_colnorm(cv.x, inv_radius, sv.x, dd.x, unused); lm_from_colnorm(cv.y, inv_radius, sv.y, dd.y, unused);
+                lm_from_colnorm(cv.z, inv_radius, sv.z, dd.z, unused); lm_from_colnorm(cv.w, inv_radius, sv.w, dd.w, unused);
+                auto minv_of = [&](float c, float s) -> float {
+                    if (s == 0.0f) return 0.0f;
+                    const float t = __fmul_rn(c, s), cs = __fmul_rn(s, t), cl = fminf(fmaxf(cs, 1e-6f), 1e32f);
+                    return __builtin_amdgcn_rcpf(first ? __fmaf_rn(inv_radius, cl, cs) : __fmaf_rn(s, t, __fmul_rn(cl, inv_radius)));
+                };
+                mv.x = minv_of(cv.x, sv.x); mv.y = minv_of(cv.y, sv.y); mv.z = minv_of(cv.z, sv.z); mv.w = minv_of(cv.w, sv.w);
+                pi = make_float4(__fmul_rn(mv.x, pi.x), __fmul_rn(mv.y, pi.y), __fmul_rn(mv.z, pi.z), __fmul_rn(mv.w, pi.w));
+                if (!first) { const float4 po = p4[i]; pi.x = __fmaf_rn(betaf, po.x, pi.x); pi.y = __fmaf_rn(betaf, po.y, pi.y); pi.z = __fmaf_rn(betaf, po.z, pi.z); pi.w = __fmaf_rn(betaf, po.w, pi.w); }
+                p4[i] = pi;
+            } else {
+                if (!first) { const float4 po = p4[i]; pi.x += betaf * po.x; pi.y += betaf * po.y; pi.z += betaf * po.z; pi.w += betaf * po.w; }
+                p4[i] = pi;
+                float mi;
+                lm_from_colnorm(cv.x, inv_radius, sv.x, dd.x, mi); lm_from_colnorm(cv.y, inv_radius, sv.y, dd.y, mi);
+                lm_from_colnorm(cv.z, inv_radius, sv.z, dd.z, mi); lm_from_colnorm(cv.w, inv_radius, sv.w, dd.w, mi);
+            }
             u4[i] = make_float4(sv.x * pi.x, sv.y * pi.y, sv.z * pi.z, sv.w * pi.w);
             d2 += (double)dd.x * (double)pi.x * (double)pi.x + (double)dd.y * (double)pi.y * (double)pi.y + (double)dd.z * (double)pi.z * (double)pi.z + (double)dd.w * (double)pi.w * (double)pi.w;
         }
@@ -148,7 +164,7 @@
     if (tail_wg) {
         for (int t = threadIdx.x; t < ntail; t += PF_THREADS) {
             const size_t i = tail_rel + t;
-            const float pi = first ? z[i] : z[i] + betaf * p[i]; p[i] = pi; u[i] = S[i] * pi;
+            const float pi = first ? tz[t] : tz[t] + betaf * p[i]; p[i] = pi; u[i] = S[i] * pi;
             d2 += (double)tD2[t] * (double)pi * (double)pi;
         }
     }
@@ -159,17 +175,26 @@
                                                         const float* __restrict__ S, float* __restrict__ u, const float* __restrict__ D2 ,
                                                         const float* __restrict__ cm, const LmState* __restrict__ lm, const double* __restrict__ step_partials, int n_step, double* __restrict__ d2_partials,
                                                         const PcgState* __restrict__ prev, PcgState* __restrict__ next, int* host_flags, int seq, ShardArgs sa) {
-    pcg_dir3_body<SH>(init, n4, seg4, tail_rel, ntail, z, p, S, u, D2 + tail_rel, cm, lm->inv_radius , step_partials, n_step, d2_partials, prev, next, host_flags, seq, sa);
-}
-template <bool COLL>
-__global__ void __launch_bounds__(PF_THREADS, 1) k_pcg_dir3_lad(int init, int n4, int seg4, size_t tail_rel, int ntail, const float* __restrict__ z0, float* __restrict__ p0,
+    pcg_dir3_body<SH>((int)blockIdx.x, (int)gridDim.x, init, n4, seg4, tail_rel, ntail, z, z + tail_rel, p, S, u, D2 + tail_rel, cm, lm->inv_radius , step_partials, n_step, d2_partials, prev, next, host_flags, seq, sa);
+}
+struct LadWg { int slot, wg, nwg; };
+template <bool COLOC> static __device__ __forceinline__ LadWg lad_workgroup(int nsys, int blocks) {
+    if (!COLOC) return LadWg{(int)blockIdx.y, (int)blockIdx.x, (int)gridDim.x};
+    const int id = (int)blockIdx.x;
+    return LadWg{(id >> 3) % nsys, (id / (8 * nsys)) * 8 + (id & 7), blocks};
+}
+static int lad_coloc_grid(int blocks, int nsys) { return ((blocks + 7) / 8) * 8 * nsys; }
+template <bool COLL, bool COLOC>
+__global__ void __launch_bounds__(PF_THREADS, 1) k_pcg_dir3_lad(int nsys, int blocks, int init, int n4, int seg4, size_t tail_rel, int ntail, const float* __restrict__ r0, const float* __restrict__ tz0, float* __restrict__ p0,
                                                         const float* __restrict__ S, float* __restrict__ u0, const float* __restrict__ tD2_0, const float* __restrict__ cm, const LmState* __restrict__ lm,
                                                         const double* __restrict__ step_partials0, int n_step, double* __restrict__ d2_partials0, PcgState* __restrict__ st2_0 , int prev_parity,
                                                         int* host_flags0, int seq, LadVec lv, int n_slice_partials, const double* __restrict__ red4_0) {
-    const int j = lv.sysid[blockIdx.y];
+    const LadWg w = lad_workgroup<COLOC>(nsys, blocks);
+    if (COLOC && w.wg >= blocks) return;
+    const int j = lv.sysid[w.slot];
     ShardArgs none; none.n_rim_wg = 0; none.n_slice_partials = n_slice_partials;
     const size_t vo = (size_t)j * lv.vec;
-    pcg_dir3_body<COLL ? 2 : 0>(init, n4, seg4, tail_rel, ntail, z0 + vo, p0 + vo, S, u0 + vo, tD2_0 + (size_t)j * lv.tail, cm, lm->lad_inv_radius[j], step_partials0 + (size_t)j * lv.part, n_step,
+    pcg_dir3_body<COLL ? 2 : 0, true>(w.wg, w.nwg, init, n4, seg4, tail_rel, ntail, r0 + vo, tz0 + (size_t)j * lv.tail, p0 + vo, S, u0 + vo, tD2_0 + (size_t)j * lv.tail, cm, lm->lad_inv_radius[j], step_partials0 + (size_t)j * lv.part, n_step,
                                 d2_partials0 + (size_t)j * lv.part, st2_0 + 2 * j + prev_parity, st2_0 + 2 * j + (prev_parity ^ 1), host_flags0 + 4 * j, seq, none, COLL ? red4_0 + 4 * j : nullptr);
 }
 
@@ -191,18 +216,21 @@
     return n_main;
 }
 
-int launch_pcg_dir3_lad(hipStream_t st, bool init, int nsys, Seg2 sg, size_t tail_off, int ntail, const float* z0, float* p0, const float* S, float* u0, const float* tD2_0, const float* cm, const LmState* lm,
+int launch_pcg_dir3_lad(hipStream_t st, bool init, int nsys, bool coloc, Seg2 sg, size_t tail_off, int ntail, const float* r0, const float* tz0, float* p0, const float* S, float* u0, const float* tD2_0, const float* cm, const LmState* lm,
                         const double* step_partials0, int n_step, double* d2_partials0, PcgState* st2_0, int prev_parity, int* host_flags0, int seq, const LadVec& lv,
                         int n_slice_partials, const double* red4_0) {
     const int n4 = sg.n >> 2, seg4 = (int)((sg.off1 - sg.off0) >> 2);
     const size_t o = sg.off0;
     const int blocks = dir3_main_wgs(sg.n, PF_MAX_WG);
     if (red4_0)
-        k_pcg_dir3_lad<true><<<dim3(blocks + 1, nsys), PF_THREADS, 0, st>>>(init ? 1 : 0, n4, seg4, tail_off - o, ntail, z0 + o, p0 + o, S + o, u0 + o, tD2_0, cm + o, lm, step_partials0, n_step, d2_partials0,
-                                                                            st2_0, prev_parity, host_flags0, seq, lv, n_slice_partials, red4_0);
+        k_pcg_dir3_lad<true, false><<<dim3(blocks + 1, nsys), PF_THREADS, 0, st>>>(nsys, blocks + 1, init ? 1 : 0, n4, seg4, tail_off - o, ntail, r0 + o, tz0, p0 + o, S + o, u0 + o, tD2_0, cm + o, lm, step_partials0, n_step,
+                                                                                   d2_partials0, st2_0, prev_parity, host_flags0, seq, lv, n_slice_partials, red4_0);
+    else if (coloc)
+        k_pcg_dir3_lad<false, true><<<lad_coloc_grid(blocks, nsys), PF_THREADS, 0, st>>>(nsys, blocks, init ? 1 : 0, n4, seg4, tail_off - o, ntail, r0 + o, tz0, p0 + o, S + o, u0 + o, tD2_0, cm + o, lm, step_partials0, n_step,
+                                                                                         d2_partials0, st2_0, prev_parity, host_flags0, seq, lv, 0, nullptr);
     else
-        k_pcg_dir3_lad<false><<<dim3(blocks, nsys), PF_THREADS, 0, st>>>(init ? 1 : 0, n4, seg4, tail_off - o, ntail, z0 + o, p0 + o, S + o, u0 + o, tD2_0, cm + o, lm, step_partials0, n_step, d2_partials0,
-                                                                         st2_0, prev_parity, host_flags0, seq, lv, 0, nullptr);
+        k_pcg_dir3_lad<false, false><<<dim3(blocks, nsys), PF_THREADS, 0, st>>>(nsys, blocks, init ? 1 : 0, n4, seg4, tail_off - o, ntail, r0 + o, tz0, p0 + o, S + o, u0 + o, tD2_0, cm + o, lm, step_partials0, n_step,
+                                                                                d2_partials0, st2_0, prev_parity, host_flags0, seq, lv, 0, nullptr);
     return blocks;
 }
 
@@ -224,7 +252,7 @@
 enum { S3_INIT = 0, S3_NORMAL = 1, S3_XONLY = 2, S3_RESET = 3 };
 
 
-struct S3Off { size_t v4, vo, qh2, part, cam, mblk, tail; int st, sys; };
+struct S3Off { size_t v4, vo, qh2, part, cam, mblk, tail; int st, sys; int wg;  };
 struct S3In { float4 as, aa; int4 o; int o4; float4 x[2], p[2], b[2], cm[2], r[2]; };
 template <int MODE> static __device__ inline void s3_load(const Step3Args& a, const S3Off& o, int q, S3In& v) {
     const float4* const qacc = a.qacc + o.v4; const float4* const x = a.x + o.v4; const float4* const p = a.p + o.v4; const float4* const r = a.r + o.v4;
@@ -247,7 +275,7 @@
     }
 }
 
-template <int MODE, int SH>
+template <int MODE, int SH, bool NOZ = false>
 static __device__ __forceinline__ void pcg_step3_body(const Step3Args& a, const S3Off& o) {
     __shared__ double sm[4 * 8];
     __shared__ double smx[SH == 1 ? P2P_MAX_RANKS : 1];
@@ -258,9 +286,9 @@
     float4* const X = a.x + o.v4; float4* const R = a.r + o.v4; float4* const Z = a.z + o.v4;
     const double* const pq_partials = a.pq_partials + o.part; const double* const d2_partials = a.d2_partials + o.part; double* const step_partials = a.step_partials + o.part;
     const float2* const qh = a.qh + o.qh2; const float* const cam_partials = a.cam_partials + o.cam; const float* const Mblk = a.Mblk + o.mblk;
-    const float* const tp = a.tp + o.vo; float* const tx = a.tx + o.vo; float* const tr = a.tr + o.vo; float* const tz = a.tz + o.vo; const float* const tD2 = a.tD2 + o.tail;
-    const bool slice_wg = (int)blockIdx.x < a.n_slice_wg;
-    const int q0 = blockIdx.x * PF_THREADS + threadIdx.x, qstride = a.n_slice_wg * PF_THREADS;
+    const float* const tp = a.tp + o.vo; float* const tx = a.tx + o.vo; float* const tr = a.tr + o.vo; float* const tz = a.tz + (NOZ ? o.tail : o.vo); const float* const tD2 = a.tD2 + o.tail;
+    const bool slice_wg = o.wg < a.n_slice_wg;
+    const int q0 = o.wg * PF_THREADS + threadIdx.x, qstride = a.n_slice_wg * PF_THREADS;
     S3In in;
     __shared__ int done_s;
     if (threadIdx.x == 0) done_s = cur->done;
@@ -274,14 +302,14 @@
         else reduce_partials_all<1>(pq_partials, a.n_pq, t1, sm, d2_partials, a.n_d2);
         if (SH == 1) {
             const unsigned e32 = p2p_pass_epoch(a.sh.seq, P2P_X_STEP);
-            if (blockIdx.x == 0 && threadIdx.x == 0) p2p_put_double_all(a.sh.pd, 1, e32, 0, t1[0]);
+            if (o.wg == 0 && threadIdx.x == 0) p2p_put_double_all(a.sh.pd, 1, e32, 0, t1[0]);
             p2p_sum_all<1>(a.sh.pd, 1, e32, t1, smx);
             t1[0] += d2_partials[a.n_d2];
         }
         const double pq = t1[0];
         const double al = cur->rho / pq;
         const bool bad = !(pq > 0.0) || isinf(pq) || isinf(al);
-        if (blockIdx.x == 0 && threadIdx.x == 0) { cur->pq = pq; if (bad) cur->done = 2; else cur->alpha = al; }
+        if (o.wg == 0 && threadIdx.x == 0) { cur->pq = pq; if (bad) cur->done = 2; else cur->alpha = al; }
         if (bad) return;
         alpha = (float)al;
     }
@@ -340,13 +368,13 @@
                     for (int k = 0; k < 4; ++k) { const double xd = xv[k]; s1 += xd * ((double)bv[k] + (double)rv[k]); s2 += xd * (double)rv[k]; s3 += (double)dv[k] * xd * xd; }
                 }
                 const float zv[4] = {mv[0] * rv[0], mv[1] * rv[1], mv[2] * rv[2], mv[3] * rv[3]};
-                Z[i] = make_float4(zv[0], zv[1], zv[2], zv[3]);
+                if (!NOZ) Z[i] = make_float4(zv[0], zv[1], zv[2], zv[3]);
 #pragma unroll
                 for (int k = 0; k < 4; ++k) s0 += (double)rv[k] * (double)zv[k];
             }
         }
     } else {
-        const int K = a.K, tw = (int)blockIdx.x - a.n_slice_wg, n_pose_wg = (K + PF_POSES_PER_WG - 1) / PF_POSES_PER_WG;
+        const int K = a.K, tw = o.wg - a.n_slice_wg, n_pose_wg = (K + PF_POSES_PER_WG - 1) / PF_POSES_PER_WG;
         int col0, ncol;
         if (tw < n_pose_wg) { col0 = 6 * PF_POSES_PER_WG * tw; const int c1 = min(6 * K, col0 + 6 * PF_POSES_PER_WG); ncol = c1 - col0; }
         else { col0 = 6 * K; ncol = 9; }
@@ -402,15 +430,18 @@
         }
     }
     if (MODE == S3_XONLY) return;
-    block_partial_d(s0, step_partials, 4, 0); block_partial_d(s1, step_partials, 4, 1); block_partial_d(s2, step_partials, 4, 2); block_partial_d(s3, step_partials, 4, 3);
+    { const double t0 = block_sum_d(s0), t1 = block_sum_d(s1), t2 = block_sum_d(s2), t3 = block_sum_d(s3);
+      if (threadIdx.x == 0) { double* const sp = step_partials + 4 * (size_t)o.wg; sp[0] = t0; sp[1] = t1; sp[2] = t2; sp[3] = t3; } }
 }
 template <int MODE, int SH>
-__global__ void __launch_bounds__(PF_THREADS) k_pcg_step3(Step3Args a) { const S3Off o{0, 0, 0, 0, 0, 0, 0, 0, -1}; pcg_step3_body<MODE, SH>(a, o); }
-template <int MODE, bool COLL>
-__global__ void __launch_bounds__(PF_THREADS) k_pcg_step3_lad(Step3Args a, LadVec lv) {
-    const int j = lv.sysid[blockIdx.y];
-    const S3Off o{((size_t)j * lv.vec) >> 2, (size_t)j * lv.vec, ((size_t)j * lv.qh) >> 1, (size_t)j * lv.part, (size_t)j * lv.cam, (size_t)j * lv.mblk, (size_t)j * lv.tail, 2 * j, j};
-    pcg_step3_body<MODE, COLL ? 2 : 0>(a, o);
+__global__ void __launch_bounds__(PF_THREADS) k_pcg_step3(Step3Args a) { const S3Off o{0, 0, 0, 0, 0, 0, 0, 0, -1, (int)blockIdx.x}; pcg_step3_body<MODE, SH>(a, o); }
+template <int MODE, bool COLL, bool COLOC>
+__global__ void __launch_bounds__(PF_THREADS) k_pcg_step3_lad(Step3Args a, LadVec lv, int nsys, int blocks) {
+    const LadWg w = lad_workgroup<COLOC>(nsys, blocks);
+    if (COLOC && w.wg >= blocks) return;
+    const int j = lv.sysid[w.slot];
+    const S3Off o{((size_t)j * lv.vec) >> 2, (size_t)j * lv.vec, ((size_t)j * lv.qh) >> 1, (size_t)j * lv.part, (size_t)j * lv.cam, (size_t)j * lv.mblk, (size_t)j * lv.tail, 2 * j, j, w.wg};
+    pcg_step3_body<MODE, COLL ? 2 : 0, true>(a, o);
 }
 
 int pcg_step3_slice_wgs(int n_entries, int cap) { if (cap <= 0 || cap > PF_MAX_WG) cap = PF_MAX_WG; int b = (n_entries / 4 + PF_THREADS - 1) / PF_THREADS; return b < 1 ? 1 : (b > cap ? cap : b); }
@@ -429,10 +460,12 @@
     return mode == S3_XONLY ? 0 : blocks;
 }
 
-int launch_pcg_step3_lad(hipStream_t st, int mode, int nsys, Step3Args a, const LadVec& lv) {
+int launch_pcg_step3_lad(hipStream_t st, int mode, int nsys, bool coloc, Step3Args a, const LadVec& lv) {
     const int blocks = a.n_slice_wg + pcg_step3_tail_wgs(a.K);
     const dim3 grid(blocks, nsys);
-#define I3D_S3L(M) do { if (a.redop) k_pcg_step3_lad<M, true><<<grid, PF_THREADS, 0, st>>>(a, lv); else k_pcg_step3_lad<M, false><<<grid, PF_THREADS, 0, st>>>(a, lv); } while (0)
+#define I3D_S3L(M) do { if (a.redop) k_pcg_step3_lad<M, true, false><<<grid, PF_THREADS, 0, st>>>(a, lv, nsys, blocks); \
+                        else if (coloc) k_pcg_step3_lad<M, false, true><<<lad_coloc_grid(blocks, nsys), PF_THREADS, 0, st>>>(a, lv, nsys, blocks); \
+                        else k_pcg_step3_lad<M, false, false><<<grid, PF_THREADS, 0, st>>>(a, lv, nsys, blocks); } while (0)
     switch (mode) {
         case S3_INIT:   I3D_S3L(S3_INIT); break;
         case S3_NORMAL: I3D_S3L(S3_NORMAL); break;
diff --git a/intrinsic3d_amd/csrc/host/capi.cpp b/intrinsic3d_amd/csrc/host/capi.cpp
--- a/intrinsic3d_amd/csrc/host/capi.cpp
+++ b/intrinsic3d_amd/csrc/host/capi.cpp
@@ -201,6 +201,12 @@
     return I3D_OK;
 }
 
+int i3d_debug_ladder_vector(i3d_context* c, int64_t* out4) {
+    if (!c || !out4) return I3D_ERR_INVALID_ARGUMENT;
+    for (int n = 0; n < 4; ++n) out4[n] = c->lad_vec_wgs[n];
+    return I3D_OK;
+}
+
 int i3d_debug_cull_stats(i3d_context* c, int64_t* pairs, int64_t* culled) {
     if (!c || !pairs || !culled) return I3D_ERR_INVALID_ARGUMENT;
     if (!c->cull_mask.p || c->nC <= 0) return ctx_fail(c, I3D_ERR_STATE, "i3d_debug_cull_stats: nothing assembled");
diff --git a/intrinsic3d_amd/csrc/host/context.hpp b/intrinsic3d_amd/csrc/host/context.hpp
--- a/intrinsic3d_amd/csrc/host/context.hpp
+++ b/intrinsic3d_amd/csrc/host/context.hpp
@@ -163,6 +163,7 @@
     i3d::DevBuf<double> lad_red;
     i3d::DevBuf<i3d::PcgState> lad_st;
     long long lad_batches = 0, lad_streams = 0, lad_system_passes = 0, lad_resyncs = 0, lad_wasted = 0;
+    long long lad_vec_wgs[4] = {0, 0, 0, 0};
     long long lad_pass_live[7] = {0, 0, 0, 0, 0, 0, 0}, lad_paired = 0;
     double t_add_end = 0.0;
     bool deterministic = false;
diff --git a/intrinsic3d_amd/csrc/host/solver.cpp b/intrinsic3d_amd/csrc/host/solver.cpp
--- a/intrinsic3d_amd/csrc/host/solver.cpp
+++ b/intrinsic3d_amd/csrc/host/solver.cpp
@@ -554,6 +554,7 @@
     return I3D_OK;
 }
 
+enum { LV_X = 0, LV_R, LV_P, LV_U, LV_Q, LV_KINDS };
 constexpr int LAD_PART_STEP = 4 * 2048, LAD_PART_PQ = 2048, LAD_PART_D2 = 2048;
 static size_t lad_redop_stride(int NS) { return ((size_t)NS + 1 + 3) & ~(size_t)3; }
 static int alloc_ladder(i3d_context* c) {
@@ -563,9 +564,10 @@
     const size_t vec = ((size_t)L.NP + 65535) & ~(size_t)65535;
     const size_t qh = 2 * (size_t)tile_plan_tiles_of((int)std::min((size_t)c->Acap, ((size_t)c->chunk + 65535) & ~(size_t)65535), 512) * (size_t)tile_plan_hmax_of(512);
     const size_t cam = (size_t)2048 * (((size_t)L.NS + 3) & ~(size_t)3);
-    lv.vec = vec; lv.qh = qh; lv.cam = cam; lv.part = LAD_PART_STEP + LAD_PART_PQ + LAD_PART_D2; lv.mblk = ((size_t)36 * c->K + 41 + 3) & ~(size_t)3; lv.tail = ((size_t)L.NS + 3) & ~(size_t)3;
-    const bool fresh = c->lad_vec.n < (size_t)6 * nsys * vec || !c->lad_vec.p;
-    bool ok = c->lad_vec.alloc((size_t)6 * nsys * vec) == hipSuccess;
+    lv.vec = vec; lv.qh = qh; lv.cam = cam; lv.part = LAD_PART_STEP + LAD_PART_PQ + LAD_PART_D2; lv.mblk = ((size_t)36 * c->K + 41 + 3) & ~(size_t)3; lv.tail = 2 * (((size_t)L.NS + 3) & ~(size_t)3);
+    const size_t kinds = LV_KINDS;
+    const bool fresh = c->lad_vec.n < kinds * nsys * vec || !c->lad_vec.p;
+    bool ok = c->lad_vec.alloc(kinds * nsys * vec) == hipSuccess;
     if (ok && fresh) ok = hipMemsetAsync(c->lad_vec.p, 0, sizeof(float) * c->lad_vec.n, c->stream) == hipSuccess;
     ok = ok && c->lad_qh.alloc((size_t)nsys * qh) == hipSuccess && c->lad_cam.alloc((size_t)nsys * cam) == hipSuccess && c->lad_part.alloc((size_t)nsys * lv.part) == hipSuccess
             && c->lad_mblk.alloc((size_t)nsys * lv.mblk) == hipSuccess && c->lad_tail.alloc((size_t)nsys * lv.tail) == hipSuccess && c->lad_st.alloc((size_t)2 * LADDER_MAX) == hipSuccess;
@@ -579,12 +581,11 @@
         (void)hipGetLastError();
         c->lad_vec.release(); c->lad_qh.release(); c->lad_cam.release(); c->lad_part.release();
         std::fprintf(stderr, "[i3d] the slabs of the damping ladder (%d systems x %.1f MB) do not fit the device: this outer iteration runs the serial trust-region loop\n", nsys,
-                     (double)(6 * vec + qh + cam) * 4.0 / 1e6);
+                     (double)(LV_KINDS * vec + qh + cam) * 4.0 / 1e6);
         return 1;
     }
     return I3D_OK;
 }
-enum { LV_X = 0, LV_R, LV_P, LV_Z, LV_U, LV_Q };
 static float* lad_vecp(const i3d_context* c, int kind, int sys = 0) { return c->lad_vec.p + ((size_t)kind * c->ladder_max + sys) * c->lad.vec; }
 
 static int pcg_solve_ladder(i3d_context* c, const i3d_optimizer_config& cfg, const OptParams& p, int B, const PcgState** finals, int* passes_out) {
@@ -593,7 +594,8 @@
     const int K = c->K; const size_t to = L.tail_off; const Seg2 own = L.own;
     RowView r = c->row_view(); TilePlan tp = c->tile_plan();
     LadVec lv = c->lad;
-    float* const X0 = lad_vecp(c, LV_X); float* const R0 = lad_vecp(c, LV_R); float* const P0 = lad_vecp(c, LV_P); float* const Z0 = lad_vecp(c, LV_Z);
+    float* const X0 = lad_vecp(c, LV_X); float* const R0 = lad_vecp(c, LV_R); float* const P0 = lad_vecp(c, LV_P);
+    float* const TZ0 = c->lad_tail.p + lv.tail / 2;
     float* const U0 = lad_vecp(c, LV_U); float* const Q0 = lad_vecp(c, LV_Q);
     PcgState* const st2 = c->lad_st.p;
     const int NSP = (L.NS + 3) & ~3;
@@ -603,6 +605,7 @@
     const int group_cap = [] { const char* e = std::getenv("I3D_LADDER_GROUP"); const int v = e ? std::atoi(e) : 3; return v < 1 ? 1 : (v > 3 ? 3 : v); }();
     const int mr_cap = std::min(group_cap, eg_tile_mr_max_systems(K));
     const bool pair = [] { const char* e = std::getenv("I3D_LADDER_PAIR"); return !(e && e[0] == '0'); }();
+    const bool coloc = [] { const char* e = std::getenv("I3D_LADDER_VEC_COLOC"); return !(e && e[0] == '0'); }() && !sharded(c);
     const bool mr_ok = use_mr && mr_cap >= 1 && tp.T == 512 && tp.hp_off != nullptr && r.slots == 5;
     const bool sh = sharded(c);
     double* const red4 = sh ? c->lad_red.p : nullptr;
@@ -616,14 +619,14 @@
     auto c4 = [&](const float* v) { return reinterpret_cast<const float4*>(v + own.off0); };
     auto m4 = [&](float* v) { return reinterpret_cast<float4*>(v + own.off0); };
     a.nq = own.n >> 2; a.chunk4 = (int)((own.off1 - own.off0) >> 2);
-    a.p = c4(P0); a.qacc = c4(Q0); a.x = m4(X0); a.r = m4(R0); a.b = c4(c->v_b.p); a.z = m4(Z0); a.cm = c4(c->v_cm.p); a.lm = c->d_lm.p;
+    a.p = c4(P0); a.qacc = c4(Q0); a.x = m4(X0); a.r = m4(R0); a.b = c4(c->v_b.p); a.z = nullptr; a.cm = c4(c->v_cm.p); a.lm = c->d_lm.p;
     a.ext_off = tp.ext_off; a.ext_pos = tp.ext_pos; a.qh = reinterpret_cast<const float2*>(c->lad_qh.p); a.e0 = (int)own.off0;
     a.pq_partials = pq_part0; a.d2_partials = d2_part0; a.n_pq = 0; a.n_d2 = 0;
     a.n_slice_wg = pcg_step3_slice_wgs(own.n, 0);
     a.sharded = 0; a.lad_sys = 0; a.redop = redop; a.redop_stride = rstride;
     a.K = K; a.fix_poses = p.fix_poses; a.fix_intr = p.fix_intr; a.fix_dist = p.fix_dist;
     a.cam_partials = c->lad_cam.p; a.n_cam = 0; a.cam_stride = NSP; a.Mblk = c->lad_mblk.p;
-    a.tp = P0 + to; a.tx = X0 + to; a.tr = R0 + to; a.tb = c->v_b.p + to; a.tD2 = c->lad_tail.p; a.tz = Z0 + to; a.tS = c->v_S.p + to;
+    a.tp = P0 + to; a.tx = X0 + to; a.tr = R0 + to; a.tb = c->v_b.p + to; a.tD2 = c->lad_tail.p; a.tz = TZ0; a.tS = c->v_S.p + to;
     a.step_partials = step_part0;
     std::vector<int> live(B); for (int j = 0; j < B; ++j) live[j] = j;
     auto set_slots = [&]() { for (int q = 0; q < LADDER_MAX; ++q) lv.sysid[q] = live[q < (int)live.size() ? q : (int)live.size() - 1]; };
@@ -670,7 +673,8 @@
     };
     int n_step = 0;
     set_slots();
-    { TimedScope t(c, I3D_K_VECTOR); a.cur = st2; n_step = launch_pcg_step3_lad(s, 0 , B, a, lv); }
+    { TimedScope t(c, I3D_K_VECTOR); a.cur = st2; n_step = launch_pcg_step3_lad(s, 0 , B, coloc, a, lv); }
+    c->lad_vec_wgs[0] = a.n_slice_wg; c->lad_vec_wgs[1] = n_step; c->lad_vec_wgs[3] = coloc ? 1 : 0;
     const int seq0 = c->pcg_seq;
     for (int j = 0; j < B; ++j) finals[j] = st2 + 2 * j;
     int it = 1;
@@ -679,17 +683,18 @@
         const int nl = (int)live.size();
         { const int rc = step_sums(nl, a.n_slice_wg); if (rc) return rc; }
         { TimedScope t(c, I3D_K_VECTOR);
-          a.n_d2 = launch_pcg_dir3_lad(s, it == 1, nl, own, to, L.NS, Z0, P0, c->v_S.p, U0, c->lad_tail.p, c->v_cm.p, c->d_lm.p, step_part0, n_step, d2_part0, st2, (it + 1) & 1, c->d_flags, seq0 + it, lv,
-                                       a.n_slice_wg, red4); }
+          a.n_d2 = launch_pcg_dir3_lad(s, it == 1, nl, coloc, own, to, L.NS, R0, TZ0, P0, c->v_S.p, U0, c->lad_tail.p, c->v_cm.p, c->d_lm.p, step_part0, n_step, d2_part0, st2, (it + 1) & 1, c->d_flags, seq0 + it, lv,
+                                       a.n_slice_wg, red4);
+          c->lad_vec_wgs[2] = a.n_d2; }
         { const int n = rows_apply(it & 1, true); if (n < 0) return ctx_fail(c, I3D_ERR_STATE, "pcg_solve_ladder: the multi-system operator pass could not be launched"); a.n_pq = n; a.n_cam = n; }
         a.cur = st2 + (it & 1);
-        if (it % 10 != 0) { TimedScope t(c, I3D_K_VECTOR); n_step = launch_pcg_step3_lad(s, 1, nl, a, lv); }
+        if (it % 10 != 0) { TimedScope t(c, I3D_K_VECTOR); n_step = launch_pcg_step3_lad(s, 1, nl, coloc, a, lv); }
         else {
-            { TimedScope t(c, I3D_K_VECTOR); launch_pcg_step3_lad(s, 2, nl, a, lv);
+            { TimedScope t(c, I3D_K_VECTOR); launch_pcg_step3_lad(s, 2, nl, coloc, a, lv);
               for (int j : live) { float* xj = X0 + (size_t)j * lv.vec; float* uj = U0 + (size_t)j * lv.vec;
                                    launch_mul2(s, own, c->v_S.p, xj, uj); launch_mul(s, L.NS, c->v_S.p + to, xj + to, uj + to); } }
             { const int n = rows_apply(it & 1, false); if (n < 0) return ctx_fail(c, I3D_ERR_STATE, "pcg_solve_ladder: the multi-system operator pass could not be launched"); a.n_cam = n; }
-            { TimedScope t(c, I3D_K_VECTOR); n_step = launch_pcg_step3_lad(s, 3, nl, a, lv); }
+            { TimedScope t(c, I3D_K_VECTOR); n_step = launch_pcg_step3_lad(s, 3, nl, coloc, a, lv); }
         }
         {
             const int want = seq0 + it;
```

Result: no change. 44.03 (median of 6 runs) (+1.8%).
